# pdlfs/old-vpic

Hardware: AMD Instinct MI355X
Metric: particle-pushes/sec (full step: advance_p + sort when due + field solve + glue) (higher is better)
Workload: dtype f32

## Files before the change

old-vpic_amd/csrc/collide.hip:

```cpp
#include "engine.h"
#include <algorithm>

namespace vpichip {

enum { CW_BAD = 0, CW_FULLEST_A, CW_FULLEST_B, CW_SLOTS = 8, COLLIDE_SLOTS = 64, COLLIDE_WORDS = CW_SLOTS + 4 * COLLIDE_SLOTS };
enum { CS_CELLS = 0, CS_PAIRS, CS_SKIPPED, CS_ONE_SIDED };
constexpr int COLLIDE_MAX_GROUPS_WAVE = 16384, COLLIDE_MAX_GROUPS = 4096;
constexpr int COLLIDE_SLAB_ARRAYS = 6;

__device__ __forceinline__ unsigned c_mix32(unsigned x) { x ^= x >> 16; x *= 0x7feb352du; x ^= x >> 15; x *= 0x846ca68bu; x ^= x >> 16; return x; }
__device__ __forceinline__ float c_unit(unsigned r) { return ((float)(r >> 8) + 0.5f) * (1.f / 16777216.f); }

struct CollideSpK {
  float *ux, *uy, *uz; const float *q; const float4 *r; const int *starts;
  int order, np;
  float wq, f;
  unsigned id;
};
struct CollideK {
  CollideSpK a, b;
  float cvar, dt, den;
  unsigned seed, call, rank;
  const float *draws;
  unsigned long long *words;
  int nx, ny, nz, sy, sz, nv, stride;
  TileK tk;
};

__global__ __launch_bounds__(256) void collide_check_particles(CollideSpK s, CollideK k) {
  const int p = blockIdx.x * 256 + threadIdx.x;
  bool bad = false;
  if (p < s.np) {
    const int v = record_cell(s.r, p);
    if (v < 0 || v >= k.nv) bad = true;
    else {
      int cx, cy, cz;
      voxel_cell(v, k.tk, cx, cy, cz);
      if (cx < 1 || cx > k.nx || cy < 1 || cy > k.ny || cz < 1 || cz > k.nz) bad = true;
      else {
        const int at = s.order == 2 ? sort_key<true>(v, k.tk) : v;
        bad = !(p >= s.starts[at] && p < s.starts[at + 1]);
      }
    }
  }
  if (__ballot(bad) && (threadIdx.x & 63) == 0) atomicOr(k.words + CW_BAD, 1ull);
}
__global__ __launch_bounds__(256) void collide_check_cells(CollideSpK s, int n_ranges, unsigned long long *words, int slot) {
// ... 12 lines not shown
struct Slab { float *ux, *uy, *uz, *w; unsigned *key; int *perm; };
__device__ __forceinline__ Slab slab_at(unsigned *base, int stride) {
  Slab s;
  s.ux = reinterpret_cast<float *>(base); s.uy = s.ux + stride; s.uz = s.uy + stride; s.w = s.uz + stride;
  s.key = base + 4 * stride; s.perm = reinterpret_cast<int *>(base + 5 * stride);
  return s;
}
__device__ __forceinline__ unsigned cell_c0(const CollideK &k, unsigned species, int v) {
  return c_mix32((k.seed ^ c_mix32(k.call * 0x9e3779b9u + species)) + c_mix32(k.rank * 0x85ebca6bu + (unsigned)v));
}
__device__ __forceinline__ void cell_range(const CollideSpK &s, int v, int key, int &lo, int &n) {
  lo = 0; n = 0;
  if (s.order == 0) return;
  const int at = s.order == 2 ? key : v;
  lo = s.starts[at]; n = s.starts[at + 1] - lo;
}
__device__ __forceinline__ bool block_cell(const CollideK &k, unsigned b, int &v, int &key) {
  int x, y, z;
  if (k.a.order == 2) {
    const int tile = (int)(b >> 6), c = (int)(b & 63u);
    const int tx = tile % k.tk.ntx, ty = (tile / k.tk.ntx) % k.tk.nty, tz = tile / (k.tk.ntx * k.tk.nty);
    x = tx << 2 | (c & 3); y = ty << 2 | (c >> 2 & 3); z = tz << 2 | (c >> 4);
    if (x >= k.nx || y >= k.ny || z >= k.nz) return false;
  } else {
    x = (int)(b % (unsigned)k.nx); y = (int)((b / (unsigned)k.nx) % (unsigned)k.ny); z = (int)(b / ((unsigned)k.nx * (unsigned)k.ny));
  }
  v = (x + 1) + k.sy * (y + 1) + k.sz * (z + 1);
  key = (((z >> 2) * k.tk.nty + (y >> 2)) * k.tk.ntx + (x >> 2)) * TILE_CELLS + ((z & 3) << 4 | (y & 3) << 2 | (x & 3));
  return true;
}
template <int T>
__device__ __forceinline__ void load_cell(const CollideSpK &s, const Slab &l, int lo, int n, unsigned c0) {
  for (int k = threadIdx.x; k < n; k += T) {
    l.ux[k] = s.ux[lo + k]; l.uy[k] = s.uy[lo + k]; l.uz[k] = s.uz[lo + k];
    l.w[k] = fabsf(s.q[lo + k]) * s.wq;
    l.key[k] = c_mix32(c0 + (unsigned)k);
  }
}
template <int T>
__device__ __forceinline__ void store_cell(const CollideSpK &s, const Slab &l, int lo, int n) {
  for (int k = threadIdx.x; k < n; k += T) { s.ux[lo + k] = l.ux[k]; s.uy[lo + k] = l.uy[k]; s.uz[lo + k] = l.uz[k]; }
}
template <int T>
__device__ __forceinline__ void rank_cell(const Slab &l, int n, unsigned c0) {
  if (T == 64) {
    const unsigned mine = c_mix32(c0 + threadIdx.x);
    int r = 0;
    for (int j = 0; j < n; j++) r += (unsigned)__shfl((int)mine, j) < mine ? 1 : 0;
    if ((int)threadIdx.x < n) l.perm[r] = (int)threadIdx.x;
  } else {
    for (int k = threadIdx.x; k < n; k += T) {
      const unsigned mine = l.key[k];
      int r = 0;
      for (int j = 0; j < n; j++) r += l.key[j] < mine ? 1 : 0;
      l.perm[r] = k;
    }
  }
}

struct Draws { float n, c, s, u; };
__device__ __forceinline__ Draws pair_draws(const CollideK &k, unsigned c0, unsigned j, int first_index) {
  Draws d;
  if (k.draws) {
    const float4 t = reinterpret_cast<const float4 *>(k.draws)[first_index];
    d.n = t.x; d.c = t.y; d.s = t.z; d.u = t.w;
  } else {
    const unsigned base = c_mix32(c0 ^ 0x2545f491u) + 4u * j;
    const float u0 = c_unit(c_mix32(base)), u1 = c_unit(c_mix32(base + 1u)), u2 = c_unit(c_mix32(base + 2u));
    d.n = sqrtf(-2.f * logf(u0)) * cospif(2.f * u1);
    d.s = sinpif(2.f * u2); d.c = cospif(2.f * u2);
    d.u = c_unit(c_mix32(base + 3u));
  }
  return d;
}
// ... 126 lines not shown
        for (int j = m; j < n_L; j += n_S) {
          const int kf = L.perm[j];
          count(pair_of<REL>(k, L, kf, S, ks, f_L, f_S, fN, false, pair_draws(k, c0_L, (unsigned)j, lo_L + kf)));
        }
      }
    }
    __syncthreads();
    store_cell<T>(k.a, A, lo_a, n_a);
    if (!SAME) store_cell<T>(k.b, B, lo_b, n_b);
  }
  __syncthreads();
  if (n_pairs) atomicAdd(&s_cnt[0], n_pairs);
  if (n_skipped) atomicAdd(&s_cnt[1], n_skipped);
  if (n_one_sided) atomicAdd(&s_cnt[2], n_one_sided);
  __syncthreads();
  if (threadIdx.x == 0 && cells) {
    unsigned long long *slot = k.words + CW_SLOTS + 4 * (blockIdx.x % COLLIDE_SLOTS);
    atomicAdd(slot + CS_CELLS, (unsigned long long)cells);
    if (s_cnt[0]) atomicAdd(slot + CS_PAIRS, (unsigned long long)s_cnt[0]);
    if (s_cnt[1]) atomicAdd(slot + CS_SKIPPED, (unsigned long long)s_cnt[1]);
    if (s_cnt[2]) atomicAdd(slot + CS_ONE_SIDED, (unsigned long long)s_cnt[2]);
  }
}

static CollideSpecies describe(const Species &s, const TileK &tk) {
  CollideSpecies d;
  d.np = s.np; d.n_sorted = s.n_sorted; d.n_holes = s.n_holes; d.fuse_pending = s.fuse_pending;
  d.tile_valid = s.tile_valid && tile_partition_usable(s, tk); d.coarse_sorted = s.coarse_sorted;
  d.partition_valid = !s.tile_valid && s.partition_valid && s.partition;
  return d;
}
static CollideSpK species_k(const Species &s, const CollideSpecies &d, int id, float wq, float f) {
  CollideSpK k;
  k.ux = s.p.ux; k.uy = s.p.uy; k.uz = s.p.uz; k.q = s.p.q; k.r = s.p.r;
  k.order = s.np == 0 ? 0 : d.tile_valid ? 2 : 1;
  k.starts = k.order == 2 ? s.tpart : s.partition;
  k.np = (int)s.np; k.wq = wq; k.f = f; k.id = (unsigned)id;
  return k;
}
static int sort_exact(Engine *e, Species &s, bool wants_tile) {
  if (s.nm > 0) VH_FAIL("collide: the species must be sorted first and has %lld movers pending", (long long)s.nm);
  const bool tile = s.tile_valid || (!s.partition_valid && wants_tile);
  const int knob = e->knobs.tile_coarse;
  e->knobs.tile_coarse = 0;
  const int rc = k_sort_p(e, s, tile, false);
  e->knobs.tile_coarse = knob;
  return rc;
}
static int check_species(Engine *e, const CollideSpK &s, const CollideK &k, int slot) {
  if (s.order == 0) return 0;
  const int n_ranges = s.order == 2 ? k.tk.ntiles * TILE_CELLS : k.nv;
  hipLaunchKernelGGL(collide_check_cells, dim3((n_ranges + 255) / 256), dim3(256), 0, e->stream, s, n_ranges, k.words, slot);
  hipLaunchKernelGGL(collide_check_particles, dim3((s.np + 255) / 256), dim3(256), 0, e->stream, s, k);
  VH_CHECK(hipGetLastError());
  return 0;
}

template <bool REL>
static void launch_collide(Engine *e, const CollideK &K, bool wave, bool same, unsigned groups, size_t lds, unsigned cells) {
  if (wave) {
    if (same) hipLaunchKernelGGL((collide_kernel<64, true, REL>), dim3(groups), dim3(64), lds, e->stream, K, cells);
    else hipLaunchKernelGGL((collide_kernel<64, false, REL>), dim3(groups), dim3(64), lds, e->stream, K, cells);
  } else {
    if (same) hipLaunchKernelGGL((collide_kernel<256, true, REL>), dim3(groups), dim3(256), lds, e->stream, K, cells);
    else hipLaunchKernelGGL((collide_kernel<256, false, REL>), dim3(groups), dim3(256), lds, e->stream, K, cells);
  }
}
// ... 63 lines not shown
```

old-vpic_amd/csrc/cool.hip:

```cpp
#include "dist_coords.h"
#include <algorithm>

namespace vpichip {

constexpr int COOL_WAVES = 4;
constexpr int COOL_THREADS = 64 * COOL_WAVES;
constexpr int COOL_MAX_BLOCKS = 1024;
constexpr int COOL_TOGETHER_ROUNDS = 2;
constexpr unsigned COOL_NEED = NEED_FIELD;
enum { COOL_SEEN = 0, COOL_CHANGED, COOL_REFUSED, COOL_ALONE, COOL_SUM };

struct CoolK { double sync, ic, quantum; };

template <bool DRY, bool CELLS>
__global__ __launch_bounds__(COOL_THREADS)
void cool_kernel(ParticlesK p, long long np, CoolK k, int nv, const vpic_interpolator_t *__restrict__ fi,
                 unsigned long long *__restrict__ cells, unsigned long long *__restrict__ stats) {
  const int lane = threadIdx.x & 63;
  const long long stride = (long long)gridDim.x * COOL_THREADS;
  long long idx = (long long)blockIdx.x * COOL_THREADS + threadIdx.x;
  unsigned long long n_seen = 0, n_changed = 0, n_refused = 0, n_alone = 0;
  long long sum = 0;
  DistRaw next = dist_load<true>(p, idx, np, COOL_NEED);
  float next_q = dist_load_q(p, idx, np, VAL_Q);
  for (; idx - lane < np; idx += stride) {
    const DistRaw r = next;
    const float q = next_q;
    const DistField f = dist_gather(fi, r.voxel, nv, COOL_NEED);
    next = dist_load<true>(p, idx + stride, np, COOL_NEED);
    next_q = dist_load_q(p, idx + stride, np, VAL_Q);
    const bool live = r.voxel >= 0 && r.voxel < nv;
    n_seen += __popcll(__ballot(live));
    bool tallied = false;
    long long addend = 0;
    if (live) {
      const float3 el = dist_e_at(r, f), cb = dist_b_at(r, f);
      const double Ex = (double)el.x, Ey = (double)el.y, Ez = (double)el.z, Bx = (double)cb.x, By = (double)cb.y, Bz = (double)cb.z;
      const double ux = (double)r.ux, uy = (double)r.uy, uz = (double)r.uz;
      const double u2 = (ux * ux + uy * uy) + uz * uz, g = sqrt(1.0 + u2), rg = 1.0 / g;
      const double vx = ux * rg, vy = uy * rg, vz = uz * rg;
      const double Lx = Ex + (vy * Bz - vz * By), Ly = Ey + (vz * Bx - vx * Bz), Lz = Ez + (vx * By - vy * Bx);
      const double vE = (vx * Ex + vy * Ey) + vz * Ez;
      const double Ax = (Ly * Bz - Lz * By) + vE * Ex, Ay = (Lz * Bx - Lx * Bz) + vE * Ey, Az = (Lx * By - Ly * Bx) + vE * Ez;
      const double L2 = (Lx * Lx + Ly * Ly) + Lz * Lz;
      double chi = L2 - vE * vE;
      if (chi < 0.0) chi = 0.0;
      const double D = g * (k.sync * chi + k.ic), den = 1.0 + D;
      const double nx = (ux + k.sync * Ax) / den, ny = (uy + k.sync * Ay) / den, nz = (uz + k.sync * Az) / den;
      if (isfinite(D) && isfinite(nx) && isfinite(ny) && isfinite(nz)) {
        const float fx = (float)nx, fy = (float)ny, fz = (float)nz;
        if (__float_as_uint(fx) != __float_as_uint(r.ux) || __float_as_uint(fy) != __float_as_uint(r.uy) ||
            __float_as_uint(fz) != __float_as_uint(r.uz)) n_changed++;
        if (!DRY) { p.ux[idx] = fx; p.uy[idx] = fy; p.uz[idx] = fz; }
        const double wx = (double)fx, wy = (double)fy, wz = (double)fz;
        const double u2n = (wx * wx + wy * wy) + wz * wz, g1 = sqrt(1.0 + u2n);
        const double val = (double)fabsf(q) * ((u2 - u2n) / (g + g1));
        const double t = val / k.quantum;
        tallied = fabs(t) < 4294967296.0;
        if (tallied) { addend = llrint(t); sum += addend; }
        else n_refused++;
      } else n_alone++;
    }
    if (CELLS) {
      bool pending = tallied;
#pragma unroll
      for (int round = 0; round < COOL_TOGETHER_ROUNDS; round++) {
        const unsigned long long any = __ballot(pending);
        if (!any) break;
        const int lead = __ffsll((long long)any) - 1;
        const int v0 = __builtin_amdgcn_readlane(r.voxel, lead);
        const bool shared = pending && r.voxel == v0;
        const unsigned long long same = __ballot(shared);
        add_sums_together(cells, r.voxel, addend, shared, __popcll(same) >= SUMS_TOGETHER_MIN, same, lead, lane);
        pending = pending && !shared;
      }
      if (pending && addend) atomicAdd(cells + r.voxel, (unsigned long long)addend);
    }
  }
#pragma unroll
  for (int m = 32; m >= 1; m >>= 1) {
    sum += __shfl_xor(sum, m);
    n_changed += __shfl_xor(n_changed, m);
    n_refused += __shfl_xor(n_refused, m);
    n_alone += __shfl_xor(n_alone, m);
  }
  if (lane == 0 && n_seen) {
// ... 28 lines not shown
```

old-vpic_amd/csrc/dist_coords.h:

```cpp
#pragma once
#include "engine.h"
#include <math.h>

namespace vpichip {

constexpr unsigned NEED_POS = 7u, NEED_KE = 3u << VPIC_HIP_COORD_KE;
constexpr unsigned NEED_FIELD = 0x3fu << VPIC_HIP_COORD_U_PAR, NEED_FIELD_E = 1u << VPIC_HIP_COORD_E_PAR;
constexpr unsigned NEED_FIELD_U = NEED_FIELD & ~(1u << VPIC_HIP_COORD_B | NEED_FIELD_E);
constexpr unsigned NEED_FIELD_PERP = 1u << VPIC_HIP_COORD_U_PERP | 1u << VPIC_HIP_COORD_MU;
static_assert(VPIC_HIP_COORD_U_PAR == 16 && VPIC_HIP_COORD_E_PAR == 21 && NEED_FIELD == 0x3f0000u, "the field coordinates are bits 16 to 21");

struct DistCoords { double x, y, z, ux, uy, uz, ke, log_ke, u_par, u_perp, pitch, mu, b, e_par; };

template <bool FIELDS>
__device__ __forceinline__ double dist_coord(const DistCoords &v, int coord) {
  if (FIELDS) {
    if (coord >= VPIC_HIP_COORD_U_PAR)
      return coord == VPIC_HIP_COORD_U_PAR ? v.u_par : coord == VPIC_HIP_COORD_U_PERP ? v.u_perp : coord == VPIC_HIP_COORD_PITCH ? v.pitch
           : coord == VPIC_HIP_COORD_MU ? v.mu : coord == VPIC_HIP_COORD_B ? v.b : v.e_par;
  }
  return coord == VPIC_HIP_COORD_X ? v.x : coord == VPIC_HIP_COORD_Y ? v.y : coord == VPIC_HIP_COORD_Z ? v.z
       : coord == VPIC_HIP_COORD_UX ? v.ux : coord == VPIC_HIP_COORD_UY ? v.uy : coord == VPIC_HIP_COORD_UZ ? v.uz
       : coord == VPIC_HIP_COORD_KE ? v.ke : v.log_ke;
}

template <bool FIELDS>
__device__ __forceinline__ bool dist_in_range(const DistCoords &v, const vpic_hip_dist_range_t &r) {
  const double c = dist_coord<FIELDS>(v, r.coord);
  return c >= r.lo && c < r.hi;
}

template <bool FIELDS>
__device__ __forceinline__ bool dist_in_ranges(const DistCoords &v, const vpic_hip_dist_range_t (&sel)[4], int n_sel) {
  bool in = true;
  if (n_sel > 0) in = in && dist_in_range<FIELDS>(v, sel[0]);
  if (n_sel > 1) in = in && dist_in_range<FIELDS>(v, sel[1]);
  if (n_sel > 2) in = in && dist_in_range<FIELDS>(v, sel[2]);
  if (n_sel > 3) in = in && dist_in_range<FIELDS>(v, sel[3]);
  return in;
}

struct DistRaw { int voxel; float dx, dy, dz, ux, uy, uz; };

template <bool FIELDS>
__device__ __forceinline__ DistRaw dist_load(const ParticlesK &p, long long idx, long long end, unsigned need) {
  DistRaw r{-1, 0.f, 0.f, 0.f, 0.f, 0.f, 0.f};
  const bool u = FIELDS && (need & NEED_FIELD_U);
  if (idx < end) {
    const float4 rec = p.r[idx];
    r.voxel = record_cell(rec); r.dx = rec.x; r.dy = rec.y; r.dz = rec.z;
    if (u || (need & (NEED_KE | 1u << VPIC_HIP_COORD_UX))) r.ux = p.ux[idx];
    if (u || (need & (NEED_KE | 1u << VPIC_HIP_COORD_UY))) r.uy = p.uy[idx];
    if (u || (need & (NEED_KE | 1u << VPIC_HIP_COORD_UZ))) r.uz = p.uz[idx];
  }
  return r;
}

struct DistField { float4 b; float2 c; float4 ex, ey, ez; };

__device__ __forceinline__ DistField dist_gather(const vpic_interpolator_t *__restrict__ fi, int voxel, int nv, unsigned need) {
  DistField f{};
  if (voxel >= 0 && voxel < nv) {
    const float4 *q = reinterpret_cast<const float4 *>(fi + voxel);
    f.b = q[3];
    f.c = *reinterpret_cast<const float2 *>(q + 4);
    if (need & NEED_FIELD_E) { f.ex = q[0]; f.ey = q[1]; f.ez = q[2]; }
  }
  return f;
}
static_assert(sizeof(vpic_interpolator_t) == 80, "an interpolator record is five float4");

__device__ __forceinline__ float3 dist_b_at(const DistRaw &r, const DistField &f) {
  return make_float3(f.b.x + r.dx * f.b.y, f.b.z + r.dy * f.b.w, f.c.x + r.dz * f.c.y);
}
__device__ __forceinline__ float3 dist_e_at(const DistRaw &r, const DistField &f) {
  return make_float3((f.ex.x + r.dy * f.ex.y) + r.dz * (f.ex.z + r.dy * f.ex.w),
                     (f.ey.x + r.dz * f.ey.y) + r.dx * (f.ey.z + r.dz * f.ey.w),
                     (f.ez.x + r.dx * f.ez.y) + r.dy * (f.ez.z + r.dx * f.ez.w));
}

template <bool FIELDS>
__device__ __forceinline__ DistCoords dist_coords(const DistRaw &r, const DistField &f, unsigned need, const TileK &t, int &cx, int &cy, int &cz) {
  DistCoords v{};
  if (need & NEED_POS) {
    voxel_cell(r.voxel, t, cx, cy, cz);
    if (need & 1u) v.x = (double)(cx - 1) + ((double)r.dx + 1.0) * 0.5;
// ... 11 lines not shown
    const double b = sqrt((bx * bx + by * by) + bz * bz);
    v.b = b;
    if (need & NEED_FIELD_U) {
      const double u_par = ((v.ux * bx + v.uy * by) + v.uz * bz) / b;
      const double u2 = (v.ux * v.ux + v.uy * v.uy) + v.uz * v.uz;
      v.u_par = u_par;
      if (need & NEED_FIELD_PERP) {
        const double perp2 = u2 - u_par * u_par;
        const double p2 = perp2 < 0.0 ? 0.0 : perp2;
        if (need & 1u << VPIC_HIP_COORD_U_PERP) v.u_perp = sqrt(p2);
        if (need & 1u << VPIC_HIP_COORD_MU) v.mu = p2 / (2.0 * b);
      }
      if (need & 1u << VPIC_HIP_COORD_PITCH) v.pitch = u_par / sqrt(u2);
    }
    if (need & NEED_FIELD_E) {
      const float3 el = dist_e_at(r, f);
      v.e_par = (((double)el.x * bx + (double)el.y * by) + (double)el.z * bz) / b;
    }
  }
  return v;
}

constexpr unsigned VAL_Q = 1u, VAL_EDOTV = 2u, VAL_EPAR_VPAR = 4u;
inline void dist_factor_need(int code, unsigned &need, unsigned &vneed) {
  if (code < VPIC_HIP_FACTOR_ONE) { need |= 1u << code; return; }
  if (code == VPIC_HIP_FACTOR_Q) vneed |= VAL_Q;
  if (code == VPIC_HIP_FACTOR_EDOTV) { vneed |= VAL_EDOTV; need |= 1u << VPIC_HIP_COORD_KE | NEED_FIELD_E; }
  if (code == VPIC_HIP_FACTOR_EPAR_VPAR) { vneed |= VAL_EPAR_VPAR; need |= 1u << VPIC_HIP_COORD_KE | NEED_FIELD_E | 1u << VPIC_HIP_COORD_U_PAR; }
}

struct DistExtra { double q, edotv, epar_vpar; };

__device__ __forceinline__ float dist_load_q(const ParticlesK &p, long long idx, long long end, unsigned vneed) {
  return (vneed & VAL_Q) && idx < end ? p.q[idx] : 0.f;
}

template <bool FIELDS>
__device__ __forceinline__ DistExtra dist_extra(const DistRaw &r, const DistField &f, float q, const DistCoords &v, unsigned vneed) {
  DistExtra x{};
  x.q = (double)q;
  if (FIELDS && (vneed & (VAL_EDOTV | VAL_EPAR_VPAR))) {
    const double gamma = sqrt(((1.0 + v.ux * v.ux) + v.uy * v.uy) + v.uz * v.uz);
    if (vneed & VAL_EDOTV) {
      const float3 el = dist_e_at(r, f);
      x.edotv = (((double)el.x * v.ux + (double)el.y * v.uy) + (double)el.z * v.uz) / gamma;
    }
    if (vneed & VAL_EPAR_VPAR) x.epar_vpar = (v.e_par * v.u_par) / gamma;
  }
  return x;
}

template <bool FIELDS>
__device__ __forceinline__ double dist_factor(const DistCoords &v, const DistExtra &x, int code) {
  if (code >= VPIC_HIP_FACTOR_ONE)
    return code == VPIC_HIP_FACTOR_ONE ? 1.0 : code == VPIC_HIP_FACTOR_Q ? x.q
         : FIELDS && code == VPIC_HIP_FACTOR_EDOTV ? x.edotv : x.epar_vpar;
  return dist_coord<FIELDS>(v, code);
}

struct SelectK {
  vpic_hip_select_t s;
  unsigned need;
  int use_tag;
};
inline SelectK make_select_k(const vpic_hip_select_t &d) {
  SelectK k{};
  k.s = d;
// ... 18 lines not shown
```

old-vpic_amd/csrc/engine.h:

```cpp
#pragma once
#include <hip/hip_runtime.h>
#include <stdint.h>
#include <string>
#include <vector>
#include "vpic_hip.h"
#include "policy.h"
#include "moments_device.h"

namespace vpichip {

void set_error(const char *fmt, ...);
#define VH_CHECK(expr)                                                                     \
  do {                                                                                     \
    hipError_t _e = (expr);                                                                \
    if (_e != hipSuccess) {                                                                \
      vpichip::set_error("%s failed: %s (%s:%d)", #expr, hipGetErrorString(_e), __FILE__, __LINE__); \
      return 1;                                                                            \
    }                                                                                      \
  } while (0)
#define VH_FAIL(...) do { vpichip::set_error(__VA_ARGS__); return 1; } while (0)

struct GridK {
  int nx, ny, nz, sy, sz, nv;
  int fbc[6], pbc[6];
  int rank;
};

enum { F_EX = 0, F_EY, F_EZ, F_DIV_E_ERR, F_CBX, F_CBY, F_CBZ, F_DIV_B_ERR,
       F_TCAX, F_TCAY, F_TCAZ, F_RHOB, F_JFX, F_JFY, F_JFZ, F_RHOF, F_NCOMP };
enum { M_EMATX = 0, M_EMATY, M_EMATZ, M_NMAT, M_FMATX, M_FMATY, M_FMATZ, M_CMAT, M_NCOMP };
struct FieldsK {
  float *c[F_NCOMP];
  uint16_t *m[M_NCOMP];
};

struct ParticlesK {
  float4 *r;
  float *ux, *uy, *uz, *q;
};
__host__ __device__ __forceinline__ float4 make_record(float dx, float dy, float dz, int i) {
  union { int i; float f; } w; w.i = i;
  return make_float4(dx, dy, dz, w.f);
}
__device__ __forceinline__ int record_cell(const float4 *r, long long k) { return __float_as_int(r[k].w); }
__device__ __forceinline__ int record_cell(const float4 &v) { return __float_as_int(v.w); }
__device__ __forceinline__ void record_set_cell(float4 *r, long long k, int i) { r[k].w = __int_as_float(i); }
__host__ __device__ __forceinline__ ParticlesK offset_particles(const ParticlesK &p, int64_t at) {
  ParticlesK o = p;
  o.r += at; o.ux += at; o.uy += at; o.uz += at; o.q += at;
  return o;
}

struct DrainParams {
  int nx, ny, nz, sy, sz, rank, max_nm;
  unsigned mul_sz;
  int pbc[6];
  unsigned mul_sy, shifts;
  vpic_particle_mover_t *pm;
  int *nm_counter;
};

inline void magic_div(unsigned d, unsigned &mul, unsigned &shift) {
  unsigned l = 0;
  while ((1ull << l) < d) l++;
  const unsigned p = 31 + l;
  mul = (unsigned)(((unsigned long long)1 << p) / d + 1);
  shift = p - 32;
}

enum { C_NM = 0, C_DISORDER = 1, C_LOCAL = 2, C_SEND = 8, C_HOLES = 14, C_FILLS = 15, C_NP = 16, C_NMS = 48, C_CHARGED = 80, C_OVER = 81, C_RETRY = 82, C_QMSG = 83, C_NHOLE = 96, C_QTOP = 128, C_TOTAL = 160 };
constexpr int MAX_SPECIES = 32;
constexpr int HEADER_BASE = 256, MAX_HEADERS = 192;
constexpr int RETRY_CAP = 1 << 16;
static_assert(C_NMS + MAX_SPECIES == C_CHARGED && C_NP + MAX_SPECIES == C_NMS && C_NHOLE + MAX_SPECIES == C_QTOP && C_QTOP + MAX_SPECIES == C_TOTAL && C_TOTAL <= HEADER_BASE, "counter layout");

struct Species {
  float q_m = 0;
  float q_max = 0;
  int64_t np = 0, max_np = 0, nm = 0, max_nm = 0;
  int64_t n_holes = 0;
  ParticlesK p{}, aux{};
  DrainParams *drain_k = nullptr;
// ... 374 lines not shown
```

old-vpic_amd/csrc/engine.hip:

```cpp
#include "engine.h"
#include "cell_coords.h"
#include <algorithm>
#include <cstdarg>
#include <cstdio>
#include <cstring>
#include <functional>
#include <cstdlib>
#include <cmath>

namespace vpichip {

static thread_local char g_error[1024] = "";
void set_error(const char *fmt, ...) {
  va_list ap;
  va_start(ap, fmt);
  vsnprintf(g_error, sizeof(g_error), fmt, ap);
  va_end(ap);
}

static vpic_hip_host_access_fn g_host_access = nullptr;
void host_will_read(const void *p, size_t bytes) { if (g_host_access && p && bytes) g_host_access(p, bytes, 0); }
void host_will_write(void *p, size_t bytes) { if (g_host_access && p && bytes) g_host_access(p, bytes, 1); }

int ensure_stage(Engine *e, size_t bytes) { return grow(e->stage, e->stage_bytes, bytes); }
// ... 103 lines not shown
static double fixed_scale(double largest) {
  int ex = 0;
  (void)frexp(largest, &ex);
  return ldexp(1.0, 37 - ex);
}
int acc_prepare_det(Engine *e, double q_arriving) {
  if (!e->acc64) {
    VH_CHECK(hipMalloc(&e->acc64, sizeof(unsigned long long) * 12 * (size_t)e->gk.nv));
    VH_CHECK(hipMemsetAsync(e->acc64, 0, sizeof(unsigned long long) * 12 * (size_t)e->gk.nv, e->stream));
  }
  if (e->acc_scale == 0) {
    double q = e->acc_qref;
    if (!(q > 0)) for (auto &s : e->species) q = std::max(q, (double)s.q_max);
    if (!(q > 0)) q = q_arriving;
    if (!(q > 0) && q_arriving < 0) return 0;
    if (!(q > 0)) VH_FAIL("deterministic accumulation: no macro-particle charge is known yet (give vpic_hip_set_accumulation a reference charge)");
    e->acc_scale = fixed_scale(4.2 * q);
  }
  e->acc64_dirty = true;
  return 0;
}
int acc_finalize(Engine *e) {
  if (!e->acc64 || !e->acc64_dirty) return 0;
  const size_t n = 12 * (size_t)e->gk.nv;
  hipLaunchKernelGGL(acc_finalize_kernel, dim3((unsigned)((n + 255) / 256)), dim3(256), 0, e->stream,
                     reinterpret_cast<float *>(e->acc), e->acc64, n, 1.0 / e->acc_scale);
  VH_CHECK(hipGetLastError());
  e->acc64_dirty = false;
  return 0;
}

void free_particles(ParticlesK &p) {
  (void)hipFree(p.r);
  (void)hipFree(p.ux); (void)hipFree(p.uy); (void)hipFree(p.uz); (void)hipFree(p.q);
  p = ParticlesK{};
}

static void destroy(Engine *e) {
  if (e->stream) (void)hipStreamSynchronize(e->stream);
  for (auto &s : e->species) {
    free_particles(s.p); free_particles(s.aux);
    (void)hipFree(s.tag); (void)hipFree(s.tag2); (void)hipFree(s.tag_aux); (void)hipFree(s.tag2_aux);
    (void)hipFree(s.pm); (void)hipFree(s.partition); (void)hipFree(s.tpart); (void)hipFree(s.tpart2); (void)hipFree(s.ttail); (void)hipFree(s.hist); (void)hipFree(s.drain_k); (void)hipFree(s.crossed_dev); (void)hipHostFree(s.crossed_host);
    for (int i = 0; i < 4; i++) if (s.ev[i]) (void)hipEventDestroy(s.ev[i]);
    for (auto ev : s.sp_ev) if (ev) (void)hipEventDestroy(ev);
    for (auto ev : s.hp_ev) if (ev) (void)hipEventDestroy(ev);
  }
  (void)hipFree(e->field_block); (void)hipFree(e->mat_block); (void)hipFree(e->mc);
  (void)hipFree(e->fi); (void)hipFree(e->acc_block); (void)hipHostFree(e->host_miss); (void)hipFree(e->stage); (void)hipFree(e->counters); (void)hipFree(e->hydro); (void)hipFree(e->hydro_buf[0]); (void)hipFree(e->hydro_buf[1]);
  (void)hipHostFree(e->host_counters); (void)hipFree(e->dsum); (void)hipHostFree(e->host_dsum);
  (void)hipFree(e->sort_next); (void)hipFree(e->scan_tmp);
  (void)hipFree(e->face_buf[0]); (void)hipFree(e->face_buf[1]);
  for (int f = 0; f < 6; f++) (void)hipFree(e->send_buf[f]);
  (void)hipFree(e->local_buf); (void)hipFree(e->reflux_draws); (void)hipFree(e->emit_draws);
  (void)hipFree(e->wall_table); (void)hipFree(e->wall_rec); (void)hipFree(e->wall_cursor);
  (void)hipFree(e->collide_draws); (void)hipFree(e->collide_dev); (void)hipHostFree(e->collide_host);
  (void)hipFree(e->load_draws); (void)hipFree(e->load_tab);
  (void)hipFree(e->cool_cells); (void)hipHostFree(e->cool_cells_host); e->cool_stats.release();
  (void)hipFree(e->hole_list); (void)hipFree(e->fill_list); (void)hipFree(e->tail_flag);
  (void)hipFree(e->sp_table_dev); (void)hipHostFree(e->sp_table_host); (void)hipFree(e->xmsg_dev); (void)hipHostFree(e->xmsg_host);
  (void)hipFree(e->retry_buf); (void)hipFree(e->tile_list[0]); (void)hipFree(e->tile_list[1]);
  (void)hipFree(e->acc64); (void)hipFree(e->rho64);
  (void)hipFree(e->spec_lin); (void)hipFree(e->spec_bands); (void)hipFree(e->spec_log); (void)hipHostFree(e->spec_log_host);
  e->species_hist.release(); e->cell_hist.release(); (void)hipFree(e->hydro64);
  (void)hipFree(e->sel_mask); (void)hipFree(e->sel_offsets); (void)hipFree(e->sel_counts);
  (void)hipFree(e->sel_p); (void)hipFree(e->sel_f); (void)hipFree(e->sel_i);
  for (DiagStats<4> *st : {&e->spec_stats, &e->dist_stats, &e->mom_stats, &e->sel_stats}) st->release();
  for (auto &ev : e->ev_pool) { (void)hipEventDestroy(ev.first); (void)hipEventDestroy(ev.second); }
// ... 365 lines not shown
  if (s.nm == 0) return 0;
  host_will_write(pm, sizeof(*pm) * (size_t)s.nm);
  if (copy_out(e, pm, s.pm, sizeof(*pm) * (size_t)s.nm)) return 1;
  std::sort(pm, pm + s.nm, [](const vpic_particle_mover_t &a, const vpic_particle_mover_t &b) { return a.i < b.i; });
  return 0;
}
int vpic_hip_species_get_partition(vpic_hip_engine_t *e, int sp, int32_t *partition) {
  ENGINE(e); SPECIES(e, sp);
  Species &s = e->species[sp];
  if (!s.partition || !s.partition_valid) VH_FAIL("partition is only valid right after sort_p");
  return copy_out(e, partition, s.partition, sizeof(int) * ((size_t)e->gk.nv + 1));
}

#ifdef VPIC_HIP_ABLATION
int vpic_hip_debug_set_ablate(vpic_hip_engine_t *e, int bits) { ENGINE(e); e->knobs.ablate = bits; return 0; }
#endif
int vpic_hip_debug_poke_tile_max(vpic_hip_engine_t *e, int sp, unsigned value) {
  ENGINE(e); SPECIES(e, sp);
  if (!e->species[sp].crossed_host) VH_FAIL("no counter word");
  e->species[sp].crossed_host[PW_FULLEST_TILE] = value;
  return 0;
}
int vpic_hip_debug_set_particles_any_voxel(vpic_hip_engine_t *e, int sp, const vpic_particle_t *p, int64_t np) {
  ENGINE(e); SPECIES(e, sp);
  if (np < 0 || (np > 0 && !p)) VH_FAIL("Bad particle array");
  host_will_read(p, sizeof(*p) * (size_t)np);
  return k_particles_from_aos(e, e->species[sp], p, np, 0, true);
}
int vpic_hip_debug_set_momenta(vpic_hip_engine_t *e, int sp, const float *ux, const float *uy, const float *uz, int64_t n) {
  ENGINE(e); SPECIES(e, sp);
  Species &s = e->species[sp];
  if (!ux || !uy || !uz || n != s.np) VH_FAIL("Bad momenta: %lld, the species' extent is %lld", (long long)n, (long long)s.np);
  if (n == 0) return 0;
  if (copy_in(e, s.p.ux, ux, sizeof(float) * (size_t)n) || copy_in(e, s.p.uy, uy, sizeof(float) * (size_t)n)) return 1;
  return copy_in(e, s.p.uz, uz, sizeof(float) * (size_t)n);
}
int vpic_hip_species_get_tile_partition(vpic_hip_engine_t *e, int sp, int32_t *tpart, int64_t *count) {
  ENGINE(e); SPECIES(e, sp);
  Species &s = e->species[sp];
  const int64_t n1 = (int64_t)make_tile_k(e->gk).ntiles * TILE_CELLS + 1;
  if (count) *count = n1;
  if (!tpart) return 0;
  if (!s.tpart || !s.tile_valid || s.tpart_count < n1) VH_FAIL("the tile partition is only valid while the species is in the engine's order");
  return copy_out(e, tpart, s.tpart, sizeof(int) * (size_t)n1);
}

int vpic_hip_load_interpolator(vpic_hip_engine_t *e) { ENGINE(e); return k_load_interpolator(e); }
int vpic_hip_clear_accumulators(vpic_hip_engine_t *e) {
  ENGINE(e);
  VH_CHECK(hipMemsetAsync(e->acc, 0, sizeof(vpic_accumulator_t) * (size_t)e->gk.nv, e->stream));
  if (e->acc64 && e->acc64_dirty) {
    VH_CHECK(hipMemsetAsync(e->acc64, 0, sizeof(unsigned long long) * 12 * (size_t)e->gk.nv, e->stream));
    e->acc64_dirty = false;
  }
  return 0;
}
int vpic_hip_set_accumulation(vpic_hip_engine_t *e, int mode, double q_ref) {
  ENGINE(e);
  if (mode != 0 && mode != 1) VH_FAIL("Bad accumulation mode %d", mode);
  if (acc_finalize(e)) return 1;
  e->det_acc = mode == 1;
  e->acc_qref = q_ref > 0 ? q_ref : 0;
  e->acc_scale = 0;
  return 0;
}
int vpic_hip_reduce_accumulators(vpic_hip_engine_t *e) { ENGINE(e); return 0; }
int vpic_hip_unload_accumulator(vpic_hip_engine_t *e) { ENGINE(e); return k_unload_accumulator(e); }
int vpic_hip_set_push_mode(vpic_hip_engine_t *e, int mode) {
// ... 587 lines not shown
```

old-vpic_amd/csrc/fields.hip:

```cpp
#include "push_device.h"

namespace vpichip {

#define VOX(x, y, z) ((x) + g.sy * (y) + g.sz * (z))

struct Box3 { int bx, by, bz; };
__device__ __forceinline__ bool decode(const Box3 &b, unsigned t, int &x, int &y, int &z) {
  const unsigned per_z = (unsigned)b.bx * b.by;
  if (t >= per_z * (unsigned)b.bz) return false;
  const unsigned zz = t / per_z, r = t - zz * per_z, yy = r / (unsigned)b.bx;
  x = 1 + (int)(r - yy * b.bx); y = 1 + (int)yy; z = 1 + (int)zz;
  return true;
}

constexpr int BAND = 8;
__host__ __device__ __forceinline__ unsigned banded_count(const Box3 &b) {
  return (unsigned)((b.by + BAND - 1) / BAND) * (unsigned)b.bz * BAND * (unsigned)b.bx;
}
static inline unsigned banded_grid(const Box3 &b) { return ((banded_count(b) + 255u) / 256u + 7u) / 8u * 8u; }
__device__ __forceinline__ bool decode_banded(const Box3 &b, unsigned block, unsigned nblocks, unsigned tid, int &x, int &y, int &z) {
  const unsigned t = xcd_block(block, nblocks) * 256u + tid;
  if (t >= banded_count(b)) return false;
  const unsigned r = t / (unsigned)b.bx, yy = r % BAND, r2 = r / BAND, band = r2 / (unsigned)b.bz;
  x = 1 + (int)(t - r * b.bx); z = 1 + (int)(r2 - band * b.bz); y = 1 + (int)(band * BAND + yy);
// ... 699 lines not shown
  const vpic_hip_grid_t &G = e->grid;
  if (!e->mc) VH_FAIL("energy_f: no material coefficients set");
  const int nb = (int)(e->dsum_count / 6);
  if (e->f.m[0])
    hipLaunchKernelGGL(energy_f_kernel<false>, dim3(nb), dim3(256), 0, e->stream, e->f, e->mc, g, e->dsum);
  else
    hipLaunchKernelGGL(energy_f_kernel<true>, dim3(nb), dim3(256), 0, e->stream, e->f, e->mc, g, e->dsum);
  VH_CHECK(hipGetLastError());
  VH_CHECK(hipMemcpyAsync(e->host_dsum, e->dsum, sizeof(double) * 6 * nb, hipMemcpyDeviceToHost, e->stream));
  VH_CHECK(hipStreamSynchronize(e->stream));
  const double v0 = 0.5 * G.eps0 * G.dx * G.dy * G.dz;
  for (int k = 0; k < 6; k++) {
    double s = 0;
    for (int b = 0; b < nb; b++) s += e->host_dsum[b * 6 + k];
    en6[k] = s * v0;
  }
  return 0;
}



int k_clear_rhof(Engine *e) {
  VH_CHECK(hipMemsetAsync(e->f.c[F_RHOF], 0, sizeof(float) * (size_t)e->gk.nv, e->stream));
  return 0;
}

__global__ __launch_bounds__(256)
void accumulate_rho_p_kernel(float *__restrict__ rhof, ParticlesK p, int np, float r8V, int sy, int sz) {
  const int idx = blockIdx.x * 256 + threadIdx.x;
  if (idx >= np) return;
  const float4 rec = p.r[idx];
  if (record_cell(rec) < 0) return;
  float w[8];
  node_weights(rec.x, rec.y, rec.z, p.q[idx], r8V, w);
  float *r = rhof + record_cell(rec);
  atomicAdd(r, w[0]); atomicAdd(r + 1, w[1]); atomicAdd(r + sy, w[2]); atomicAdd(r + sy + 1, w[3]);
  atomicAdd(r + sz, w[4]); atomicAdd(r + sz + 1, w[5]); atomicAdd(r + sz + sy, w[6]); atomicAdd(r + sz + sy + 1, w[7]);
}
__global__ __launch_bounds__(256)
void accumulate_rho_cells_kernel(float *__restrict__ rhof, ParticlesK p, const int *__restrict__ partition, int nv,
                                 float r8V, int sy, int sz) {
  const int v = blockIdx.x * 256 + threadIdx.x;
  if (v >= nv) return;
  const int first = partition[v], last = partition[v + 1];
  if (first >= last) return;
  float s0 = 0, s1 = 0, s2 = 0, s3 = 0, s4 = 0, s5 = 0, s6 = 0, s7 = 0;
#pragma unroll 1
  for (int idx = first; idx < last; idx++) {
    float w[8];
    const float4 rec = p.r[idx];
    node_weights(rec.x, rec.y, rec.z, p.q[idx], r8V, w);
    s0 += w[0]; s1 += w[1]; s2 += w[2]; s3 += w[3]; s4 += w[4]; s5 += w[5]; s6 += w[6]; s7 += w[7];
  }
  float *r = rhof + v;
  atomicAdd(r, s0); atomicAdd(r + 1, s1); atomicAdd(r + sy, s2); atomicAdd(r + sy + 1, s3);
  atomicAdd(r + sz, s4); atomicAdd(r + sz + 1, s5); atomicAdd(r + sz + sy, s6); atomicAdd(r + sz + sy + 1, s7);
}
int k_rho_p_untiled(Engine *e, Species &s, bool by_cell) {
  const vpic_hip_grid_t &G = e->grid;
  const float r8V = 0.125 * G.rdx * G.rdy * G.rdz;
  if (by_cell) {
    if (!s.partition_valid && k_sort_p(e, s)) return 1;
    hipLaunchKernelGGL(accumulate_rho_cells_kernel, dim3((unsigned)((e->gk.nv + 255) / 256)), dim3(256), 0, e->stream,
                       e->f.c[F_RHOF], s.p, s.partition, e->gk.nv, r8V, e->gk.sy, e->gk.sz);
    VH_CHECK(hipGetLastError());
    return 0;
  }
  hipLaunchKernelGGL(accumulate_rho_p_kernel, dim3((unsigned)((s.np + 255) / 256)), dim3(256), 0, e->stream,
                     e->f.c[F_RHOF], s.p, (int)s.np, r8V, e->gk.sy, e->gk.sz);
  VH_CHECK(hipGetLastError());
  return 0;
}

static int local_adjust_rho(Engine *e) {
  const GridK &g = e->gk;
  for (int comp = 0; comp < 2; comp++)
    for (int face = 0; face < 6; face++) {
      const int bc = g.fbc[face];
      if (bc >= 0) continue;
      const int axis = face % 3, hi = face >= 3, n = n_axis(g, axis);
      const PlaneBox b = node_box(g, axis, hi ? n + 1 : 1);
      if (bc == VPIC_PEC_FIELDS) { if (local_op(e, one_seg(b, e->f.c[comp ? F_RHOB : F_RHOF]), L_ZERO)) return 1; }
      else if (!comp)            { if (local_op(e, one_seg(b, e->f.c[F_RHOF]), L_DOUBLE)) return 1; }
    }
// ... 445 lines not shown
```

old-vpic_amd/csrc/load.hip:

```cpp
#include "engine.h"
#include "load_rule.h"
#include <cmath>
#include <cstring>
#include <algorithm>
#include <vector>

namespace vpichip {

struct LoadK {
  const int *count;
  const float *q, *ud[3], *uth[3];
  int tsx, tsy, tsz;
  long long g0x, g0y, g0z, GX, GY;
  unsigned seed, stream;
  int flip;
  const float *draws;
  long long tag0;
};

__global__ __launch_bounds__(256)
void load_counts_kernel(int *__restrict__ per_voxel, int nv, GridK g, TileK t, LoadK k) {
  const int v = blockIdx.x * 256 + threadIdx.x;
  if (v > nv) return;
  int n = 0;
// ... 27 lines not shown
  if (threadIdx.x == 64) s_span[1] = holding_voxel(off, 0, nv, m_last);
  __syncthreads();
  const int v0 = s_span[0], v1 = s_span[1], span = v1 - v0;
  const bool in_lds = span < LOAD_SPAN;
  if (in_lds) {
    for (int a = threadIdx.x; a <= span + 1; a += 256) s_off[a] = off[v0 + a];
    __syncthreads();
  }
  const int m = m0 + (int)threadIdx.x;
  if (m >= total) return;
  int v, first;
  if (in_lds) { const int a = holding_voxel(s_off, 0, span + 1, m); v = v0 + a; first = s_off[a]; }
  else { v = holding_voxel(off, v0, v1 + 1, m); first = off[v]; }
  int cx, cy, cz;
  voxel_cell(v, t, cx, cy, cz);
  cx -= 1; cy -= 1; cz -= 1;
  const int at = cx * k.tsx + cy * k.tsy + cz * k.tsz;
  const uint64_t cell = load_global_cell((uint64_t)(k.g0x + cx), (uint64_t)(k.g0y + cy), (uint64_t)(k.g0z + cz), (uint64_t)k.GX, (uint64_t)k.GY);
  float d[7];
  if (k.draws) {
#pragma unroll
    for (int a = 0; a < 7; a++) d[a] = k.draws[7ll * m + a];
  } else {
    uint32_t r[8];
    load_words(cell, (uint32_t)(m - first), k.seed, k.stream, r);
    load_numbers(r, d);
  }
  float uth[3], ud[3], u[3];
#pragma unroll
  for (int a = 0; a < 3; a++) { uth[a] = k.uth[a] ? k.uth[a][at] : 0.f; ud[a] = k.ud[a] ? k.ud[a][at] : 0.f; }
  const float n[3] = {d[3], d[4], d[5]};
  load_momentum(uth, ud, n, d[6], k.flip != 0, u);
  p.r[m] = make_record(load_offset(d[0]), load_offset(d[1]), load_offset(d[2]), v);
  p.ux[m] = u[0]; p.uy[m] = u[1]; p.uz[m] = u[2]; p.q[m] = k.q[at];
  if (tags) { tag[m] = tags == 1 ? k.tag0 + m : 0; tag2[m] = 0; }
}

int k_load_profile(Engine *e, Species &s, const vpic_hip_load_t &d, int64_t *n_loaded) {
  const GridK &g = e->gk;
  const int n[3] = {g.nx, g.ny, g.nz};
  if (!d.count) VH_FAIL("load_profile: count is NULL");
  if (!d.q) VH_FAIL("load_profile: q is NULL");
  if (d.flags & ~(VPIC_HIP_LOAD_APPEND | VPIC_HIP_LOAD_FLIP | VPIC_HIP_LOAD_TAGS)) VH_FAIL("load_profile: flags = %d has unknown bits", d.flags);
  const bool append = d.flags & VPIC_HIP_LOAD_APPEND, with_tags = d.flags & VPIC_HIP_LOAD_TAGS;
  for (int a = 0; a < 3; a++) {
    if (d.tdim[a] != 1 && d.tdim[a] != n[a]) VH_FAIL("load_profile: tdim[%d] = %d is neither 1 nor the grid's %d", a, d.tdim[a], n[a]);
    if (d.goff[a] < 0) VH_FAIL("load_profile: goff[%d] = %lld is negative", a, (long long)d.goff[a]);
    if (d.goff[a] > d.gdim[a] - n[a]) VH_FAIL("load_profile: goff[%d] + %d = %lld is beyond gdim[%d] = %lld", a, n[a], (long long)d.goff[a] + n[a], a, (long long)d.gdim[a]);
  }
  if ((double)d.gdim[0] * (double)d.gdim[1] * (double)d.gdim[2] >= 9.2e18) VH_FAIL("load_profile: gdim holds more than 2^63 cells");
  const int64_t T = (int64_t)d.tdim[0] * d.tdim[1] * d.tdim[2], cells = (int64_t)g.nx * g.ny * g.nz, mult = cells / T;
  const size_t count_bytes = sizeof(int32_t) * (size_t)T, table_bytes = sizeof(float) * (size_t)T;
  host_will_read(d.count, count_bytes); host_will_read(d.q, table_bytes);
  for (int a = 0; a < 3; a++) { host_will_read(d.ud[a], table_bytes); host_will_read(d.uth[a], table_bytes); }
  int64_t sum = 0;
  float q_top = 0;
  for (int64_t c = 0; c < T; c++) {
    if (d.count[c] < 0) VH_FAIL("load_profile: count[%lld] = %d is negative", (long long)c, d.count[c]);
    if (!std::isfinite(d.q[c])) VH_FAIL("load_profile: q[%lld] is not finite", (long long)c);
    for (int a = 0; a < 3; a++) {
      if (d.ud[a] && !std::isfinite(d.ud[a][c])) VH_FAIL("load_profile: ud[%d][%lld] is not finite", a, (long long)c);
      if (d.uth[a] && !std::isfinite(d.uth[a][c])) VH_FAIL("load_profile: uth[%d][%lld] is not finite", a, (long long)c);
      if (d.uth[a] && d.uth[a][c] < 0) VH_FAIL("load_profile: uth[%d][%lld] = %g is negative", a, (long long)c, (double)d.uth[a][c]);
    }
    sum += d.count[c];
    if (d.count[c] > 0) q_top = std::max(q_top, fabsf(d.q[c]));
  }
// ... 74 lines not shown
```

old-vpic_amd/csrc/moments.hip:

```cpp
#include "engine.h"
#include "push_device.h"
#include "dist_coords.h"
#include <algorithm>
#include <math.h>

namespace vpichip {

constexpr int MOM_WX = TILE_EDGE + 3;
constexpr int MOM_SLOTS = MOM_WX * MOM_WX * MOM_WX;
constexpr int MOM_TAIL_BLOCKS = 4096;

struct MomK {
  ParticlesK p;
  const float4 *fi;
  const int *tpart; const unsigned *bad;
  long long n_sorted, np;
  int sy, sz, nv_safe;
  TileK t;
  HydroConsts h;
  double scale[HYDRO_MOMENTS];
  unsigned long long *stats;
};
enum { MOM_SEL_NONE = 0, MOM_SEL_BOX = 1, MOM_SEL_FIELD = 2 };
template <int SEL> struct MomKS : MomK { SelectK sel; const int64_t *tag; };
// ... 6 lines not shown
  if (j >= ntiles) return;
  const long long b0 = tpart[(size_t)j * TILE_CELLS], b1 = j + 1 < ntiles ? (long long)tpart[(size_t)(j + 1) * TILE_CELLS] : n_sorted;
  if (b0 < 0 || b0 > b1 || b1 > n_sorted || (j == 0 && b0 != 0)) atomicOr(bad, 1u);
}
int k_check_tile_partition(Engine *e, const Species &s, unsigned *bad) {
  const int ntiles = make_tile_k(e->gk).ntiles;
  hipLaunchKernelGGL(check_tile_partition_kernel, dim3((ntiles + 255) / 256), dim3(256), 0, e->stream, (const int *)s.tpart, ntiles,
                     (long long)s.n_sorted, bad);
  VH_CHECK(hipGetLastError());
  return 0;
}

__device__ __forceinline__ void mom_add(float *word, float x, double, unsigned &) { atomicAdd(word, x); }
__device__ __forceinline__ void mom_add(unsigned long long *word, float x, double scale, unsigned &n_range) {
  if (fabs((double)x * scale) < 2251799813685248.0) atomicAdd(word, to_fixed(x, scale));
  else n_range++;
}

template <int NM, typename ACC> struct MomLayout { static constexpr int STRIDE = NM; };
template <> struct MomLayout<HYDRO_MOMENTS, float> { static constexpr int STRIDE = HYDRO_STRIDE; };

struct MomCount { unsigned live = 0, lds = 0, global = 0, range = 0; };

template <int NM, typename ACC, bool WINDOW, int SEL>
__device__ __forceinline__ void moments_of_particle(const MomKS<SEL> &K, ACC *__restrict__ out, ACC *s_win, long long idx, int bx, int by, int bz, MomCount &n) {
  const float4 rec = K.p.r[idx];
  const int voxel = record_cell(rec);
  if (voxel < 0 || voxel >= K.nv_safe) return;
  HydroP P;
  if constexpr (SEL != MOM_SEL_NONE) {
    static_assert(NM == HYDRO_MOMENTS, "a selection is for the hydro moments");
    constexpr bool FIELDS = SEL == MOM_SEL_FIELD;
    if (K.sel.use_tag && !select_tag_ok(K.sel.s, K.tag ? K.tag[idx] : 0)) return;
    const DistRaw r{voxel, rec.x, rec.y, rec.z, K.p.ux[idx], K.p.uy[idx], K.p.uz[idx]};
    InterpK f;
    if (FIELDS) f = load_interp(K.fi, voxel);
    if (K.sel.s.n_sel > 0) {
      const DistField df = FIELDS ? DistField{f.b0, f.b1, f.ex, f.ey, f.ez} : DistField{};
      int cx = 0, cy = 0, cz = 0;
      const DistCoords v = dist_coords<FIELDS>(r, df, K.sel.need, K.t, cx, cy, cz);
      if (!dist_in_ranges<FIELDS>(v, K.sel.s.sel, K.sel.s.n_sel)) return;
    }
    if (!FIELDS) f = load_interp(K.fi, voxel);
    n.live++;
    hydro_particle(r.dx, r.dy, r.dz, r.ux, r.uy, r.uz, K.p.q[idx], f, K.h, P);
  } else {
    n.live++;
    if constexpr (NM == HYDRO_MOMENTS)
      hydro_particle(rec.x, rec.y, rec.z, K.p.ux[idx], K.p.uy[idx], K.p.uz[idx], K.p.q[idx], load_interp(K.fi, voxel), K.h, P);
    else
      node_weights(rec.x, rec.y, rec.z, K.p.q[idx], K.h.r8V, P.w);
  }
  bool inside = false;
  int slot0 = 0;
  if (WINDOW) {
    int cx, cy, cz;
    voxel_cell(voxel, K.t, cx, cy, cz);
    const unsigned lx = (unsigned)(cx - bx), ly = (unsigned)(cy - by), lz = (unsigned)(cz - bz);
    inside = lx < (unsigned)(MOM_WX - 1) && ly < (unsigned)(MOM_WX - 1) && lz < (unsigned)(MOM_WX - 1);
    slot0 = (int)(lx + MOM_WX * (ly + MOM_WX * lz));
  }
  unsigned range = 0;
  if constexpr (SEL != MOM_SEL_NONE) { n.lds += inside ? 1u : 0u; n.global += inside ? 0u : 1u; }
  if (WINDOW && inside) {
#pragma unroll
    for (int nd = 0; nd < 8; nd++) {
      float c[NM];
      if constexpr (NM == HYDRO_MOMENTS) hydro_node(P, P.w[nd], K.h.mc_q, c); else c[0] = P.w[nd];
      const int slot = slot0 + (nd & 1) + ((nd >> 1) & 1) * MOM_WX + (nd >> 2) * MOM_WX * MOM_WX;
#pragma unroll
      for (int k = 0; k < NM; k++) mom_add(&s_win[k * MOM_SLOTS + slot], c[k], K.scale[k], range);
    }
    if constexpr (SEL == MOM_SEL_NONE) n.lds++;
  } else {
    ACC *g = out + (size_t)voxel * MomLayout<NM, ACC>::STRIDE;
#pragma unroll
    for (int nd = 0; nd < 8; nd++) {
      float c[NM];
      if constexpr (NM == HYDRO_MOMENTS) hydro_node(P, P.w[nd], K.h.mc_q, c); else c[0] = P.w[nd];
      ACC *m = g + (size_t)((nd & 1) + ((nd >> 1) & 1) * K.sy + (nd >> 2) * K.sz) * MomLayout<NM, ACC>::STRIDE;
#pragma unroll
      for (int k = 0; k < NM; k++) mom_add(m + k, c[k], K.scale[k], range);
    }
    if constexpr (SEL == MOM_SEL_NONE) n.global++;
// ... 185 lines not shown
```

old-vpic_amd/csrc/particles.hip:

```cpp
#include "push_device.h"
#include "unit_draw.h"
#include "dist_coords.h"
#include <cstddef>
#include <cstring>
#include <algorithm>

namespace vpichip {

__global__ void particles_from_aos_kernel(ParticlesK p, int64_t *tag, int64_t *tag2,
                                          const vpic_particle_t *__restrict__ src, int64_t first, int n) {
  const int t = blockIdx.x * blockDim.x + threadIdx.x;
  if (t >= n) return;
  const vpic_particle_t s = src[t];
  const int64_t k = first + t;
  p.r[k] = make_record(s.dx, s.dy, s.dz, s.i);
  p.ux[k] = s.ux; p.uy[k] = s.uy; p.uz[k] = s.uz; p.q[k] = s.q;
  if (tag) { tag[k] = s.tag; tag2[k] = s.tag2; }
}
__global__ void particles_to_aos_kernel(ParticlesK p, const int64_t *tag, const int64_t *tag2,
                                        vpic_particle_t *__restrict__ dst, int64_t first, int n) {
  const int t = blockIdx.x * blockDim.x + threadIdx.x;
  if (t >= n) return;
  const int64_t k = first + t;
  vpic_particle_t s;
  const float4 rec = p.r[k];
  s.dx = rec.x; s.dy = rec.y; s.dz = rec.z; s.i = record_cell(rec);
  s.ux = p.ux[k]; s.uy = p.uy[k]; s.uz = p.uz[k]; s.q = p.q[k];
  s.tag = tag ? tag[k] : 0; s.tag2 = tag ? tag2[k] : 0;
  dst[t] = s;
}

static int alloc_particles_raw_impl(ParticlesK &p, int64_t n);
static int alloc_particles_raw(ParticlesK &p, int64_t n) { return alloc_particles_raw_impl(p, n); }
static const int64_t CHUNK = 8 << 20;

int ensure_tags(Engine *e, Species &s) {
  if (s.tag) return 0;
  VH_CHECK(hipMalloc(&s.tag, sizeof(int64_t) * s.max_np));
  VH_CHECK(hipMalloc(&s.tag2, sizeof(int64_t) * s.max_np));
  VH_CHECK(hipMemsetAsync(s.tag, 0, sizeof(int64_t) * s.max_np, e->stream));
  VH_CHECK(hipMemsetAsync(s.tag2, 0, sizeof(int64_t) * s.max_np, e->stream));
  return 0;
}

int k_particles_from_aos(Engine *e, Species &s, const vpic_particle_t *host, int64_t n_new, int64_t at, bool any_voxel) {
  const int64_t np = at + n_new;
  if (np > s.max_np) VH_FAIL("species particles: np=%lld exceeds max_np=%lld", (long long)np, (long long)s.max_np);
  {
    const GridK &g = e->gk;
    for (int64_t k = 0; k < n_new; k++) {
      const int v = host[k].i, z = v / g.sz, r = v - z * g.sz, y = r / g.sy, x = r - y * g.sy;
      if (any_voxel && v >= 0 && v < g.nv) continue;
      if (v < 0 || (unsigned)(x - 1) >= (unsigned)g.nx || (unsigned)(y - 1) >= (unsigned)g.ny || (unsigned)(z - 1) >= (unsigned)g.nz)
        VH_FAIL("particle %lld is not in an interior voxel (i = %d)", (long long)k, v);
    }
  }
  bool any_tag = false;
  for (int64_t k = 0; k < n_new && !any_tag; k++) any_tag = host[k].tag != 0 || host[k].tag2 != 0;
  if (any_tag) { if (ensure_tags(e, s)) return 1; s.has_tags = true; }
  bool any_q = false;
// ... 19 lines not shown
  if (cap < count) VH_FAIL("species_get_particles: buffer holds %lld, asked for %lld", (long long)cap, (long long)count);
  host -= from;
  for (int64_t first = from; first < from + count; first += CHUNK) {
    const int n = (int)((from + count - first < CHUNK) ? from + count - first : CHUNK);
    if (ensure_stage(e, sizeof(vpic_particle_t) * (size_t)n)) return 1;
    hipLaunchKernelGGL(particles_to_aos_kernel, dim3((n + 255) / 256), dim3(256), 0, e->stream, s.p,
                       s.has_tags ? s.tag : nullptr, s.tag2, (vpic_particle_t *)e->stage, first, n);
    VH_CHECK(hipGetLastError());
    VH_CHECK(hipMemcpyAsync(host + first, e->stage, sizeof(vpic_particle_t) * (size_t)n, hipMemcpyDeviceToHost, e->stream));
    VH_CHECK(hipStreamSynchronize(e->stream));
  }
  return 0;
}

__device__ __forceinline__ unsigned hash32(unsigned x) {
  x ^= x >> 16; x *= 0x7feb352du; x ^= x >> 15; x *= 0x846ca68bu; x ^= x >> 16;
  return x;
}
__device__ __forceinline__ float u01(unsigned seed, unsigned idx, unsigned k) {
  const unsigned h = hash32(hash32(idx * 9u + k) ^ hash32(seed * 0x9e3779b9u + k));
  return unit_top_closed(h);
}
__global__ __launch_bounds__(256)
void load_maxwellian_kernel(ParticlesK p, GridK g, int ppc, int np, unsigned seed, float q,
                            float ux0, float uy0, float uz0, float vth) {
  const int idx = blockIdx.x * 256 + threadIdx.x;
  if (idx >= np) return;
  const int cell = idx / ppc;
  const int cz = cell / (g.nx * g.ny), r = cell - cz * g.nx * g.ny, cy = r / g.nx, cx = r - cy * g.nx;
  p.r[idx] = make_record(2.f * u01(seed, idx, 0) - 1.f, 2.f * u01(seed, idx, 1) - 1.f, 2.f * u01(seed, idx, 2) - 1.f,
                         (cx + 1) + g.sy * (cy + 1) + g.sz * (cz + 1));
  const float r1 = sqrtf(-2.f * logf(u01(seed, idx, 3))), a1 = 6.2831853f * u01(seed, idx, 4);
  const float r2 = sqrtf(-2.f * logf(u01(seed, idx, 5))), a2 = 6.2831853f * u01(seed, idx, 6);
  p.ux[idx] = ux0 + vth * r1 * cosf(a1);
  p.uy[idx] = uy0 + vth * r1 * sinf(a1);
  p.uz[idx] = uz0 + vth * r2 * cosf(a2);
  p.q[idx] = q;
}

int k_load_maxwellian(Engine *e, Species &s, int ppc, unsigned seed, float q, float ux, float uy, float uz, float vth) {
  const int64_t np = (int64_t)e->gk.nx * e->gk.ny * e->gk.nz * ppc;
  if (ppc < 1 || np > s.max_np) VH_FAIL("load_maxwellian: %lld particles exceed max_np=%lld", (long long)np, (long long)s.max_np);
  hipLaunchKernelGGL(load_maxwellian_kernel, dim3((unsigned)((np + 255) / 256)), dim3(256), 0, e->stream, s.p, e->gk,
                     ppc, (int)np, seed, q, ux, uy, uz, vth);
  VH_CHECK(hipGetLastError());
  s.np = np; s.nm = 0; s.partition_valid = false; s.tile_valid = false; s.n_holes = 0; s.hist_valid = false;
  s.q_max = std::max(s.q_max, fabsf(q));
  s.chargeless = q == 0.f;
  return 0;
}

constexpr int MAX_GROUPS = 16;
__device__ __forceinline__ void group_info(int key, bool valid, int lane, int &leader, int &rank, int &cnt) {
  unsigned long long todo = __ballot(valid);
  leader = lane; rank = 0; cnt = 1;
  for (int it = 0; todo && it < MAX_GROUPS; ++it) {
    const int lead = __ffsll((long long)todo) - 1;
    const int k0 = __builtin_amdgcn_readlane(key, lead);
    const bool mine = valid && key == k0;
    const unsigned long long m = __ballot(mine);
    if (mine) {
      leader = lead;
      rank = (int)__builtin_amdgcn_mbcnt_hi((unsigned)(m >> 32), __builtin_amdgcn_mbcnt_lo((unsigned)m, 0u));
      cnt = __popcll(m);
    }
    todo &= ~m;
  }
}

TileK make_tile_k(const GridK &g) {
// ... 50 lines not shown
    const int v = k < nb ? block_sum[k] : 0;
    int incl = v;
    for (int off = 1; off < 64; off <<= 1) { const int u = __shfl_up(incl, off); if (lane >= off) incl += u; }
    if (lane == 63) s_wave[threadIdx.x >> 6] = incl;
    __syncthreads();
    int wave_off = 0;
    for (int w = 0; w < (int)(threadIdx.x >> 6); w++) wave_off += s_wave[w];
    const int carry = s_carry;
    if (k < nb) block_sum[k] = carry + wave_off + incl - v;
    __syncthreads();
    if (threadIdx.x == 255) s_carry = carry + wave_off + incl;
    __syncthreads();
  }
}
__global__ __launch_bounds__(256)
void scan_add_kernel(int *__restrict__ out, int *__restrict__ copy, const int *__restrict__ block_sum, int n) {
  const int base = blockIdx.x * 1024 + threadIdx.x * 4;
  const int add = block_sum[blockIdx.x];
#pragma unroll
  for (int k = 0; k < 4; k++)
    if (base + k < n) { const int v = out[base + k] + add; out[base + k] = v; copy[base + k] = v; }
}

template <bool TILE>
__global__ __launch_bounds__(256)
void sort_scatter_kernel(ParticlesK in, ParticlesK out, const int64_t *tin, const int64_t *t2in,
                         int64_t *tout, int64_t *t2out, int np, int *__restrict__ next, const TileK t) {
  const int idx = blockIdx.x * 256 + threadIdx.x;
  const int lane = threadIdx.x & 63;
  const int li = idx < np ? idx : 0;
  const float4 rec = in.r[li];
  const int key = idx < np ? record_cell(rec) : -1;
  const bool valid = key >= 0;
  const float ux = in.ux[li], uy = in.uy[li], uz = in.uz[li], q = in.q[li];
  int leader, rank, cnt;
  group_info(key, valid, lane, leader, rank, cnt);
  int base = 0;
  if (valid && lane == leader) base = atomicAdd(&next[sort_key<TILE>(key, t)], cnt);
  base = __shfl(base, leader);
  if (!valid) return;
  const int dst = base + rank;
  out.r[dst] = rec;
  out.ux[dst] = ux; out.uy[dst] = uy; out.uz[dst] = uz; out.q[dst] = q;
  if (tin) { tout[dst] = tin[idx]; t2out[dst] = t2in[idx]; }
}

#ifndef VPIC_HIP_SORT_THREADS
#define VPIC_HIP_SORT_THREADS 256
#endif
#ifndef VPIC_HIP_SORT_XCD
#define VPIC_HIP_SORT_XCD 1
#endif
constexpr int WG_T = VPIC_HIP_SORT_THREADS, WG_PER_THREAD = 8, WG_CHUNK = WG_T * WG_PER_THREAD, WG_TABLE = 512, WG_EPT = WG_TABLE / WG_T;
static_assert(WG_T == 256 || WG_T == 512, "threads of a sort workgroup");

__device__ __forceinline__ int wg_slot(int *s_key, int skey) {
  unsigned h = ((unsigned)skey * 2654435761u) >> 23;
  for (int probe = 0; probe < WG_TABLE; probe++) {
    const int prev = atomicCAS(&s_key[h], -1, skey);
    if (prev == -1 || prev == skey) return (int)h;
    h = (h + 1) & (WG_TABLE - 1);
  }
  return -1;
}

template <bool TILE>
__global__ __launch_bounds__(WG_T)
void wg_count_kernel(const float4 *__restrict__ rec, int np, int *__restrict__ count, const TileK t) {
  __shared__ int s_key[WG_TABLE], s_cnt[WG_TABLE];
  for (int k = threadIdx.x; k < WG_TABLE; k += WG_T) { s_key[k] = -1; s_cnt[k] = 0; }
  __syncthreads();
  const int first = blockIdx.x * WG_CHUNK;
  int key[WG_PER_THREAD];
#pragma unroll
  for (int j = 0; j < WG_PER_THREAD; j++) { const int idx = first + j * WG_T + threadIdx.x; key[j] = idx < np ? record_cell(rec, idx) : -1; }
  const int lane = threadIdx.x & 63;
#pragma unroll
  for (int j = 0; j < WG_PER_THREAD; j++) {
    const bool valid = key[j] >= 0;
    int leader, rank, cnt;
    group_info(key[j], valid, lane, leader, rank, cnt);
    if (valid && lane == leader) {
      const int skey = sort_key<TILE>(key[j], t);
      const int h = wg_slot(s_key, skey);
      if (h >= 0) atomicAdd(&s_cnt[h], cnt); else atomicAdd(&count[skey], cnt);
    }
  }
  __syncthreads();
  for (int k = threadIdx.x; k < WG_TABLE; k += WG_T) if (s_key[k] >= 0) atomicAdd(&count[s_key[k]], s_cnt[k]);
}

template <bool TILE, bool COARSE = false>
__global__ __launch_bounds__(WG_T)
void wg_scatter_kernel(ParticlesK in, ParticlesK out, const int64_t *tin, const int64_t *t2in,
                       int64_t *tout, int64_t *t2out, int np, int *__restrict__ next, const TileK t) {
  static_assert(WG_CHUNK >= 4 * WG_TABLE, "the tables fit the first staging buffer");
  __shared__ float4 s_both[WG_CHUNK / 2];
  int *const s_tables = reinterpret_cast<int *>(s_both);
  float *const s_stage = reinterpret_cast<float *>(s_both) + WG_CHUNK;
  int *const s_key = s_tables, *const s_cnt = s_tables + WG_TABLE, *const s_lbase = s_tables + 2 * WG_TABLE, *const s_gbase = s_tables + 3 * WG_TABLE;
  __shared__ int s_dst[WG_CHUNK];
  __shared__ int s_wave[WG_T / 64], s_total;
  for (int k = threadIdx.x; k < WG_TABLE; k += WG_T) { s_key[k] = -1; s_cnt[k] = 0; }
  __syncthreads();
#if VPIC_HIP_SORT_XCD
  if ((long long)xcd_block(blockIdx.x, gridDim.x) * WG_CHUNK >= np) return;
  const int first = (int)xcd_block(blockIdx.x, gridDim.x) * WG_CHUNK;
#else
  if ((long long)blockIdx.x * WG_CHUNK >= np) return;
  const int first = blockIdx.x * WG_CHUNK;
#endif
  int slot[WG_PER_THREAD], rank[WG_PER_THREAD], key[WG_PER_THREAD];
#pragma unroll
  for (int j = 0; j < WG_PER_THREAD; j++) { const int idx = first + j * WG_T + threadIdx.x; key[j] = idx < np ? record_cell(in.r, idx) : -1; }
  const int lane = threadIdx.x & 63;
#pragma unroll
  for (int j = 0; j < WG_PER_THREAD; j++) {
    const bool valid = key[j] >= 0;
    int leader, r, cnt, h = -2, base = 0;
    const int gkey = COARSE ? (valid ? sort_key<true>(key[j], t) / TILE_CELLS : -1) : key[j];
    group_info(gkey, valid, lane, leader, r, cnt);
    if (valid && lane == leader) {
      const int skey = COARSE ? gkey * TILE_CELLS : sort_key<TILE>(key[j], t);
      h = wg_slot(s_key, skey);
      if (h >= 0) base = atomicAdd(&s_cnt[h], cnt);
      else base = atomicAdd(&next[skey], cnt);
    }
    h = __shfl(h, leader); base = __shfl(base, leader);
    slot[j] = valid ? h : -2; rank[j] = base + r;
  }
  __syncthreads();
  {
    int c[WG_EPT], t = 0;
#pragma unroll
    for (int k = 0; k < WG_EPT; k++) { c[k] = s_cnt[WG_EPT * threadIdx.x + k]; t += c[k]; }
    int incl = t;
    const int lane = threadIdx.x & 63;
    for (int off = 1; off < 64; off <<= 1) { const int u = __shfl_up(incl, off); if (lane >= off) incl += u; }
    if (lane == 63) s_wave[threadIdx.x >> 6] = incl;
    __syncthreads();
    int wave_off = 0;
    for (int w = 0; w < (int)(threadIdx.x >> 6); w++) wave_off += s_wave[w];
    int run = wave_off + incl - t;
#pragma unroll
    for (int k = 0; k < WG_EPT; k++) {
      s_lbase[WG_EPT * threadIdx.x + k] = run; run += c[k];
      if (c[k]) s_gbase[WG_EPT * threadIdx.x + k] = atomicAdd(&next[s_key[WG_EPT * threadIdx.x + k]], c[k]);
    }
    if (threadIdx.x == WG_T - 1) s_total = wave_off + incl;
  }
  __syncthreads();
  int local[WG_PER_THREAD];
#pragma unroll
  for (int j = 0; j < WG_PER_THREAD; j++) {
    local[j] = -1;
    if (slot[j] >= 0) { local[j] = s_lbase[slot[j]] + rank[j]; s_dst[local[j]] = s_gbase[slot[j]] + rank[j]; }
  }
  __syncthreads();
  const int n_staged = s_total;
  float *const src[4] = {in.ux, in.uy, in.uz, in.q};
  float *const dst[4] = {out.ux, out.uy, out.uz, out.q};
  float *const stage2 = reinterpret_cast<float *>(s_tables);
  float v[WG_PER_THREAD];
  {
    constexpr int HALF = WG_CHUNK / 2, GROUP = 4;
#pragma unroll
    for (int half = 0; half < 2; half++) {
#pragma unroll
      for (int j0 = 0; j0 < WG_PER_THREAD; j0 += GROUP) {
        float4 rec[GROUP];
        bool here[GROUP];
#pragma unroll
        for (int j = 0; j < GROUP; j++) {
          const int idx = first + (j0 + j) * WG_T + threadIdx.x;
          here[j] = local[j0 + j] >= 0 ? (local[j0 + j] >= HALF) == (half == 1) : (slot[j0 + j] == -1 && half == 0);
          rec[j] = here[j] ? in.r[idx] : make_float4(0.f, 0.f, 0.f, 0.f);
        }
#pragma unroll
        for (int j = 0; j < GROUP; j++) {
          if (!here[j]) continue;
          if (local[j0 + j] >= 0) s_both[local[j0 + j] - half * HALF] = rec[j];
          else out.r[rank[j0 + j]] = rec[j];
        }
      }
      if (half == 1) {
#pragma unroll
        for (int j = 0; j < WG_PER_THREAD; j++) { const int idx = first + j * WG_T + threadIdx.x; v[j] = (slot[j] != -2) ? src[0][idx] : 0.f; }
      }
      __syncthreads();
      for (int k = threadIdx.x; k < HALF; k += WG_T) { if (half * HALF + k < n_staged) out.r[s_dst[half * HALF + k]] = s_both[k]; }
      __syncthreads();
    }
  }
#pragma unroll
  for (int f = 0; f < 4; f++) {
    float *const stage = (f & 1) ? stage2 : s_stage;
    float vn[WG_PER_THREAD];
    if (f + 1 < 4) {
#pragma unroll
      for (int j = 0; j < WG_PER_THREAD; j++) { const int idx = first + j * WG_T + threadIdx.x; vn[j] = (slot[j] != -2) ? src[f + 1][idx] : 0.f; }
    }
#pragma unroll
    for (int j = 0; j < WG_PER_THREAD; j++) {
      if (local[j] >= 0) stage[local[j]] = v[j];
      else if (slot[j] == -1) dst[f][rank[j]] = v[j];
    }
    __syncthreads();
#pragma unroll
    for (int j = 0; j < WG_PER_THREAD; j++) { const int k = j * WG_T + threadIdx.x; if (k < n_staged) dst[f][s_dst[k]] = stage[k]; }
    if (f + 1 < 4) {
#pragma unroll
      for (int j = 0; j < WG_PER_THREAD; j++) v[j] = vn[j];
    }
  }
  if (tin) {
#pragma unroll
    for (int j = 0; j < WG_PER_THREAD; j++) {
      if (slot[j] == -2) continue;
      const int idx = first + j * WG_T + threadIdx.x;
      const int d = local[j] >= 0 ? s_dst[local[j]] : rank[j];
      tout[d] = tin[idx]; t2out[d] = t2in[idx];
    }
  }
}

constexpr int COARSE_CHUNK = 2048, COARSE_PER_THREAD = COARSE_CHUNK / 256, COARSE_TABLE = 128;

__device__ __forceinline__ int tile_of(int voxel, const TileK &t) { return sort_key<true>(voxel, t) / TILE_CELLS; }

__device__ __forceinline__ int coarse_slot(int *s_key, int tile) {
  unsigned h = ((unsigned)tile * 2654435761u) >> 25;
  for (int probe = 0; probe < COARSE_TABLE; probe++) {
    const int prev = atomicCAS(&s_key[h], -1, tile);
    if (prev == -1 || prev == tile) return (int)h;
    h = (h + 1) & (COARSE_TABLE - 1);
  }
  return -1;
}

__global__ __launch_bounds__(256)
void coarse_count_kernel(const float4 *__restrict__ rec, int np, int *__restrict__ count, const TileK t) {
  __shared__ int s_key[COARSE_TABLE], s_cnt[COARSE_TABLE];
  if (threadIdx.x < COARSE_TABLE) { s_key[threadIdx.x] = -1; s_cnt[threadIdx.x] = 0; }
  __syncthreads();
  const int first = blockIdx.x * COARSE_CHUNK;
#pragma unroll
  for (int j = 0; j < COARSE_PER_THREAD; j++) {
    const int idx = first + j * 256 + threadIdx.x;
    const int voxel = idx < np ? record_cell(rec, idx) : -1;
    if (voxel >= 0) {
      const int tile = tile_of(voxel, t);
      const int h = coarse_slot(s_key, tile);
      if (h >= 0) atomicAdd(&s_cnt[h], 1);
      else atomicAdd(&count[tile * TILE_CELLS], 1);
    }
  }
  __syncthreads();
  if (threadIdx.x < COARSE_TABLE && s_key[threadIdx.x] >= 0) atomicAdd(&count[s_key[threadIdx.x] * TILE_CELLS], s_cnt[threadIdx.x]);
}

int alloc_particles(ParticlesK &p, int64_t n_req) {
  const int64_t n = (n_req + PUSH_TILE + PARTICLE_PAD - 1) / PARTICLE_PAD * PARTICLE_PAD;
  if (alloc_particles_raw(p, n)) return 1;
  VH_CHECK(hipMemset(p.r + (n - PARTICLE_PAD), 0, sizeof(float4) * PARTICLE_PAD));
  float *arr[4] = {p.ux, p.uy, p.uz, p.q};
  for (float *a : arr) VH_CHECK(hipMemset(a + (n - PARTICLE_PAD), 0, sizeof(float) * PARTICLE_PAD));
  VH_CHECK(hipDeviceSynchronize());
  return 0;
}
static int alloc_particles_raw_impl(ParticlesK &p, int64_t n) {
  VH_CHECK(hipMalloc(&p.r, sizeof(float4) * n));
  VH_CHECK(hipMalloc(&p.ux, sizeof(float) * n)); VH_CHECK(hipMalloc(&p.uy, sizeof(float) * n));
  VH_CHECK(hipMalloc(&p.uz, sizeof(float) * n)); VH_CHECK(hipMalloc(&p.q, sizeof(float) * n));
  return 0;
}

__global__ __launch_bounds__(256) void tile_max_kernel(const int *__restrict__ tpart, int ntiles, unsigned *__restrict__ host_word) {
  __shared__ int s_max[4];
  int m = 0;
  for (int t = blockIdx.x * 256 + threadIdx.x; t < ntiles; t += gridDim.x * 256) m = max(m, tpart[(t + 1) * TILE_CELLS] - tpart[t * TILE_CELLS]);
  for (int off = 32; off; off >>= 1) m = max(m, __shfl_down(m, off));
  if ((threadIdx.x & 63) == 0) s_max[threadIdx.x >> 6] = m;
  __syncthreads();
  if (threadIdx.x == 0) atomicMax(host_word, (unsigned)max(max(s_max[0], s_max[1]), max(s_max[2], s_max[3])));
}
__global__ void clear_word_kernel(unsigned *__restrict__ w) { *w = 0; }
__global__ void publish_word_kernel(unsigned *__restrict__ host_word, const unsigned *__restrict__ dev_word) { *host_word = *dev_word; }

int k_sort_p(Engine *e, Species &s, bool tile_order, bool may_fuse) {
  const TileK tk = make_tile_k(e->gk);
  const int n1 = (tile_order ? tk.ntiles * TILE_CELLS : e->gk.nv) + 1;
  SortInputs in;
  in.tile_order = tile_order; in.may_fuse = may_fuse; in.np = s.np; in.n_sorted = s.n_sorted;
  in.adaptive = s.adaptive; in.chargeless = s.chargeless; in.has_tags = s.has_tags;
  in.tile_valid = s.tile_valid; in.coarse_sorted = s.coarse_sorted; in.counts_ready = s.hist_valid && s.hist && s.hist_count >= n1;
  in.det_acc = e->det_acc; in.time_kernels = e->time_kernels; in.tile_coarse = e->knobs.tile_coarse; in.old_sort = e->knobs.old_sort;
  const SortPlan pl = plan_sort(s.pol, in);
  const bool coarse = pl.coarse;
  const int nv = e->gk.nv;
  if (!s.partition) VH_CHECK(hipMalloc(&s.partition, sizeof(int) * (nv + 1)));
  if (tile_order && s.tpart_count < n1) {
    if (s.tpart) VH_CHECK(hipFree(s.tpart));
    s.tpart = nullptr; s.tpart_count = 0;
    VH_CHECK(hipMalloc(&s.tpart, sizeof(int) * n1));
    s.tpart_count = n1;
  }
// ... 58 lines not shown
  hipLaunchKernelGGL(scan_add_kernel, dim3(nb), dim3(256), 0, e->stream, starts, e->sort_next, e->scan_tmp, n1);
  VH_CHECK(hipGetLastError());
  return 0;
}

int k_sort_finish(Engine *e, Species &s, bool tile_order, bool coarse) {
  const TileK tk = make_tile_k(e->gk);
  if (tile_order) {
    unsigned *word = reinterpret_cast<unsigned *>(e->counters + 200);
    hipLaunchKernelGGL(clear_word_kernel, dim3(1), dim3(1), 0, e->stream, word);
    hipLaunchKernelGGL(tile_max_kernel, dim3((unsigned)std::min(256, (tk.ntiles + 255) / 256)), dim3(256), 0, e->stream, s.tpart, tk.ntiles, word);
    hipLaunchKernelGGL(publish_word_kernel, dim3(1), dim3(1), 0, e->stream, s.crossed_host_dev + PW_FULLEST_TILE, (const unsigned *)word);
  }
  VH_CHECK(hipGetLastError());
  std::swap(s.p, s.aux);
  if (s.has_tags) { std::swap(s.tag, s.tag_aux); std::swap(s.tag2, s.tag2_aux); }
  s.np -= s.n_holes; s.n_holes = 0;
  s.partition_valid = !tile_order;
  s.tile_valid = tile_order; s.n_sorted = s.np; s.coarse_sorted = coarse;
  if (s.crossed_dev) VH_CHECK(hipMemsetAsync(s.crossed_dev + 2, 0, sizeof(unsigned), e->stream));
  if (e->time_kernels) { (void)hipEventRecord(s.ev[3], e->stream); s.sort_timed = true; }
  s.pol.new_cycle(tile_order);
  return 0;
}

int k_compact(Engine *e, Species &s) { return s.n_holes > 0 ? k_sort_p(e, s, s.tile_valid) : 0; }

int k_species_reserve(Engine *e, Species &s, int64_t max_np, int64_t max_nm) {
  VH_CHECK(hipStreamSynchronize(e->stream));
  if (max_np > (1ll << 31) - 8192) VH_FAIL("a species holds at most 2^31 - 8192 particles");
  if (max_np > s.max_np) {
    ParticlesK bigger{};
    if (alloc_particles(bigger, max_np)) return 1;
    float *src[4] = {s.p.ux, s.p.uy, s.p.uz, s.p.q};
    float *dst[4] = {bigger.ux, bigger.uy, bigger.uz, bigger.q};
    if (s.np > 0) VH_CHECK(hipMemcpyAsync(bigger.r, s.p.r, sizeof(float4) * (size_t)s.np, hipMemcpyDeviceToDevice, e->stream));
    for (int a = 0; a < 4; a++) {
      if (s.np > 0) VH_CHECK(hipMemcpyAsync(dst[a], src[a], sizeof(float) * (size_t)s.np, hipMemcpyDeviceToDevice, e->stream));
    }
    VH_CHECK(hipStreamSynchronize(e->stream));
    free_particles(s.p);
    s.p = bigger;
    if (s.aux.r) free_particles(s.aux);
    if (s.tag) {
      int64_t *t = nullptr, *t2 = nullptr;
      VH_CHECK(hipMalloc(&t, sizeof(int64_t) * max_np)); VH_CHECK(hipMalloc(&t2, sizeof(int64_t) * max_np));
      VH_CHECK(hipMemsetAsync(t, 0, sizeof(int64_t) * max_np, e->stream)); VH_CHECK(hipMemsetAsync(t2, 0, sizeof(int64_t) * max_np, e->stream));
      if (s.np > 0) {
        VH_CHECK(hipMemcpyAsync(t, s.tag, sizeof(int64_t) * (size_t)s.np, hipMemcpyDeviceToDevice, e->stream));
        VH_CHECK(hipMemcpyAsync(t2, s.tag2, sizeof(int64_t) * (size_t)s.np, hipMemcpyDeviceToDevice, e->stream));
      }
      VH_CHECK(hipStreamSynchronize(e->stream));
      (void)hipFree(s.tag); (void)hipFree(s.tag2); (void)hipFree(s.tag_aux); (void)hipFree(s.tag2_aux);
      s.tag = t; s.tag2 = t2; s.tag_aux = s.tag2_aux = nullptr;
    }
    s.max_np = max_np;
  }
  if (max_nm > s.max_nm) {
    vpic_particle_mover_t *pm = nullptr;
    VH_CHECK(hipMalloc(&pm, sizeof(vpic_particle_mover_t) * max_nm));
    if (s.nm > 0) VH_CHECK(hipMemcpy(pm, s.pm, sizeof(vpic_particle_mover_t) * (size_t)s.nm, hipMemcpyDeviceToDevice));
    (void)hipFree(s.pm);
    s.pm = pm; s.max_nm = max_nm;
    VH_CHECK(hipMemcpy(reinterpret_cast<char *>(s.drain_k) + offsetof(DrainParams, pm), &pm, sizeof(pm), hipMemcpyHostToDevice));
    const int cap = (int)max_nm;
    VH_CHECK(hipMemcpy(reinterpret_cast<char *>(s.drain_k) + offsetof(DrainParams, max_nm), &cap, sizeof(cap), hipMemcpyHostToDevice));
  }
  return 0;
}

__global__ __launch_bounds__(256)
void tail_copy_back_kernel(ParticlesK dst, ParticlesK src, const int64_t *tsrc, const int64_t *t2src, int64_t *tdst, int64_t *t2dst, int n,
                           const int *__restrict__ n_live) {
  const int k = blockIdx.x * 256 + threadIdx.x;
  if (k >= n) return;
  if (k >= *n_live) { record_set_cell(dst.r, k, -1); return; }
  dst.r[k] = src.r[k];
  dst.ux[k] = src.ux[k]; dst.uy[k] = src.uy[k]; dst.uz[k] = src.uz[k]; dst.q[k] = src.q[k];
  if (tsrc) { tdst[k] = tsrc[k]; t2dst[k] = t2src[k]; }
}

int k_tail_sort(Engine *e, Species &s) {
  s.tail_sorted = false;
  if (!s.tile_valid || s.np <= s.n_sorted) return 0;
  const TileK tk = make_tile_k(e->gk);
  const int n1 = tk.ntiles * TILE_CELLS + 1;
  const int n = (int)(s.np - s.n_sorted), nb = (n1 + 1023) / 1024;
  if (!s.ttail) VH_CHECK(hipMalloc(&s.ttail, sizeof(int) * s.tpart_count));
  if (!s.aux.r && alloc_particles(s.aux, s.max_np)) return 1;
  if (s.has_tags && !s.tag_aux) {
    VH_CHECK(hipMalloc(&s.tag_aux, sizeof(int64_t) * s.max_np));
    VH_CHECK(hipMalloc(&s.tag2_aux, sizeof(int64_t) * s.max_np));
  }
  const ParticlesK in = offset_particles(s.p, s.n_sorted), out = offset_particles(s.aux, s.n_sorted);
  const int64_t *tin = s.has_tags ? s.tag + s.n_sorted : nullptr, *t2in = s.has_tags ? s.tag2 + s.n_sorted : nullptr;
  int64_t *tout = s.has_tags ? s.tag_aux + s.n_sorted : nullptr, *t2out = s.has_tags ? s.tag2_aux + s.n_sorted : nullptr;
  VH_CHECK(hipMemsetAsync(e->sort_next, 0, sizeof(int) * n1, e->stream));
  hipLaunchKernelGGL(sort_count_kernel<true>, dim3((n + 255) / 256), dim3(256), 0, e->stream, (const float4 *)in.r, n, e->sort_next, tk);
  hipLaunchKernelGGL(scan_local_kernel, dim3(nb), dim3(256), 0, e->stream, e->sort_next, s.ttail, e->scan_tmp, n1);
  hipLaunchKernelGGL(scan_blocks_kernel, dim3(1), dim3(256), 0, e->stream, e->scan_tmp, nb);
  hipLaunchKernelGGL(scan_add_kernel, dim3(nb), dim3(256), 0, e->stream, s.ttail, e->sort_next, e->scan_tmp, n1);
  hipLaunchKernelGGL(sort_scatter_kernel<true>, dim3((n + 255) / 256), dim3(256), 0, e->stream, in, out, tin, t2in, tout, t2out, n, e->sort_next, tk);
  hipLaunchKernelGGL(tail_copy_back_kernel, dim3((n + 255) / 256), dim3(256), 0, e->stream, in, out, (const int64_t *)tout, (const int64_t *)t2out,
                     s.has_tags ? s.tag + s.n_sorted : nullptr, s.has_tags ? s.tag2 + s.n_sorted : nullptr, n,
                     (const int *)(s.ttail + (size_t)tk.ntiles * TILE_CELLS));
  VH_CHECK(hipGetLastError());
  s.tail_sorted = true;
  return 0;
}


// ... 129 lines not shown
int k_accumulate_rhob(Engine *e, const vpic_particle_t *host, int64_t n, float q_scale) {
  for (int64_t first = 0; first < n; first += CHUNK) {
    const int m = (int)((n - first < CHUNK) ? n - first : CHUNK);
    if (ensure_stage(e, sizeof(vpic_particle_t) * (size_t)m)) return 1;
    VH_CHECK(hipMemcpyAsync(e->stage, host + first, sizeof(vpic_particle_t) * (size_t)m, hipMemcpyHostToDevice, e->stream));
    hipLaunchKernelGGL(accumulate_rhob_list_kernel, dim3((m + 255) / 256), dim3(256), 0, e->stream, e->f.c[F_RHOB],
                       (const vpic_particle_t *)e->stage, m, q_scale, e->gk, e->grid.rdx, e->grid.rdy, e->grid.rdz);
    VH_CHECK(hipGetLastError());
    VH_CHECK(hipStreamSynchronize(e->stream));
  }
  return 0;
}

template <bool WALLS>
__global__ __launch_bounds__(256)
void boundary_classify_kernel(ParticlesK p, const vpic_particle_mover_t *__restrict__ pm, int nm, int np,
                              int sp_id, GridK g, float rdx, float rdy, float rdz, float *__restrict__ rhob,
                              SendTable send, int *__restrict__ counters, int *__restrict__ tail_flag,
                              int *__restrict__ holes, RefluxK rk, float gdx, float gdy, float gdz,
                              const int *__restrict__ nm_dev = nullptr, const int *__restrict__ np_dev = nullptr,
                              RetryMover *__restrict__ retry = nullptr, const WallK wk = WallK{}) {
  const int t = blockIdx.x * 256 + threadIdx.x;
  if (nm_dev) {
    const int have = *nm_dev;
    if (have > nm && t == 0) atomicOr(&counters[C_OVER], 1);
    nm = min(have, nm); np = *np_dev;
  }
  if (t >= nm) return;
  const vpic_particle_mover_t m = pm[t];
  bool parked = false;
  const int idx = m.i, new_np = np - nm;
  const float4 rec = p.r[idx];
  const float dx = rec.x, dy = rec.y, dz = rec.z;
  const float ux = p.ux[idx], uy = p.uy[idx], uz = p.uz[idx], q = p.q[idx];
  const int pi = record_cell(rec);
  bool absorb = true;
  int abs_face = 6, abs_flags = 0;
  for (int face = 0; face < 6; face++) {
    const int axis = face % 3, hi = face >= 3;
    const float d = axis == 0 ? dx : axis == 1 ? dy : dz, u = axis == 0 ? ux : axis == 1 ? uy : uz;
    const bool cond = hi ? ((d == 1.f) & (u > 0)) : ((d == -1.f) & (u < 0));
    if (!cond) continue;
    const int code = pbc_of(g, face);
    if (WALLS && code <= VPIC_ABSORB_PARTICLES) {
      abs_flags = wall_flags_of(wk, code);
      if (abs_flags || code == VPIC_ABSORB_PARTICLES) { abs_face = face; break; }
    }
    if (code == VPIC_ABSORB_PARTICLES) break;
    if (code < VPIC_ABSORB_PARTICLES) {
      int h = -1;
      for (int k = 0; k < rk.n; k++) if (rk.code[k] == code) h = k;
      if (h < 0) continue;
      float u[3];
      if (rk.draws && idx < rk.draws_n) {
        u[0] = rk.ut_para[h] * (hi ? -1.41421356237309504880f : 1.41421356237309504880f) * sqrtf(-logf(rk.draws[3 * idx]));
        u[1] = rk.ut_perp[h] * rk.draws[3 * idx + 1];
        u[2] = rk.ut_perp[h] * rk.draws[3 * idx + 2];
      } else {
        const unsigned c0 = mix32(rk.seed ^ mix32(rk.call * 0x9e3779b9u + (unsigned)sp_id) ^ mix32((unsigned)t * 3u + 1u));
        const float r0 = unit_open(mix32(c0)), r1 = unit_open(mix32(c0 + 0x68bc21ebu)), r2 = unit_open(mix32(c0 + 0x02e5be93u));
        const float rad = sqrtf(-2.f * logf(r1));
        u[0] = rk.ut_para[h] * (hi ? -1.41421356237309504880f : 1.41421356237309504880f) * sqrtf(-logf(r0));
        u[1] = rk.ut_perp[h] * rad * cosf(6.28318530717958647692f * r2);
        u[2] = rk.ut_perp[h] * rad * sinf(6.28318530717958647692f * r2);
      }
      const float nux = axis == 0 ? u[0] : axis == 1 ? u[2] : u[1];
      const float nuy = axis == 0 ? u[1] : axis == 1 ? u[0] : u[2];
// ... 69 lines not shown
  __syncthreads();
  for (int base = 0; base < left; base += blockDim.x) {
    const int t = base + threadIdx.x;
    vpic_particle_mover_t m; m.dispx = m.dispy = m.dispz = 0; m.i = 0;
    if (t < left) m = pm[nm_cap + t];
    __syncthreads();
    if (t < left) pm[t] = m;
    __syncthreads();
  }
  if (threadIdx.x == 0) *nm_dev = left;
}
__global__ void exchange_unpark_kernel(int *__restrict__ counters, const RetryMover *__restrict__ retry, const SpeciesTable *__restrict__ Tp) {
  const int n = min(counters[C_RETRY], RETRY_CAP);
  for (int t = threadIdx.x; t < n; t += blockDim.x) {
    const int s = retry[t].sp;
    const int slot = atomicAdd(&counters[C_NMS + s], 1);
    if (slot < Tp->max_nm[s]) Tp->pm[s][slot] = retry[t].m; else atomicOr(&counters[C_OVER], 8);
  }
  __syncthreads();
  if (threadIdx.x == 0) counters[C_RETRY] = 0;
}
__global__ void exchange_header_kernel(int *__restrict__ counters, int *const *__restrict__ hdr, const int *__restrict__ cap) {
  const int f = threadIdx.x;
  if (f >= 6) return;
  if (hdr[f]) { hdr[f][0] = min(counters[C_SEND + f], cap[f]); hdr[f][1] = counters[C_SEND + f]; hdr[f][2] = 0; hdr[f][3] = 0; }
  counters[C_SEND + f] = 0;
}
__global__ void boundary_backfill_kernel(ParticlesK p, int64_t *tag, int64_t *tag2, const int *__restrict__ counters,
                                         const int *__restrict__ holes, const int *__restrict__ fills) {
  const int t = blockIdx.x * blockDim.x + threadIdx.x;
  if (t >= counters[C_HOLES]) return;
  const int d = holes[t], s = fills[t];
  p.r[d] = p.r[s];
  p.ux[d] = p.ux[s]; p.uy[d] = p.uy[s]; p.uz[d] = p.uz[s]; p.q[d] = p.q[s];
  if (tag) { tag[d] = tag[s]; tag2[d] = tag2[s]; }
}

static WallK wall_k(const Engine *e, size_t k) {
  WallK wk = {};
  if (!e->wall_ready) return wk;
  wk.n = (int)e->walls.size();
  for (int h = 0; h < wk.n; h++) { wk.code[h] = e->walls[h].code; wk.flags[h] = e->walls[h].flags; }
  wk.quantum[0] = e->wall_quantum[0]; wk.quantum[1] = e->wall_quantum[1];
  wk.row = e->wall_table + k; wk.row_stride = MAX_SPECIES;
  wk.rec = e->wall_rec; wk.rec_cap = e->wall_rec_cap; wk.cursor = e->wall_cursor;
  const Species &s = e->species[k];
  wk.tag = s.has_tags ? s.tag : nullptr; wk.tag2 = s.has_tags ? s.tag2 : nullptr;
  return wk;
}

static int ensure_lists(Engine *e, int64_t n) {
  if (n <= e->list_cap) return 0;
  if (e->hole_list) { (void)hipFree(e->hole_list); (void)hipFree(e->fill_list); (void)hipFree(e->tail_flag); }
  const int64_t cap = n + (n >> 2) + 1024;
  VH_CHECK(hipMalloc(&e->hole_list, sizeof(int) * cap));
  VH_CHECK(hipMalloc(&e->fill_list, sizeof(int) * cap));
  VH_CHECK(hipMalloc(&e->tail_flag, sizeof(int) * cap));
  e->list_cap = cap; e->tail_clean = false;
  return 0;
}

static int ensure_send(Engine *e, int64_t n) {
  if (n <= e->send_cap) return 0;
  const int64_t cap = n + (n >> 2) + 1024;
  for (int f = 0; f < 6; f++) {
    const int code = e->gk.pbc[f];
    if (!(code >= 0 && code != e->gk.rank)) continue;
// ... 76 lines not shown
  const int s = inj.sp_id;
  if (s < 0 || s >= Tp->n) return;
  int idx = 0;
  {
    const int lane = threadIdx.x & 63;
    unsigned long long todo = __ballot(true);
    while (todo) {
      const int lead = __ffsll((long long)todo) - 1;
      const int s0 = __builtin_amdgcn_readlane(s, lead);
      const unsigned long long m = __ballot(s == s0) & todo;
      if (s == s0) {
        int base = 0;
        if (lane == lead) base = atomicAdd(&counters[C_NP + s0], __popcll(m));
        base = __builtin_amdgcn_readlane(base, lead);
        idx = base + __popcll(m & ((1ull << lane) - 1ull));
      }
      const unsigned long long charged = __ballot(s == s0 && inj.q != 0.f);
      if (charged && lane == lead) atomicOr(&counters[C_CHARGED], 1 << s0);
      todo &= ~m;
    }
  }
  if (idx >= Tp->max_np[s]) { atomicOr(&counters[C_OVER], 4); return; }
  {
    const unsigned qb = __float_as_uint(fabsf(inj.q));
    unsigned *top = reinterpret_cast<unsigned *>(counters + C_QTOP + s);
    if (qb < 0x7f800000u && qb > *top) atomicMax(top, qb);
  }
  float dx = inj.dx, dy = inj.dy, dz = inj.dz, ux = inj.ux, uy = inj.uy, uz = inj.uz;
  float mx = inj.dispx, my = inj.dispy, mz = inj.dispz;
  int pi = inj.i;
  const int stuck = move_p_lane<false>(dx, dy, dz, pi, ux, uy, uz, inj.q, mx, my, mz, nullptr, g_acc, NO_WINDOW, g, false, det_scale);
  const ParticlesK p = Tp->p[s];
  p.r[idx] = make_record(dx, dy, dz, pi);
  p.ux[idx] = ux; p.uy[idx] = uy; p.uz[idx] = uz; p.q[idx] = inj.q;
  if (Tp->tag[s]) { Tp->tag[s][idx] = tags ? tags[2 * t] : 0; Tp->tag2[s][idx] = tags ? tags[2 * t + 1] : 0; }

  if (stuck) {
    const int slot = atomicAdd(&counters[C_NMS + s], 1);
    if (slot >= Tp->max_nm[s]) atomicOr(&counters[C_OVER], 8);
    if (slot < Tp->max_nm[s]) {
      vpic_particle_mover_t m; m.dispx = mx; m.dispy = my; m.dispz = mz; m.i = idx;
      Tp->pm[s][slot] = m;
    }
  }
}

__global__ __launch_bounds__(256)
void injector_q_top_kernel(const vpic_particle_injector_t *__restrict__ in, int n, const int *__restrict__ n_dev, int n_species,
                           unsigned *__restrict__ top) {
  if (n_dev) n = min(*n_dev, n);
  unsigned best = 0;
  for (int t = blockIdx.x * 256 + threadIdx.x; t < n; t += gridDim.x * 256) {
    const unsigned qb = __float_as_uint(fabsf(in[t].q));
    if (in[t].sp_id >= 0 && in[t].sp_id < n_species && qb < 0x7f800000u && qb > best) best = qb;
  }
  if (best) atomicMax(top, best);
}
static int prepare_det_for_arrivals(Engine *e, const vpic_particle_injector_t *inj, int n, const int *n_dev) {
  bool known = e->acc_scale != 0 || e->acc_qref > 0;
  for (auto &s : e->species) known = known || s.q_max > 0;
  if (known) return acc_prepare_det(e);
  unsigned *top = reinterpret_cast<unsigned *>(e->counters + C_QMSG), bits = 0;
  VH_CHECK(hipMemsetAsync(top, 0, sizeof(unsigned), e->stream));
  hipLaunchKernelGGL(injector_q_top_kernel, dim3(std::min((n + 255) / 256, 64)), dim3(256), 0, e->stream, inj, n, n_dev,
                     (int)e->species.size(), top);
  VH_CHECK(hipGetLastError());
  VH_CHECK(hipMemcpyAsync(e->host_counters + C_QMSG, top, sizeof(unsigned), hipMemcpyDeviceToHost, e->stream));
// ... 290 lines not shown
```

old-vpic_amd/csrc/push.hip:

```cpp
#include "push_device.h"
#include "record_offsets.h"
#include <cstdlib>
#include <cstring>
#include <cstddef>
#include <vector>
#include <algorithm>

namespace vpichip {

struct PushParams {
  float qdt_2mc, cdt_dx, cdt_dy, cdt_dz;
  int np;
  int iters;
  int sy, sz;
  int idx_base;
  unsigned *crossed;
  const int *tpart, *ttail; int ntx, nty, ntiles, n_sorted; unsigned mul_sy, sh_sy, mul_sz, sh_sz;
  const int *tile_list; int n_launch, tail_chunks;
  int nx, ny, nz;
  int follow;
  double acc_scale;
  int *hist; int ntz;
  ParticlesK out; int *next;
  int stage;
#ifdef VPIC_HIP_ABLATION
  int ablate;
#endif
};

#define SEG_STEP(v, flag, CTRL)                                                                   \
  asm volatile("v_fmac_f32_dpp %0, %0, %1 " CTRL : "+v"(v) : "v"(flag))
#define SEG_STEP12(a, flag, CTRL)                                                                 \
  do {                                                                                            \
    asm volatile("s_nop 1");                                                                      \
    SEG_STEP(a[0], flag, CTRL); SEG_STEP(a[1], flag, CTRL); SEG_STEP(a[2], flag, CTRL);           \
    SEG_STEP(a[3], flag, CTRL); SEG_STEP(a[4], flag, CTRL); SEG_STEP(a[5], flag, CTRL);           \
    SEG_STEP(a[6], flag, CTRL); SEG_STEP(a[7], flag, CTRL); SEG_STEP(a[8], flag, CTRL);           \
    SEG_STEP(a[9], flag, CTRL); SEG_STEP(a[10], flag, CTRL); SEG_STEP(a[11], flag, CTRL);         \
  } while (0)

typedef float rec4 __attribute__((ext_vector_type(4)));
__device__ __forceinline__ rec4 ldr(const float4 *base, unsigned off) { return *reinterpret_cast<const rec4 *>(reinterpret_cast<const char *>(base) + off); }
__device__ __forceinline__ void str(float4 *base, unsigned off, float x, float y, float z, int i) {
  rec4 v; v.x = x; v.y = y; v.z = z; v.w = __int_as_float(i);
  *reinterpret_cast<rec4 *>(reinterpret_cast<char *>(base) + off) = v;
}
__device__ __forceinline__ void str_nt(float4 *base, unsigned off, float x, float y, float z, int i) {
  rec4 v; v.x = x; v.y = y; v.z = z; v.w = __int_as_float(i);
  __builtin_nontemporal_store(v, reinterpret_cast<rec4 *>(reinterpret_cast<char *>(base) + off));
}
__device__ __forceinline__ rec4 *rec_at(float4 *base, unsigned dst) {
  return reinterpret_cast<rec4 *>(reinterpret_cast<char *>(base) + ((uint64_t)dst << RECORD_SHIFT));
}
__device__ __forceinline__ int ldcell(const float4 *base, unsigned off) { return __float_as_int(*reinterpret_cast<const float *>(reinterpret_cast<const char *>(base) + off + 12u)); }
__device__ __forceinline__ float ldf(const float *base, unsigned off) { return *reinterpret_cast<const float *>(reinterpret_cast<const char *>(base) + off); }
__device__ __forceinline__ void stf(float *base, unsigned off, float v) { *reinterpret_cast<float *>(reinterpret_cast<char *>(base) + off) = v; }
__device__ __forceinline__ void stf_nt(float *base, unsigned off, float v) { __builtin_nontemporal_store(v, reinterpret_cast<float *>(reinterpret_cast<char *>(base) + off)); }


__device__ __forceinline__ int in_vgpr(int s) { int v; asm volatile("v_mov_b32 %0, %1" : "=v"(v) : "s"(s)); return v; }

__device__ __forceinline__ int mbcnt64(unsigned long long m) {
  return (int)__builtin_amdgcn_mbcnt_hi((unsigned)(m >> 32), __builtin_amdgcn_mbcnt_lo((unsigned)m, 0u));
}

#ifndef VPIC_HIP_MAX_KEYS
#define VPIC_HIP_MAX_KEYS 12
#endif
constexpr int MAX_KEYS = VPIC_HIP_MAX_KEYS;

__device__ __forceinline__ int group_lanes_by_key(int key, int lane) {
  unsigned long long todo = ~0ull;
  int dest = lane, offset = 0;
  for (int it = 0; todo && it < MAX_KEYS; ++it) {
    const int lead = __ffsll((long long)todo) - 1;
    const int k0 = __builtin_amdgcn_readlane(key, lead);
    const bool mine = (key == k0);
    const unsigned long long m = __ballot(mine);
    if (mine) dest = offset + mbcnt64(m);
    offset += __popcll(m);
    todo &= ~m;
  }
  if ((todo >> lane) & 1ull) dest = offset + mbcnt64(todo);
  return dest;
}

constexpr int MISS_CAP = 5;
struct MissList { int key[MISS_CAP]; float v[MISS_CAP][12]; int total; };

__device__ __forceinline__ void flush_misses(MissList *ml, int &n_miss, float *g_acc, int lane) {
// ... 167 lines not shown
struct StagePark { int base[STAGE_CAP], qb[STAGE_CAP]; unsigned cm_lo[STAGE_CAP], cm_hi[STAGE_CAP], act_lo[STAGE_CAP], act_hi[STAGE_CAP]; };
constexpr int STAGED_BIT = 31;
struct Straggler { float4 pos_i, disp_idx; float q; bool live; unsigned long long again; };

template <bool FAST, class W, bool HIST = false, bool STAGE = false, bool WIDE = false>
__device__ __forceinline__ int drain_wave(const ParticlesK &p, const int rel, WaveQueue *mq, const int n_mq,
                                          const int lane, typename W::acc_t *s_acc, float *g_acc, const int wbase,
                                          const DrainParams *dp, const int ablate, const int max_round, const int idx_base,
                                          MissList *ml, int &n_miss, const double det_scale = 0, const HistK *hk = nullptr, Straggler *sg = nullptr) {
  if (ablate & 64) return 0;
  typedef int int8v __attribute__((ext_vector_type(8)));
  typedef int int4v __attribute__((ext_vector_type(4)));
  int8v d0, d1; int4v d2;
  asm volatile("s_load_dwordx8 %0, %3, 0x0\n\ts_load_dwordx8 %1, %3, 0x20\n\ts_load_dwordx4 %2, %3, 0x40\n\ts_waitcnt lgkmcnt(0)"
               : "=&s"(d0), "=&s"(d1), "=&s"(d2) : "s"(dp));
  static_assert(offsetof(DrainParams, pbc) == 0x20 && offsetof(DrainParams, pm) == 0x40 && sizeof(DrainParams) == 0x50, "DrainParams layout");
  const int gnx = d0[0], gny = d0[1], gnz = d0[2], gsy = d0[3], gsz = d0[4], grank = d0[5], max_nm = d0[6];
  const unsigned mul_sz = (unsigned)d0[7], mul_sy = (unsigned)d1[6], sh_sz = (unsigned)d1[7] >> 8, sh_sy = (unsigned)d1[7] & 255u;
  const int pb0 = d1[0], pb1 = d1[1], pb2 = d1[2], pb3 = d1[3], pb4 = d1[4], pb5 = d1[5];
  const TileDiv td = {mul_sy, sh_sy, mul_sz, sh_sz, det_scale};
  typedef __attribute__((address_space(1))) vpic_particle_mover_t *global_mover_ptr;
  typedef __attribute__((address_space(1))) int *global_int_ptr;
  const global_mover_ptr pm = (global_mover_ptr)(((unsigned long long)(unsigned)d2[1] << 32) | (unsigned)d2[0]);
  const global_int_ptr nm_counter = (global_int_ptr)(((unsigned long long)(unsigned)d2[3] << 32) | (unsigned)d2[2]);
  int n_again = 0;
  for (int base = 0; base < n_mq; base += 64) {
    const int k = base + lane;
    bool live = k < n_mq;
    const int kq = live ? k : 0;
    const float4 c0 = mq->pos_i[kq], c2 = mq->disp_idx[kq];
    const float q = mq->q[kq];
    vpic_particle_mover_t m; m.dispx = c2.x; m.dispy = c2.y; m.dispz = c2.z; m.i = __float_as_int(c2.w);
    const int idx = m.i;
    const unsigned o4 = word_offset(idx, rel);
    float dx = c0.x, dy = c0.y, dz = c0.z;
    int flips = (__float_as_int(c0.w) >> FLIP_SHIFT) & 7;
    const bool staged = STAGE && live && (__float_as_int(c0.w) >> STAGED_BIT) & 1;
    int pi = live ? (__float_as_int(c0.w) & ((1 << FLIP_SHIFT) - 1)) : -1, cx = 0, cy = 0, cz = 0;
    if (live) {
      cz = (int)(__umulhi((unsigned)pi, mul_sz) >> sh_sz); const int rem = pi - cz * gsz;
      cy = (int)(__umulhi((unsigned)rem, mul_sy) >> sh_sy); cx = rem - cy * gsy;
    }
    const bool mine = live;
    bool stuck = false;
    const bool w0 = pb0 != grank, w1 = pb1 != grank, w2 = pb2 != grank, w3 = pb3 != grank, w4 = pb4 != grank, w5 = pb5 != grank;
    const bool r0 = pb0 == VPIC_REFLECT_PARTICLES, r1 = pb1 == VPIC_REFLECT_PARTICLES, r2 = pb2 == VPIC_REFLECT_PARTICLES,
               r3 = pb3 == VPIC_REFLECT_PARTICLES, r4 = pb4 == VPIC_REFLECT_PARTICLES, r5 = pb5 == VPIC_REFLECT_PARTICLES;
    for (int round = 0; round < max_round && __ballot(live); round++) {
      const bool up0 = m.dispx > 0, up1 = m.dispy > 0, up2 = m.dispz > 0;
      const float s_dir0 = up0 ? 1.f : -1.f, s_dir1 = up1 ? 1.f : -1.f, s_dir2 = up2 ? 1.f : -1.f;
      const float big = (float)3.4e38;
      float t0, t1, t2;
      if (FAST) {
        t0 = (fabsf(m.dispx) < 7.9e-31f) ? big : (s_dir0 - dx) * fast_rcp(m.dispx);
        t1 = (fabsf(m.dispy) < 7.9e-31f) ? big : (s_dir1 - dy) * fast_rcp(m.dispy);
        t2 = (fabsf(m.dispz) < 7.9e-31f) ? big : (s_dir2 - dz) * fast_rcp(m.dispz);
      } else {
        t0 = (m.dispx == 0) ? big : div_normal(s_dir0 - dx, m.dispx);
        t1 = (m.dispy == 0) ? big : div_normal(s_dir1 - dy, m.dispy);
        t2 = (m.dispz == 0) ? big : div_normal(s_dir2 - dz, m.dispz);
      }
      float v3 = 2.f;
      const bool lt0 = t0 < v3; v3 = lt0 ? t0 : v3;
      const bool lt1 = t1 < v3; v3 = lt1 ? t1 : v3;
      const bool lt2 = t2 < v3; v3 = lt2 ? t2 : v3;
      const bool ty2 = lt2, ty1 = lt1 && !lt2, ty0 = lt0 && !lt1 && !lt2;
      const bool moved_on = lt0 || lt1 || lt2;
// ... 43 lines not shown
        if (__ballot(fin)) {
          float b[12];
          mover_streak12<W>(b, q, dx + m.dispx, dy + m.dispy, dz + m.dispz, m.dispx, m.dispy, m.dispz);
          const int fkey = fin ? pi : -1;
          if (fin) {
            dx += m.dispx + m.dispx; dy += m.dispy + m.dispy; dz += m.dispz + m.dispz;
            live = false;
          }
          if (ablate & 32) {}
          else run_deposit<W::DRAIN_BLOCK, W>(b, fkey, lane, s_acc, g_acc, wbase, gsy, gsz, td, ml, n_miss);
        }
      }
    }
    const unsigned long long again = __ballot(live);
    if (STAGE) {
      sg->live = live; sg->again = again; sg->q = q;
      sg->pos_i = make_float4(dx, dy, dz, __int_as_float(pi | (flips << FLIP_SHIFT)));
      sg->disp_idx = make_float4(m.dispx, m.dispy, m.dispz, __int_as_float(idx));
      if (staged) mq->pos_i[k] = make_float4(dx, dy, dz, __int_as_float(live ? -1 : pi));
    } else
    if (live) {
      const int d = mbcnt64(again);
      mq->pos_i[d] = make_float4(dx, dy, dz, __int_as_float(pi | (flips << FLIP_SHIFT)));
      mq->disp_idx[d] = make_float4(m.dispx, m.dispy, m.dispz, __int_as_float(idx));
      mq->q[d] = q;
    }
    n_again = __popcll(again);
    if (mine && !live) {
#ifdef VPIC_HIP_ABLATION
      if (ablate & 256) {} else
#endif
      if (!staged) {
        if (WIDE) { rec4 v; v.x = dx; v.y = dy; v.z = dz; v.w = __int_as_float(pi); __builtin_nontemporal_store(v, rec_at(p.r, (unsigned)idx)); }
        else str_nt(p.r, o4 << 2, dx, dy, dz, pi);
      }
      if (HIST) hist_count<W>(*hk, pi, wbase, gsy, gsz, td);
      if (flips) {
        asm volatile("s_waitcnt vmcnt(0)" ::: "memory");
        if (flips & 1) stf(p.ux, o4, -ldf(p.ux, o4));
        if (flips & 2) stf(p.uy, o4, -ldf(p.uy, o4));
        if (flips & 4) stf(p.uz, o4, -ldf(p.uz, o4));
      }
      if (stuck) {
        const int gs = __hip_atomic_fetch_add(nm_counter, 1, __ATOMIC_RELAXED, __HIP_MEMORY_SCOPE_AGENT);
        if (gs < max_nm) { pm[gs].dispx = m.dispx; pm[gs].dispy = m.dispy; pm[gs].dispz = m.dispz; pm[gs].i = m.i + idx_base; }
      }
    }
  }
  return n_again;
}

constexpr int TAIL_CHUNK = 1024;

template <bool CHARGELESS = false, bool FAST = false, int WIN = 0, bool HIST = false, bool SORT = false>
#ifndef VPIC_HIP_PUSH_VGPRS
#define VPIC_HIP_PUSH_VGPRS 80
#endif
__global__ __launch_bounds__(PUSH_THREADS) __attribute__((amdgpu_num_vgpr(VPIC_HIP_PUSH_VGPRS)))
void advance_p_kernel(ParticlesK p, const float4 *__restrict__ fi, float *__restrict__ g_acc,
                      const DrainParams *__restrict__ dp, const PushParams P) {
  typedef Window<WIN> W;
  typedef typename W::acc_t acc_t;
  constexpr bool TILE = W::TILE;
  constexpr bool DET = is_det<W>::value;
  constexpr bool UNORDERED = WIN == 3 || WIN == 5 || WIN == 6;
  constexpr int WX = W::WX, NSLOT_PAD = W::NSLOT_PAD;
  __shared__ acc_t s_acc[12 * NSLOT_PAD];
  __shared__ WaveQueue s_mq[WAVES];
  __shared__ MissList s_miss[WAVES];
  __shared__ int s_wbase;
  __shared__ unsigned s_cnt[HIST ? (NSLOT_PAD + 1) / 2 : SORT ? NSLOT_PAD : 1];
  constexpr bool STAGE = (WIN == 3 || CHARGELESS) && !HIST && !SORT;
  __shared__ StagePark s_park[STAGE ? WAVES : 1];
  static_assert(!HIST || WIN == 2, "the histogram of the next sort is taken in tile order, by cell");
// ... 189 lines not shown
        }
      }
    }
    __syncthreads();
    for (int t = tid; t < W::NSLOT; t += PUSH_THREADS) {
      const unsigned c = s_cnt[t];
      if (c) {
        const int lx = t % WX, lyz = t / WX, ly = lyz % WX, lz = lyz / WX;
        s_cnt[t] = (unsigned)__hip_atomic_fetch_add((global_int_ptr)P.next + sort_key<true>(wbase + lx + gsy * ly + gsz * lz, hk.tk), (int)c,
                                                    __ATOMIC_RELAXED, __HIP_MEMORY_SCOPE_AGENT);
      }
    }
    __syncthreads();
  }

#pragma unroll 1
  for (int seg = 0; seg < (TILE ? 2 : 1); seg++) {
  const int sfirst = seg ? first2 : first, slast = seg ? last2 : last;
  if (TILE && sfirst >= slast) continue;
  const int sspan = TILE ? ((slast - sfirst + 64 * WAVES - 1) / (64 * WAVES)) * 64 : wave_span;
  const int wave_passes = TILE ? sspan >> 6 : P.iters;
  constexpr int PASS_STRIDE = 64;
  const int wave_first = sfirst + wave * sspan;
  const int wave_last = TILE ? min(slast, wave_first + sspan) : slast;
  if (TILE && !SORT && seg && (n_mq > 0 || (STAGE && n_pend > 0))) {
    __builtin_amdgcn_fence(__ATOMIC_RELEASE, "workgroup");
    if constexpr (STAGE) n_mq = drain_release(true);
    else n_mq = drain_wave<FAST, W, HIST>(pw, rel, mq, n_mq, lane, s_acc, g_acc, wbase, dp, ablate, 1 << 30, P.idx_base, ml, n_miss, td.scale, &hk);
    __builtin_amdgcn_fence(__ATOMIC_ACQ_REL, "workgroup");
  }
  pw = offset_particles(p, sfirst);
  rel = SORT ? 0 : sfirst;
  const int vrel_max = TILE ? in_vgpr(P.np - 1 - sfirst) : P.np - 1 - sfirst;
  rec4 r_rec;
  float r_ux, r_uy, r_uz, r_q;
  {
    const unsigned k4 = (unsigned)min(wave_first - sfirst + lane, P.np - 1 - sfirst) << 2;
    r_rec = ldr(pw.r, k4 << 2);
    r_ux = ldf(pw.ux, k4); r_uy = ldf(pw.uy, k4); r_uz = ldf(pw.uz, k4); r_q = ldf(pw.q, k4);
  }

#pragma unroll 1
  for (int it = 0; it < wave_passes; it++) {
    const int base = wave_first + it * PASS_STRIDE;
    if (base >= wave_last) break;
    int idx = base + lane, key = (base + lane < wave_last) ? __float_as_int(r_rec.w) : -1;
    float dx = r_rec.x, dy = r_rec.y, dz = r_rec.z, ux = r_ux, uy = r_uy, uz = r_uz, q = r_q;
    const int kk = key < 0 ? 0x7fffffff : key;
    const int kprev = __builtin_amdgcn_update_dpp((int)0x80000000, kk, 0x138 , 0xf, 0xf, false);
    if (!UNORDERED && !(ablate & 16) && __ballot(kk < kprev)) {
      const int dest = group_lanes_by_key(key, lane);
      if (__ballot(dest != lane)) {
        const int a4 = dest << 2;
        idx = base + __builtin_amdgcn_ds_permute(a4, lane);
        key = __builtin_amdgcn_ds_permute(a4, key);
        dx = __int_as_float(__builtin_amdgcn_ds_permute(a4, __float_as_int(dx)));
        dy = __int_as_float(__builtin_amdgcn_ds_permute(a4, __float_as_int(dy)));
        dz = __int_as_float(__builtin_amdgcn_ds_permute(a4, __float_as_int(dz)));
        ux = __int_as_float(__builtin_amdgcn_ds_permute(a4, __float_as_int(ux)));
        uy = __int_as_float(__builtin_amdgcn_ds_permute(a4, __float_as_int(uy)));
        uz = __int_as_float(__builtin_amdgcn_ds_permute(a4, __float_as_int(uz)));
        q = __int_as_float(__builtin_amdgcn_ds_permute(a4, __float_as_int(q)));
      }
    }
    int dst = idx, sort_slot = -2, sort_b = 0, sort_head = 0;
    if (SORT) {
      typedef __attribute__((address_space(1))) int *global_int_ptr;
      const int slot = key >= 0 ? slot_of<W>(key, wbase, vsy, vsz, vtd) : -1;
      sort_slot = slot;
      const int kprev2 = __builtin_amdgcn_update_dpp(-2, key, 0x138 , 0xf, 0xf, false);
      const unsigned long long heads = __ballot(kprev2 != key);
      const unsigned long long upto = (2ull << lane) - 1ull;
      const int head = 63 - __clzll((long long)(heads & upto));
      const unsigned long long above = heads & ~upto;
      const int run_end = above ? __ffsll((long long)above) - 1 : 64;
      const bool reserves = lane == head && key >= 0;
      int b = 0;
      if (reserves && slot >= 0) b = (int)atomicAdd(&s_cnt[slot], (unsigned)(run_end - lane));
      if (__ballot(reserves && slot < 0)) {
        if (reserves && slot < 0)
          b = __hip_atomic_fetch_add((global_int_ptr)P.next + sort_key<true>(key, hk.tk), run_end - lane, __ATOMIC_RELAXED, __HIP_MEMORY_SCOPE_AGENT);
      }
      sort_b = b; sort_head = head;
    }
    const float4 *f = reinterpret_cast<const float4 *>(reinterpret_cast<const char *>(fi) + (unsigned)((ablate & 4) ? 0 : max(key, 0)) * 80u);
    const float4 fe_x = f[0], fe_y = f[1], fe_z = f[2], fb0 = f[3];
    const float2 fb1 = *reinterpret_cast<const float2 *>(f + 4);
    __builtin_amdgcn_sched_barrier(0);
    {
      const int k = base - sfirst + ((it + 1 < wave_passes) ? PASS_STRIDE : 0) + lane;
      const unsigned k4 = (unsigned)min(k, vrel_max) << 2;
      r_rec = ldr(pw.r, k4 << 2);
      r_ux = ldf(pw.ux, k4); r_uy = ldf(pw.uy, k4); r_uz = ldf(pw.uz, k4); r_q = ldf(pw.q, k4);
    }
    __builtin_amdgcn_sched_barrier(0);
    const bool active = key >= 0;
    float a[12];
    bool crosser;
    float sux, suy, suz;
    float spx = 0.f, spy = 0.f, spz = 0.f;
    {
      const unsigned o4 = word_offset(idx, sfirst);
      float v0, v1, v2, v3, v4, v5;
      if (FAST) {
        const float hax = qdt_2mc * __builtin_fmaf(dz, __builtin_fmaf(dy, fe_x.w, fe_x.z), __builtin_fmaf(dy, fe_x.y, fe_x.x));
        const float hay = qdt_2mc * __builtin_fmaf(dx, __builtin_fmaf(dz, fe_y.w, fe_y.z), __builtin_fmaf(dz, fe_y.y, fe_y.x));
        const float haz = qdt_2mc * __builtin_fmaf(dy, __builtin_fmaf(dx, fe_z.w, fe_z.z), __builtin_fmaf(dx, fe_z.y, fe_z.x));
        const float cbx = __builtin_fmaf(dx, fb0.y, fb0.x), cby = __builtin_fmaf(dy, fb0.w, fb0.z), cbz = __builtin_fmaf(dz, fb1.y, fb1.x);
        ux += hax; uy += hay; uz += haz;
        v0 = qdt_2mc * fast_rsq(__builtin_fmaf(ux, ux, __builtin_fmaf(uy, uy, __builtin_fmaf(uz, uz, one))));
        v1 = __builtin_fmaf(cbx, cbx, __builtin_fmaf(cby, cby, cbz * cbz));
        v2 = (v0 * v0) * v1;
        v3 = v0 * __builtin_fmaf(v2, __builtin_fmaf(v2, two_fifteenths, one_third), one);
        v4 = (v3 + v3) * fast_rcp(__builtin_fmaf(v1, v3 * v3, one));
        v0 = __builtin_fmaf(v3, __builtin_fmaf(uy, cbz, -(uz * cby)), ux);
        v1 = __builtin_fmaf(v3, __builtin_fmaf(uz, cbx, -(ux * cbz)), uy);
        v2 = __builtin_fmaf(v3, __builtin_fmaf(ux, cby, -(uy * cbx)), uz);
        ux = __builtin_fmaf(v4, __builtin_fmaf(v1, cbz, -(v2 * cby)), ux);
        uy = __builtin_fmaf(v4, __builtin_fmaf(v2, cbx, -(v0 * cbz)), uy);
        uz = __builtin_fmaf(v4, __builtin_fmaf(v0, cby, -(v1 * cbx)), uz);
        ux += hax; uy += hay; uz += haz;
      } else {
        const float hax = qdt_2mc * ((fe_x.x + dy * fe_x.y) + dz * (fe_x.z + dy * fe_x.w));
        const float hay = qdt_2mc * ((fe_y.x + dz * fe_y.y) + dx * (fe_y.z + dz * fe_y.w));
        const float haz = qdt_2mc * ((fe_z.x + dx * fe_z.y) + dy * (fe_z.z + dx * fe_z.w));
        const float cbx = fb0.x + dx * fb0.y;
        const float cby = fb0.z + dy * fb0.w;
        const float cbz = fb1.x + dz * fb1.y;
        ux += hax; uy += hay; uz += haz;
        v0 = div_normal(qdt_2mc, sqrt_normal(one + (ux * ux + (uy * uy + uz * uz))));
        v1 = cbx * cbx + (cby * cby + cbz * cbz);
        v2 = (v0 * v0) * v1;
        v3 = v0 * (one + v2 * (one_third + v2 * two_fifteenths));
        v4 = div_normal(v3, one + v1 * (v3 * v3));
        v4 += v4;
        v0 = ux + v3 * (uy * cbz - uz * cby);
        v1 = uy + v3 * (uz * cbx - ux * cbz);
        v2 = uz + v3 * (ux * cby - uy * cbx);
        ux += v4 * (v1 * cbz - v2 * cby);
        uy += v4 * (v2 * cbx - v0 * cbz);
        uz += v4 * (v0 * cby - v1 * cbx);
        ux += hax; uy += hay; uz += haz;
      }
      sux = ux; suy = uy; suz = uz;
      if (FAST) v0 = fast_rsq(__builtin_fmaf(ux, ux, __builtin_fmaf(uy, uy, __builtin_fmaf(uz, uz, one))));
      else v0 = div_normal(one, sqrt_normal(one + (ux * ux + (uy * uy + uz * uz))));
      ux *= cdt_dx; uy *= cdt_dy; uz *= cdt_dz;
      ux *= v0; uy *= v0; uz *= v0;
      v0 = dx + ux; v1 = dy + uy; v2 = dz + uz;
      v3 = v0 + ux; v4 = v1 + uy; v5 = v2 + uz;
      const bool incell = (ablate & 2) || fmaxf(fmaxf(fabsf(v3), fabsf(v4)), fabsf(v5)) <= one;
      crosser = active && !incell;
      if (SORT) {
        dst = __shfl(sort_b, sort_head) + (lane - sort_head);
        if (active) {
          const unsigned d4 = (unsigned)dst << 2;
          stf(P.out.ux, d4, sux); stf(P.out.uy, d4, suy); stf(P.out.uz, d4, suz);
          rec4 v; v.x = incell ? v3 : dx; v.y = incell ? v4 : dy; v.z = incell ? v5 : dz; v.w = __int_as_float(key);
          *rec_at(P.out.r, (unsigned)dst) = v;
          stf(P.out.q, d4, q);
        }
      } else
      if (STAGE && stage) {
        if (!TILE || active) { stf(pw.ux, o4, sux); stf(pw.uy, o4, suy); stf(pw.uz, o4, suz); }
        spx = incell ? v3 : dx; spy = incell ? v4 : dy; spz = incell ? v5 : dz;
      } else
      if ((!TILE || active) && !(ablate & 128)) {
        stf_nt(pw.ux, o4, sux); stf_nt(pw.uy, o4, suy); stf_nt(pw.uz, o4, suz);
        str(pw.r, o4 << 2, incell ? v3 : dx, incell ? v4 : dy, incell ? v5 : dz, key);
      }
      if (!CHARGELESS && !(ablate & 1)) {
        const float qd = (incell && active) ? q : 0.f;
        if constexpr (is_det<W>::value) streak12(a, qd, v0, v1, v2, ux, uy, uz, qd * ux * uy * uz * one_third);
        else streak12_moments(a, qd, v0, v1, v2, ux, uy, uz);
      } else {
#pragma unroll
        for (int k = 0; k < 12; k++) a[k] = 0.f;
      }
    }
    if constexpr (WIN == 4) run_deposit_fixed<16, W>(a, key, lane, s_acc, g_acc, wbase, gsy, gsz, td, ml, n_miss);
    else
    if (!CHARGELESS) run_deposit<UNORDERED ? 1 : TILE ? TILE_MAIN_BLOCK : MAIN_BLOCK, W>(a, (UNORDERED && crosser) ? -1 : key, lane, s_acc, g_acc, wbase, vsy, vsz, vtd, ml, n_miss,
                                                                                            HIST ? &hk : nullptr, active && !crosser, SORT ? sort_slot : -2);
    {
      const unsigned long long cm = __ballot(crosser);
      const int cnt = __popcll(cm);
      n_crossed += cnt;
      if constexpr (STAGE) {
        int phase = (n_mq + cnt > MQW) ? 0 : 1, attempt = 0;
#pragma unroll 1
        for (;;) {
          if (phase == 1) {
            if (crosser) {
              const int d = n_mq + mbcnt64(cm);
              mq->pos_i[d] = make_float4(dx, dy, dz, __int_as_float(stage ? (key | (1 << STAGED_BIT)) : key));
              mq->disp_idx[d] = make_float4(ux, uy, uz, __int_as_float(idx));
              mq->q[d] = q;
            }
            if (stage) {
              if (n_pend == 0) { st0x = spx; st0y = spy; st0z = spz; st0i = key; } else { st1x = spx; st1y = spy; st1z = spz; st1i = key; }
              const unsigned long long act = __ballot(!TILE || active);
              if (lane == 0) {
// ... 306 lines not shown
    }
    if (!s.phase_pending) {
      hipLaunchKernelGGL(publish_counter_kernel, dim3(1), dim3(256), 0, e->stream, s.crossed_host_dev, s.crossed_dev, (unsigned)(s.pol.n_cycle - (fuse ? 1 : 0)),
                         fuse ? ~0ull : (unsigned long long)e->knobs.follow_from * (unsigned long long)make_tile_k(e->gk).ntiles);
      if (e->time_kernels) { (void)hipEventRecord(s.ev[1], e->stream); s.push_timed = true; }
    }
    VH_CHECK(hipGetLastError());
  }
  if (!e->can_strand || async) { s.partition_valid = false; return 0; }
  VH_CHECK(hipMemcpyAsync(e->host_counters, s.nm_dev, sizeof(int), hipMemcpyDeviceToHost, e->stream));
  VH_CHECK(hipStreamSynchronize(e->stream));
  int64_t nm = e->host_counters[0];
  if (nm > s.max_nm) {
    fprintf(stderr, "vpic_hip: advance_p ran out of storage for %lld movers\n", (long long)(nm - s.max_nm));
    nm = s.max_nm;
  }
  s.nm = nm;
  s.partition_valid = false;
  return 0;
}

__global__ __launch_bounds__(256)
void energy_p_kernel(ParticlesK p, const float4 *__restrict__ fi, double *__restrict__ partial,
                     float qdt_2mc, int np) {
  __shared__ double s_sum[4];
  double en = 0;
  const float one = 1.f;
  for (long long idx = (long long)blockIdx.x * 256 + threadIdx.x; idx < np; idx += (long long)gridDim.x * 256) {
    const float4 rec = p.r[idx];
    if (record_cell(rec) < 0) continue;
    const float dx = rec.x, dy = rec.y, dz = rec.z;
    const float4 *f = fi + (size_t)record_cell(rec) * 5;
    const float4 fe_x = f[0], fe_y = f[1], fe_z = f[2];
    float v0 = p.ux[idx] + qdt_2mc * ((fe_x.x + dy * fe_x.y) + dz * (fe_x.z + dy * fe_x.w));
    float v1 = p.uy[idx] + qdt_2mc * ((fe_y.x + dz * fe_y.y) + dx * (fe_y.z + dz * fe_y.w));
    float v2 = p.uz[idx] + qdt_2mc * ((fe_z.x + dx * fe_z.y) + dy * (fe_z.z + dx * fe_z.w));
    v0 = v0 * v0 + v1 * v1 + v2 * v2;
    v0 /= sqrtf(one + v0) + one;
    en += (double)v0 * (double)p.q[idx];
  }
  for (int off = 32; off; off >>= 1) en += __shfl_down(en, off);
  if ((threadIdx.x & 63) == 0) s_sum[threadIdx.x >> 6] = en;
  __syncthreads();
  if (threadIdx.x == 0) partial[blockIdx.x] = (s_sum[0] + s_sum[1]) + (s_sum[2] + s_sum[3]);
}

int k_energy_p(Engine *e, Species &s, double *energy) {
  const vpic_hip_grid_t &g = e->grid;
  const float qdt_2mc = (float)(0.5 * s.q_m * g.dt / g.cvac);
  const int nb = (int)e->dsum_count;
  hipLaunchKernelGGL(energy_p_kernel, dim3(nb), dim3(256), 0, e->stream, s.p,
                     reinterpret_cast<const float4 *>(e->fi), e->dsum, qdt_2mc, (int)s.np);
  VH_CHECK(hipGetLastError());
  VH_CHECK(hipMemcpyAsync(e->host_dsum, e->dsum, sizeof(double) * nb, hipMemcpyDeviceToHost, e->stream));
  VH_CHECK(hipStreamSynchronize(e->stream));
  double sum = 0;
  for (int k = 0; k < nb; k++) sum += e->host_dsum[k];
  *energy = (double)g.cvac * (double)g.cvac * sum / (double)s.q_m;
  return 0;
}

}

namespace vpichip {
template <bool UNCENTER>
__global__ __launch_bounds__(256)
void center_p_kernel(ParticlesK p, const float4 *__restrict__ fi, float args_qdt_2mc, int np) {
  const int idx = blockIdx.x * 256 + threadIdx.x;
  if (idx >= np) return;
  const float4 rec = p.r[idx];
  if (record_cell(rec) < 0) return;
  const float qdt_2mc = UNCENTER ? -args_qdt_2mc : args_qdt_2mc;
  const float qdt_4mc = UNCENTER ? (float)(-0.5 * args_qdt_2mc) : (float)(0.5 * args_qdt_2mc);
  const float one = 1.f, one_third = 1. / 3., two_fifteenths = 2. / 15.;
  const float dx = rec.x, dy = rec.y, dz = rec.z;
  const float4 *f = fi + (size_t)record_cell(rec) * 5;
  const float4 fe_x = f[0], fe_y = f[1], fe_z = f[2], fb0 = f[3];
  const float2 fb1 = *reinterpret_cast<const float2 *>(f + 4);
  const float hax = qdt_2mc * ((fe_x.x + dy * fe_x.y) + dz * (fe_x.z + dy * fe_x.w));
  const float hay = qdt_2mc * ((fe_y.x + dz * fe_y.y) + dx * (fe_y.z + dz * fe_y.w));
  const float haz = qdt_2mc * ((fe_z.x + dx * fe_z.y) + dy * (fe_z.z + dx * fe_z.w));
  const float cbx = fb0.x + dx * fb0.y, cby = fb0.z + dy * fb0.w, cbz = fb1.x + dz * fb1.y;
  float ux = p.ux[idx], uy = p.uy[idx], uz = p.uz[idx], v0, v1, v2, v3, v4;
  if (!UNCENTER) { ux += hax; uy += hay; uz += haz; }
  v0 = qdt_4mc / sqrtf(one + (ux * ux + (uy * uy + uz * uz)));
  v1 = cbx * cbx + (cby * cby + cbz * cbz);
  v2 = (v0 * v0) * v1;
  v3 = v0 * (one + v2 * (one_third + v2 * two_fifteenths));
  v4 = v3 / (one + v1 * (v3 * v3));
  v4 += v4;
  v0 = ux + v3 * (uy * cbz - uz * cby);
  v1 = uy + v3 * (uz * cbx - ux * cbz);
  v2 = uz + v3 * (ux * cby - uy * cbx);
  ux += v4 * (v1 * cbz - v2 * cby);
  uy += v4 * (v2 * cbx - v0 * cbz);
  uz += v4 * (v0 * cby - v1 * cbx);
  if (UNCENTER) { ux += hax; uy += hay; uz += haz; }
  p.ux[idx] = ux; p.uy[idx] = uy; p.uz[idx] = uz;
}

int k_center_p(Engine *e, Species &s, bool uncenter) {
  if (s.np == 0) return 0;
  const vpic_hip_grid_t &g = e->grid;
  const float qdt_2mc = (float)(0.5 * s.q_m * g.dt / g.cvac);
  const unsigned nb = (unsigned)((s.np + 255) / 256);
  if (uncenter)
    hipLaunchKernelGGL(center_p_kernel<true>, dim3(nb), dim3(256), 0, e->stream, s.p, reinterpret_cast<const float4 *>(e->fi), qdt_2mc, (int)s.np);
  else
    hipLaunchKernelGGL(center_p_kernel<false>, dim3(nb), dim3(256), 0, e->stream, s.p, reinterpret_cast<const float4 *>(e->fi), qdt_2mc, (int)s.np);
  VH_CHECK(hipGetLastError());
  return 0;
}
}

namespace vpichip {
__global__ __launch_bounds__(256)
void accumulate_hydro_p_kernel(float *__restrict__ h0, ParticlesK p, const float4 *__restrict__ fi, int np, HydroConsts hc, int sy, int sz) {
  const int idx = blockIdx.x * 256 + threadIdx.x;
  if (idx >= np) return;
  const float4 rec = p.r[idx];
  const int ii = record_cell(rec);
  if (ii < 0) return;
  HydroP P;
  hydro_particle(rec.x, rec.y, rec.z, p.ux[idx], p.uy[idx], p.uz[idx], p.q[idx], load_interp(fi, ii), hc, P);
  float *h = h0 + (size_t)ii * HYDRO_STRIDE;
#pragma unroll
  for (int n = 0; n < 8; n++) {
    float *m = h + HYDRO_STRIDE * (size_t)((n & 1) + ((n >> 1) & 1) * sy + (n >> 2) * sz), c[HYDRO_MOMENTS];
    hydro_node(P, P.w[n], hc.mc_q, c);
#pragma unroll
    for (int k = 0; k < HYDRO_MOMENTS; k++) atomicAdd(m + k, c[k]);
  }
}

__global__ __launch_bounds__(256)
void accumulate_hydro_cells_kernel(float *__restrict__ h0, ParticlesK p, const float4 *__restrict__ fi,
                                   const int *__restrict__ partition, int nv, HydroConsts hc, int sy, int sz) {
  const int ii = blockIdx.x * 256 + threadIdx.x;
  if (ii >= nv) return;
  const int first = partition[ii], last = partition[ii + 1];
  if (first >= last) return;
  const InterpK f = load_interp(fi, ii);
  float S[8][HYDRO_MOMENTS];
#pragma unroll
  for (int n = 0; n < 8; n++)
#pragma unroll
    for (int k = 0; k < HYDRO_MOMENTS; k++) S[n][k] = 0.f;
#pragma unroll 1
  for (int idx = first; idx < last; idx++) {
    HydroP P;
    const float4 rec = p.r[idx];
    hydro_particle(rec.x, rec.y, rec.z, p.ux[idx], p.uy[idx], p.uz[idx], p.q[idx], f, hc, P);
#pragma unroll
    for (int n = 0; n < 8; n++) {
      float c[HYDRO_MOMENTS];
      hydro_node(P, P.w[n], hc.mc_q, c);
#pragma unroll
      for (int k = 0; k < HYDRO_MOMENTS; k++) S[n][k] += c[k];
    }
  }
  float *h = h0 + (size_t)ii * HYDRO_STRIDE;
#pragma unroll
  for (int n = 0; n < 8; n++) {
    float *m = h + HYDRO_STRIDE * (size_t)((n & 1) + ((n >> 1) & 1) * sy + (n >> 2) * sz);
#pragma unroll
    for (int k = 0; k < HYDRO_MOMENTS; k++) atomicAdd(m + k, S[n][k]);
  }
}

HydroConsts hydro_consts(const Engine *e, const Species &s) {
  const vpic_hip_grid_t &g = e->grid;
  HydroConsts hc;
  hc.qdt_2mc = 0.5 * s.q_m * g.dt / g.cvac;
  hc.qdt_4mc2 = 0.25 * s.q_m * g.dt / (g.cvac * g.cvac);
  hc.c = g.cvac;
  hc.r8V = 0.125 * g.rdx * g.rdy * g.rdz;
  hc.mc_q = g.cvac / s.q_m;
  return hc;
}

int k_hydro_p_untiled(Engine *e, Species &s, bool by_cell) {
  const HydroConsts hc = hydro_consts(e, s);
  if (by_cell) {
    if (!s.partition_valid && k_sort_p(e, s)) return 1;
    hipLaunchKernelGGL(accumulate_hydro_cells_kernel, dim3((unsigned)((e->gk.nv + 255) / 256)), dim3(256), 0, e->stream,
// ... 11 lines not shown
```

old-vpic_amd/csrc/select.hip:

```cpp
#include "dist_coords.h"
#include <algorithm>

namespace vpichip {

constexpr int SEL_WAVES = 4;
constexpr int SEL_CHUNK = 2048;
constexpr int SEL_GROUPS = SEL_CHUNK / 64;
constexpr int SEL_PASSES = SEL_CHUNK / (64 * SEL_WAVES);
constexpr int SEL_MAX_BLOCKS = 4096;
static_assert(SEL_CHUNK % 256 == 0 && SEL_GROUPS <= 64, "a chunk is a multiple of 256 particles whose masks one wavefront scans");

template <bool MASKS, bool FIELDS>
__global__ __launch_bounds__(64 * SEL_WAVES)
void select_mark_kernel(ParticlesK p, const int64_t *__restrict__ tag, long long np, long long n_chunks, SelectK k, GridK g, TileK t,
                        unsigned long long *__restrict__ mask, unsigned *__restrict__ counts, unsigned long long *__restrict__ stats,
                        const vpic_interpolator_t *__restrict__ fi) {
  __shared__ unsigned s_kept[SEL_WAVES];
  const int lane = threadIdx.x & 63, wave = threadIdx.x >> 6;
  unsigned long long n_seen = 0;
  for (long long c = blockIdx.x; c < n_chunks; c += gridDim.x) {
    const long long first = c * SEL_CHUNK + threadIdx.x;
    unsigned n_kept = 0;
    DistRaw next = dist_load<FIELDS>(p, first, np, k.need), next2{};
    DistField f{}, f_next{};
// ... 73 lines not shown
                         const unsigned long long *__restrict__ offsets, const vpic_interpolator_t *__restrict__ fi,
                         long long cap, vpic_particle_t *__restrict__ out_p, float *__restrict__ out_f, long long *__restrict__ out_i) {
  __shared__ unsigned long long s_mask[SEL_GROUPS];
  __shared__ unsigned s_before[SEL_GROUPS];
  const int lane = threadIdx.x & 63, wave = threadIdx.x >> 6;
  for (long long c = blockIdx.x; c < n_chunks; c += gridDim.x) {
    const long long offset = (long long)offsets[c];
    if (counts[c] == 0 || offset >= cap) continue;
    if (wave == 0) {
      const unsigned long long m = lane < SEL_GROUPS ? mask[c * SEL_GROUPS + lane] : 0;
      const unsigned mine = (unsigned)__popcll(m);
      unsigned incl = mine;
#pragma unroll
      for (int d = 1; d < 64; d <<= 1) {
        const unsigned up = __shfl_up(incl, d);
        if (lane >= d) incl += up;
      }
      if (lane < SEL_GROUPS) { s_mask[lane] = m; s_before[lane] = incl - mine; }
    }
    __syncthreads();
    for (int pass = 0; pass < SEL_PASSES; pass++) {
      const int group = pass * SEL_WAVES + wave;
      const unsigned long long m = s_mask[group];
      if (!(m >> lane & 1ull)) continue;
      const long long dest = offset + s_before[group] + __popcll(m & ((1ull << lane) - 1ull));
      if (dest >= cap) continue;
      const long long idx = c * SEL_CHUNK + (long long)group * 64 + lane;
      const float4 pos = p.r[idx];
      const int voxel = record_cell(pos);
      const float dx = pos.x, dy = pos.y, dz = pos.z;
      if (out_p) {
        float4 *rec = reinterpret_cast<float4 *>(out_p + dest);
        rec[0] = make_float4(dx, dy, dz, __int_as_float(voxel));
        rec[1] = make_float4(p.ux[idx], p.uy[idx], p.uz[idx], p.q[idx]);
        const long long t1 = tag ? tag[idx] : 0, t2 = tag ? tag2[idx] : 0;
        *reinterpret_cast<ulonglong2 *>(rec + 2) = make_ulonglong2((unsigned long long)t1, (unsigned long long)t2);
      }
      if (out_f) {
        const float4 *q = reinterpret_cast<const float4 *>(fi + voxel);
        const float4 fx = q[0], fy = q[1], fz = q[2], fb = q[3];
        const float2 fc = *reinterpret_cast<const float2 *>(q + 4);
        float2 *o = reinterpret_cast<float2 *>(out_f + 6 * dest);
        o[0] = make_float2((fx.x + dy * fx.y) + dz * (fx.z + dy * fx.w), (fy.x + dz * fy.y) + dx * (fy.z + dz * fy.w));
        o[1] = make_float2((fz.x + dx * fz.y) + dy * (fz.z + dx * fz.w), fb.x + dx * fb.y);
        o[2] = make_float2(fb.z + dy * fb.w, fc.x + dz * fc.y);
      }
      if (out_i) out_i[dest] = idx;
    }
    __syncthreads();
  }
}

int k_species_select(Engine *e, Species &s, const vpic_hip_select_t &d, int64_t cap, bool want_p, bool want_f, bool want_i, bool count_only) {
  const SelectK k = make_select_k(d);
  const long long np = s.np, n_chunks = (np + SEL_CHUNK - 1) / SEL_CHUNK;
  const int64_t *tag = s.has_tags ? s.tag : nullptr;
  if (grow(e->sel_counts, e->sel_counts_n, (size_t)n_chunks) || grow(e->sel_offsets, e->sel_offsets_n, (size_t)n_chunks)) return 1;
  if (!count_only && grow(e->sel_mask, e->sel_mask_n, (size_t)n_chunks * SEL_GROUPS)) return 1;
  if (e->sel_stats.begin(e->stream)) return 1;
  const unsigned nb = (unsigned)std::min<long long>(n_chunks, SEL_MAX_BLOCKS);
  const TileK tk = make_tile_k(e->gk);
  if (n_chunks > 0) {
    auto mark = k.need & NEED_FIELD ? (count_only ? select_mark_kernel<false, true> : select_mark_kernel<true, true>)
                                    : (count_only ? select_mark_kernel<false, false> : select_mark_kernel<true, false>);
    hipLaunchKernelGGL(mark, dim3(nb), dim3(64 * SEL_WAVES), 0, e->stream, s.p, tag, np, n_chunks, k, e->gk, tk,
                       count_only ? nullptr : e->sel_mask, e->sel_counts, e->sel_stats.dev, (const vpic_interpolator_t *)e->fi);
    VH_CHECK(hipGetLastError());
// ... 24 lines not shown
```

old-vpic_amd/csrc/spectrum.hip:

```cpp
#include "engine.h"

namespace vpichip {

constexpr int SPEC_WAVES = 4;

struct SpectrumK {
  int n_lin, n_log, win;
  double d_lin, log_lo, d_log;
};


template <bool TILE>
__device__ __forceinline__ int voxel_of_key(int key, const GridK &g, const TileK &t) {
  if (!TILE) return key < g.nv ? key : -1;
  const int tile = key >> 6, c = key & 63;
  if (tile >= t.ntiles) return -1;
  const int tz = tile / (t.ntx * t.nty), r = tile - tz * (t.ntx * t.nty), ty = r / t.ntx, tx = r - ty * t.ntx;
  const int x = 4 * tx + (c & 3) + 1, y = 4 * ty + ((c >> 2) & 3) + 1, z = 4 * tz + (c >> 4) + 1;
  if (x > g.nx || y > g.ny || z > g.nz) return -1;
  return x + g.sy * y + g.sz * z;
}

template <bool TILE>
__device__ __forceinline__ void flush_window(unsigned *win, int base, const SpectrumK &k, const GridK &g, const TileK &t,
                                             unsigned *__restrict__ lin, int lane) {
  __builtin_amdgcn_fence(__ATOMIC_ACQ_REL, "wavefront");
  for (int slot = lane; slot < k.win; slot += 64) {
    const int voxel = voxel_of_key<TILE>(base + slot, g, t);
    for (int b = 0; b < k.n_lin; b++) {
      const unsigned c = win[slot * k.n_lin + b];
      if (c) {
        if (voxel >= 0) atomicAdd(lin + (size_t)b * g.nv + voxel, c);
        win[slot * k.n_lin + b] = 0;
      }
    }
  }
  __builtin_amdgcn_fence(__ATOMIC_ACQ_REL, "wavefront");
}

template <bool TILE>
__global__ __launch_bounds__(64 * SPEC_WAVES)
void energy_spectrum_kernel(const float4 *__restrict__ prec, const float *__restrict__ pux, const float *__restrict__ puy,
                            const float *__restrict__ puz, long long np, long long chunk, SpectrumK k, GridK g, TileK t,
                            unsigned *__restrict__ lin, unsigned long long *__restrict__ logc,
                            unsigned long long *__restrict__ stats) {
  extern __shared__ unsigned s_mem[];
  unsigned *s_log = s_mem;
  const int lane = threadIdx.x & 63, wave = threadIdx.x >> 6;
  unsigned *win = s_mem + k.n_log + wave * (k.win * k.n_lin);
  for (int j = threadIdx.x; j < k.n_log + SPEC_WAVES * k.win * k.n_lin; j += 64 * SPEC_WAVES) s_mem[j] = 0;
  __syncthreads();

  const long long w = (long long)blockIdx.x * SPEC_WAVES + wave;
  const long long begin = w * chunk, end = begin + chunk < np ? begin + chunk : np;
  SlideWindow w_state;
  unsigned long long n_seen = 0, n_miss = 0;
  for (long long at = begin; at < end; at += 64) {
    const long long idx = at + lane;
    const int voxel = idx < end ? record_cell(prec, idx) : -1;
    const bool live = voxel >= 0 && voxel < g.nv;
    n_seen += __popcll(__ballot(live));
    if (!__any(live)) continue;
    double ke = 0;
    if (live) {
      const float ux = pux[idx], uy = puy[idx], uz = puz[idx];
      const double gam2 = ((1.0 + (double)ux * (double)ux) + (double)uy * (double)uy) + (double)uz * (double)uz;
      ke = sqrt(gam2) - 1.0;
    }
    if (k.n_log > 0 && live) {
      const double x = (log10(ke) - k.log_lo) / k.d_log + 1.0;
      if (x > -1.0 && x < (double)k.n_log) atomicAdd(&s_log[(int)x], 1u);
    }
    if (k.n_lin > 0) {
      int band = 0, key = 0;
      bool pending = live;
      if (live) {
        const double q = ke / k.d_lin;
        band = q < (double)(k.n_lin - 1) ? (int)q : k.n_lin - 1;
        if (band < 0) band = 0;
        key = sort_key<TILE>(voxel, t);
        if (TILE) {
          int cx, cy, cz;
          voxel_cell(voxel, t, cx, cy, cz);
          if (cx < 1 || cx > g.nx || cy < 1 || cy > g.ny || cz < 1 || cz > g.nz) key = -1;
        }
      }
      if (k.win > 0)
        pending = window_add(w_state, win, k.win, k.n_lin, key, band, pending, lane,
          [&](unsigned long long left) {
            const int first = __builtin_amdgcn_readlane(key, __ffsll((long long)left) - 1);
            return TILE ? first & ~63 : first;
          },
          [&](int base) { flush_window<TILE>(win, base, k, g, t, lin, lane); });
      if (pending) atomicAdd(lin + (size_t)band * g.nv + voxel, 1u);
      n_miss += __popcll(__ballot(pending));
    }
  }
  if (k.n_lin > 0 && k.win > 0 && w_state.placed) flush_window<TILE>(win, w_state.base, k, g, t, lin, lane);
// ... 3 lines not shown
    if (s_log[j]) atomicAdd(&logc[j], (unsigned long long)s_log[j]);
}

__global__ __launch_bounds__(256)
void energy_bands_kernel(const unsigned *__restrict__ lin, float *__restrict__ bands, int n_lin, GridK g) {
  const int v = blockIdx.x * 256 + threadIdx.x;
  if (v >= g.nv) return;
  const int z = v / g.sz, r = v - z * g.sz, y = r / g.sy, x = r - y * g.sy;
  const int xs = min(max(x, 1), g.nx), ys = min(max(y, 1), g.ny), zs = min(max(z, 1), g.nz);
  const int src = xs + g.sy * ys + g.sz * zs;
  unsigned long long n = 0;
  for (int b = 0; b < n_lin; b++) n += lin[(size_t)b * g.nv + src];
  for (int b = 0; b < n_lin; b++)
    bands[(size_t)b * g.nv + v] = n ? (float)((double)lin[(size_t)b * g.nv + src] / (double)n) : 0.f;
}

int k_energy_spectrum(Engine *e, Species &s, const vpic_hip_spectrum_t &sp) {
  const size_t lin_words = (size_t)sp.n_lin * (size_t)e->gk.nv;
  if (!e->spec_log) VH_CHECK(hipMalloc((void **)&e->spec_log, VPIC_HIP_SPECTRUM_MAX_LOG * sizeof(unsigned long long)));
  if (!e->spec_log_host) VH_CHECK(hipHostMalloc((void **)&e->spec_log_host, VPIC_HIP_SPECTRUM_MAX_LOG * sizeof(unsigned long long), hipHostMallocDefault));
  size_t bands_words = e->spec_lin_words;
  if (grow(e->spec_lin, e->spec_lin_words, lin_words) || grow(e->spec_bands, bands_words, lin_words)) { e->spec_lin_words = 0; return 1; }
  if (e->spec_stats.begin(e->stream)) return 1;
  SpectrumK k{};
  k.n_lin = sp.n_lin; k.n_log = sp.n_log; k.d_lin = sp.d_lin; k.log_lo = sp.log_lo; k.d_log = sp.d_log;
  k.win = spectrum_window(sp.n_lin);
  if (lin_words) VH_CHECK(hipMemsetAsync(e->spec_lin, 0, lin_words * sizeof(unsigned), e->stream));
  if (sp.n_log) VH_CHECK(hipMemsetAsync(e->spec_log, 0, (size_t)sp.n_log * sizeof(unsigned long long), e->stream));
  if (s.np > 0) {
    const Chunks ch = plan_chunks(s.np, SPEC_WAVES);
    const size_t lds = sizeof(unsigned) * ((size_t)sp.n_log + (size_t)SPEC_WAVES * k.win * sp.n_lin);
    const TileK tk = make_tile_k(e->gk);
    auto kernel = s.tile_valid ? energy_spectrum_kernel<true> : energy_spectrum_kernel<false>;
    hipLaunchKernelGGL(kernel, dim3((unsigned)ch.groups), dim3(64 * SPEC_WAVES), lds, e->stream, (const float4 *)s.p.r, s.p.ux, s.p.uy, s.p.uz,
                       (long long)s.np, ch.chunk, k, e->gk, tk, e->spec_lin, e->spec_log, e->spec_stats.dev);
    VH_CHECK(hipGetLastError());
  }
  if (sp.n_log) VH_CHECK(hipMemcpyAsync(e->spec_log_host, e->spec_log, (size_t)sp.n_log * sizeof(unsigned long long), hipMemcpyDeviceToHost, e->stream));
  return e->spec_stats.read(e->stream);
}

int k_energy_bands(Engine *e, int n_lin) {
  hipLaunchKernelGGL(energy_bands_kernel, dim3((e->gk.nv + 255) / 256), dim3(256), 0, e->stream, e->spec_lin, e->spec_bands, n_lin, e->gk);
  VH_CHECK(hipGetLastError());
  return 0;
}

}
```

Baseline: 60.27 billion.

## Pack particle momenta and charge into one float4 array

Replaces the four separate ux/uy/uz/q float arrays with a single float4 momentum record per particle, and updates every kernel (push, sort, collide, moments, load, select, spectrum) to match. The push and sort kernels now issue one 16-byte load and store for momentum and charge instead of four scalar accesses, and the sort scatter moves whole float4 records instead of staging four float fields separately. The intent is fewer memory transactions and simpler scatter logic in the bandwidth-bound particle push and sort. Kernels that only need charge or only some components now read the full 16-byte record, and setting momenta from the host now goes through a staging buffer and an extra kernel.

```diff
diff --git a/old-vpic_amd/csrc/collide.hip b/old-vpic_amd/csrc/collide.hip
--- a/old-vpic_amd/csrc/collide.hip
+++ b/old-vpic_amd/csrc/collide.hip
@@ -12,7 +12,7 @@
 __device__ __forceinline__ float c_unit(unsigned r) { return ((float)(r >> 8) + 0.5f) * (1.f / 16777216.f); }
 
 struct CollideSpK {
-  float *ux, *uy, *uz; const float *q; const float4 *r; const int *starts;
+  float4 *u; const float4 *r; const int *starts;
   int order, np;
   float wq, f;
   unsigned id;
@@ -91,14 +91,15 @@
 template <int T>
 __device__ __forceinline__ void load_cell(const CollideSpK &s, const Slab &l, int lo, int n, unsigned c0) {
   for (int k = threadIdx.x; k < n; k += T) {
-    l.ux[k] = s.ux[lo + k]; l.uy[k] = s.uy[lo + k]; l.uz[k] = s.uz[lo + k];
-    l.w[k] = fabsf(s.q[lo + k]) * s.wq;
+    const float4 mom = s.u[lo + k];
+    l.ux[k] = mom.x; l.uy[k] = mom.y; l.uz[k] = mom.z;
+    l.w[k] = fabsf(mom.w) * s.wq;
     l.key[k] = c_mix32(c0 + (unsigned)k);
   }
 }
 template <int T>
 __device__ __forceinline__ void store_cell(const CollideSpK &s, const Slab &l, int lo, int n) {
-  for (int k = threadIdx.x; k < n; k += T) { s.ux[lo + k] = l.ux[k]; s.uy[lo + k] = l.uy[k]; s.uz[lo + k] = l.uz[k]; }
+  for (int k = threadIdx.x; k < n; k += T) s.u[lo + k] = make_float4(l.ux[k], l.uy[k], l.uz[k], record_charge(s.u, lo + k));
 }
 template <int T>
 __device__ __forceinline__ void rank_cell(const Slab &l, int n, unsigned c0) {
@@ -291,7 +292,7 @@
 }
 static CollideSpK species_k(const Species &s, const CollideSpecies &d, int id, float wq, float f) {
   CollideSpK k;
-  k.ux = s.p.ux; k.uy = s.p.uy; k.uz = s.p.uz; k.q = s.p.q; k.r = s.p.r;
+  k.u = s.p.u; k.r = s.p.r;
   k.order = s.np == 0 ? 0 : d.tile_valid ? 2 : 1;
   k.starts = k.order == 2 ? s.tpart : s.partition;
   k.np = (int)s.np; k.wq = wq; k.f = f; k.id = (unsigned)id;
diff --git a/old-vpic_amd/csrc/cool.hip b/old-vpic_amd/csrc/cool.hip
--- a/old-vpic_amd/csrc/cool.hip
+++ b/old-vpic_amd/csrc/cool.hip
@@ -51,7 +51,7 @@
         const float fx = (float)nx, fy = (float)ny, fz = (float)nz;
         if (__float_as_uint(fx) != __float_as_uint(r.ux) || __float_as_uint(fy) != __float_as_uint(r.uy) ||
             __float_as_uint(fz) != __float_as_uint(r.uz)) n_changed++;
-        if (!DRY) { p.ux[idx] = fx; p.uy[idx] = fy; p.uz[idx] = fz; }
+        if (!DRY) p.u[idx] = make_float4(fx, fy, fz, q);
         const double wx = (double)fx, wy = (double)fy, wz = (double)fz;
         const double u2n = (wx * wx + wy * wy) + wz * wz, g1 = sqrt(1.0 + u2n);
         const double val = (double)fabsf(q) * ((u2 - u2n) / (g + g1));
diff --git a/old-vpic_amd/csrc/dist_coords.h b/old-vpic_amd/csrc/dist_coords.h
--- a/old-vpic_amd/csrc/dist_coords.h
+++ b/old-vpic_amd/csrc/dist_coords.h
@@ -49,9 +49,10 @@
   if (idx < end) {
     const float4 rec = p.r[idx];
     r.voxel = record_cell(rec); r.dx = rec.x; r.dy = rec.y; r.dz = rec.z;
-    if (u || (need & (NEED_KE | 1u << VPIC_HIP_COORD_UX))) r.ux = p.ux[idx];
-    if (u || (need & (NEED_KE | 1u << VPIC_HIP_COORD_UY))) r.uy = p.uy[idx];
-    if (u || (need & (NEED_KE | 1u << VPIC_HIP_COORD_UZ))) r.uz = p.uz[idx];
+    if (u || (need & (NEED_KE | 1u << VPIC_HIP_COORD_UX | 1u << VPIC_HIP_COORD_UY | 1u << VPIC_HIP_COORD_UZ))) {
+      const float *m = reinterpret_cast<const float *>(p.u + idx);
+      r.ux = m[0]; r.uy = m[1]; r.uz = m[2];
+    }
   }
   return r;
 }
@@ -129,7 +130,7 @@
 struct DistExtra { double q, edotv, epar_vpar; };
 
 __device__ __forceinline__ float dist_load_q(const ParticlesK &p, long long idx, long long end, unsigned vneed) {
-  return (vneed & VAL_Q) && idx < end ? p.q[idx] : 0.f;
+  return (vneed & VAL_Q) && idx < end ? record_charge(p.u, idx) : 0.f;
 }
 
 template <bool FIELDS>
diff --git a/old-vpic_amd/csrc/engine.h b/old-vpic_amd/csrc/engine.h
--- a/old-vpic_amd/csrc/engine.h
+++ b/old-vpic_amd/csrc/engine.h
@@ -36,7 +36,7 @@
 
 struct ParticlesK {
   float4 *r;
-  float *ux, *uy, *uz, *q;
+  float4 *u;
 };
 __host__ __device__ __forceinline__ float4 make_record(float dx, float dy, float dz, int i) {
   union { int i; float f; } w; w.i = i;
@@ -45,9 +45,10 @@
 __device__ __forceinline__ int record_cell(const float4 *r, long long k) { return __float_as_int(r[k].w); }
 __device__ __forceinline__ int record_cell(const float4 &v) { return __float_as_int(v.w); }
 __device__ __forceinline__ void record_set_cell(float4 *r, long long k, int i) { r[k].w = __int_as_float(i); }
+__device__ __forceinline__ float record_charge(const float4 *u, long long k) { return u[k].w; }
 __host__ __device__ __forceinline__ ParticlesK offset_particles(const ParticlesK &p, int64_t at) {
   ParticlesK o = p;
-  o.r += at; o.ux += at; o.uy += at; o.uz += at; o.q += at;
+  o.r += at; o.u += at;
   return o;
 }
 
diff --git a/old-vpic_amd/csrc/engine.hip b/old-vpic_amd/csrc/engine.hip
--- a/old-vpic_amd/csrc/engine.hip
+++ b/old-vpic_amd/csrc/engine.hip
@@ -159,8 +159,15 @@
 
 void free_particles(ParticlesK &p) {
   (void)hipFree(p.r);
-  (void)hipFree(p.ux); (void)hipFree(p.uy); (void)hipFree(p.uz); (void)hipFree(p.q);
+  (void)hipFree(p.u);
   p = ParticlesK{};
+}
+
+__global__ __launch_bounds__(256) void set_momenta_kernel(float4 *__restrict__ u, const float *__restrict__ src, int64_t n) {
+  const int64_t k = (int64_t)blockIdx.x * 256 + threadIdx.x;
+  if (k >= n) return;
+  float *m = reinterpret_cast<float *>(u + k);
+  m[0] = src[k]; m[1] = src[n + k]; m[2] = src[2 * n + k];
 }
 
 static void destroy(Engine *e) {
@@ -592,8 +599,14 @@
   Species &s = e->species[sp];
   if (!ux || !uy || !uz || n != s.np) VH_FAIL("Bad momenta: %lld, the species' extent is %lld", (long long)n, (long long)s.np);
   if (n == 0) return 0;
-  if (copy_in(e, s.p.ux, ux, sizeof(float) * (size_t)n) || copy_in(e, s.p.uy, uy, sizeof(float) * (size_t)n)) return 1;
-  return copy_in(e, s.p.uz, uz, sizeof(float) * (size_t)n);
+  const size_t bytes = sizeof(float) * (size_t)n;
+  if (ensure_stage(e, 3 * bytes)) return 1;
+  if (copy_in(e, e->stage, ux, bytes) || copy_in(e, e->stage + bytes, uy, bytes) || copy_in(e, e->stage + 2 * bytes, uz, bytes)) return 1;
+  hipLaunchKernelGGL(vpichip::set_momenta_kernel, dim3((unsigned)((n + 255) / 256)), dim3(256), 0, e->stream, s.p.u,
+                     reinterpret_cast<const float *>(e->stage), n);
+  VH_CHECK(hipGetLastError());
+  VH_CHECK(hipStreamSynchronize(e->stream));
+  return 0;
 }
 int vpic_hip_species_get_tile_partition(vpic_hip_engine_t *e, int sp, int32_t *tpart, int64_t *count) {
   ENGINE(e); SPECIES(e, sp);
diff --git a/old-vpic_amd/csrc/fields.hip b/old-vpic_amd/csrc/fields.hip
--- a/old-vpic_amd/csrc/fields.hip
+++ b/old-vpic_amd/csrc/fields.hip
@@ -755,7 +755,7 @@
   const float4 rec = p.r[idx];
   if (record_cell(rec) < 0) return;
   float w[8];
-  node_weights(rec.x, rec.y, rec.z, p.q[idx], r8V, w);
+  node_weights(rec.x, rec.y, rec.z, record_charge(p.u, idx), r8V, w);
   float *r = rhof + record_cell(rec);
   atomicAdd(r, w[0]); atomicAdd(r + 1, w[1]); atomicAdd(r + sy, w[2]); atomicAdd(r + sy + 1, w[3]);
   atomicAdd(r + sz, w[4]); atomicAdd(r + sz + 1, w[5]); atomicAdd(r + sz + sy, w[6]); atomicAdd(r + sz + sy + 1, w[7]);
@@ -772,7 +772,7 @@
   for (int idx = first; idx < last; idx++) {
     float w[8];
     const float4 rec = p.r[idx];
-    node_weights(rec.x, rec.y, rec.z, p.q[idx], r8V, w);
+    node_weights(rec.x, rec.y, rec.z, record_charge(p.u, idx), r8V, w);
     s0 += w[0]; s1 += w[1]; s2 += w[2]; s3 += w[3]; s4 += w[4]; s5 += w[5]; s6 += w[6]; s7 += w[7];
   }
   float *r = rhof + v;
diff --git a/old-vpic_amd/csrc/load.hip b/old-vpic_amd/csrc/load.hip
--- a/old-vpic_amd/csrc/load.hip
+++ b/old-vpic_amd/csrc/load.hip
@@ -83,7 +83,7 @@
   const float n[3] = {d[3], d[4], d[5]};
   load_momentum(uth, ud, n, d[6], k.flip != 0, u);
   p.r[m] = make_record(load_offset(d[0]), load_offset(d[1]), load_offset(d[2]), v);
-  p.ux[m] = u[0]; p.uy[m] = u[1]; p.uz[m] = u[2]; p.q[m] = k.q[at];
+  p.u[m] = make_float4(u[0], u[1], u[2], k.q[at]);
   if (tags) { tag[m] = tags == 1 ? k.tag0 + m : 0; tag2[m] = 0; }
 }
 
diff --git a/old-vpic_amd/csrc/moments.hip b/old-vpic_amd/csrc/moments.hip
--- a/old-vpic_amd/csrc/moments.hip
+++ b/old-vpic_amd/csrc/moments.hip
@@ -62,7 +62,8 @@
     static_assert(NM == HYDRO_MOMENTS, "a selection is for the hydro moments");
     constexpr bool FIELDS = SEL == MOM_SEL_FIELD;
     if (K.sel.use_tag && !select_tag_ok(K.sel.s, K.tag ? K.tag[idx] : 0)) return;
-    const DistRaw r{voxel, rec.x, rec.y, rec.z, K.p.ux[idx], K.p.uy[idx], K.p.uz[idx]};
+    const float4 mom = K.p.u[idx];
+    const DistRaw r{voxel, rec.x, rec.y, rec.z, mom.x, mom.y, mom.z};
     InterpK f;
     if (FIELDS) f = load_interp(K.fi, voxel);
     if (K.sel.s.n_sel > 0) {
@@ -73,13 +74,14 @@
     }
     if (!FIELDS) f = load_interp(K.fi, voxel);
     n.live++;
-    hydro_particle(r.dx, r.dy, r.dz, r.ux, r.uy, r.uz, K.p.q[idx], f, K.h, P);
+    hydro_particle(r.dx, r.dy, r.dz, r.ux, r.uy, r.uz, mom.w, f, K.h, P);
   } else {
     n.live++;
-    if constexpr (NM == HYDRO_MOMENTS)
-      hydro_particle(rec.x, rec.y, rec.z, K.p.ux[idx], K.p.uy[idx], K.p.uz[idx], K.p.q[idx], load_interp(K.fi, voxel), K.h, P);
-    else
-      node_weights(rec.x, rec.y, rec.z, K.p.q[idx], K.h.r8V, P.w);
+    if constexpr (NM == HYDRO_MOMENTS) {
+      const float4 mom = K.p.u[idx];
+      hydro_particle(rec.x, rec.y, rec.z, mom.x, mom.y, mom.z, mom.w, load_interp(K.fi, voxel), K.h, P);
+    } else
+      node_weights(rec.x, rec.y, rec.z, record_charge(K.p.u, idx), K.h.r8V, P.w);
   }
   bool inside = false;
   int slot0 = 0;
diff --git a/old-vpic_amd/csrc/particles.hip b/old-vpic_amd/csrc/particles.hip
--- a/old-vpic_amd/csrc/particles.hip
+++ b/old-vpic_amd/csrc/particles.hip
@@ -14,7 +14,7 @@
   const vpic_particle_t s = src[t];
   const int64_t k = first + t;
   p.r[k] = make_record(s.dx, s.dy, s.dz, s.i);
-  p.ux[k] = s.ux; p.uy[k] = s.uy; p.uz[k] = s.uz; p.q[k] = s.q;
+  p.u[k] = make_float4(s.ux, s.uy, s.uz, s.q);
   if (tag) { tag[k] = s.tag; tag2[k] = s.tag2; }
 }
 __global__ void particles_to_aos_kernel(ParticlesK p, const int64_t *tag, const int64_t *tag2,
@@ -25,7 +25,8 @@
   vpic_particle_t s;
   const float4 rec = p.r[k];
   s.dx = rec.x; s.dy = rec.y; s.dz = rec.z; s.i = record_cell(rec);
-  s.ux = p.ux[k]; s.uy = p.uy[k]; s.uz = p.uz[k]; s.q = p.q[k];
+  const float4 mom = p.u[k];
+  s.ux = mom.x; s.uy = mom.y; s.uz = mom.z; s.q = mom.w;
   s.tag = tag ? tag[k] : 0; s.tag2 = tag ? tag2[k] : 0;
   dst[t] = s;
 }
@@ -111,10 +112,7 @@
                          (cx + 1) + g.sy * (cy + 1) + g.sz * (cz + 1));
   const float r1 = sqrtf(-2.f * logf(u01(seed, idx, 3))), a1 = 6.2831853f * u01(seed, idx, 4);
   const float r2 = sqrtf(-2.f * logf(u01(seed, idx, 5))), a2 = 6.2831853f * u01(seed, idx, 6);
-  p.ux[idx] = ux0 + vth * r1 * cosf(a1);
-  p.uy[idx] = uy0 + vth * r1 * sinf(a1);
-  p.uz[idx] = uz0 + vth * r2 * cosf(a2);
-  p.q[idx] = q;
+  p.u[idx] = make_float4(ux0 + vth * r1 * cosf(a1), uy0 + vth * r1 * sinf(a1), uz0 + vth * r2 * cosf(a2), q);
 }
 
 int k_load_maxwellian(Engine *e, Species &s, int ppc, unsigned seed, float q, float ux, float uy, float uz, float vth) {
@@ -231,7 +229,7 @@
   const float4 rec = in.r[li];
   const int key = idx < np ? record_cell(rec) : -1;
   const bool valid = key >= 0;
-  const float ux = in.ux[li], uy = in.uy[li], uz = in.uz[li], q = in.q[li];
+  const float4 mom = in.u[li];
   int leader, rank, cnt;
   group_info(key, valid, lane, leader, rank, cnt);
   int base = 0;
@@ -240,7 +238,7 @@
   if (!valid) return;
   const int dst = base + rank;
   out.r[dst] = rec;
-  out.ux[dst] = ux; out.uy[dst] = uy; out.uz[dst] = uz; out.q[dst] = q;
+  out.u[dst] = mom;
   if (tin) { tout[dst] = tin[idx]; t2out[dst] = t2in[idx]; }
 }
 
@@ -296,7 +294,6 @@
   static_assert(WG_CHUNK >= 4 * WG_TABLE, "the tables fit the first staging buffer");
   __shared__ float4 s_both[WG_CHUNK / 2];
   int *const s_tables = reinterpret_cast<int *>(s_both);
-  float *const s_stage = reinterpret_cast<float *>(s_both) + WG_CHUNK;
   int *const s_key = s_tables, *const s_cnt = s_tables + WG_TABLE, *const s_lbase = s_tables + 2 * WG_TABLE, *const s_gbase = s_tables + 3 * WG_TABLE;
   __shared__ int s_dst[WG_CHUNK];
   __shared__ int s_wave[WG_T / 64], s_total;
@@ -357,12 +354,11 @@
   }
   __syncthreads();
   const int n_staged = s_total;
-  float *const src[4] = {in.ux, in.uy, in.uz, in.q};
-  float *const dst[4] = {out.ux, out.uy, out.uz, out.q};
-  float *const stage2 = reinterpret_cast<float *>(s_tables);
-  float v[WG_PER_THREAD];
-  {
-    constexpr int HALF = WG_CHUNK / 2, GROUP = 4;
+  const float4 *const src[2] = {in.r, in.u};
+  float4 *const dst[2] = {out.r, out.u};
+  constexpr int HALF = WG_CHUNK / 2, GROUP = 4;
+#pragma unroll
+  for (int f = 0; f < 2; f++) {
 #pragma unroll
     for (int half = 0; half < 2; half++) {
 #pragma unroll
@@ -373,43 +369,18 @@
         for (int j = 0; j < GROUP; j++) {
           const int idx = first + (j0 + j) * WG_T + threadIdx.x;
           here[j] = local[j0 + j] >= 0 ? (local[j0 + j] >= HALF) == (half == 1) : (slot[j0 + j] == -1 && half == 0);
-          rec[j] = here[j] ? in.r[idx] : make_float4(0.f, 0.f, 0.f, 0.f);
+          rec[j] = here[j] ? src[f][idx] : make_float4(0.f, 0.f, 0.f, 0.f);
         }
 #pragma unroll
         for (int j = 0; j < GROUP; j++) {
           if (!here[j]) continue;
           if (local[j0 + j] >= 0) s_both[local[j0 + j] - half * HALF] = rec[j];
-          else out.r[rank[j0 + j]] = rec[j];
+          else dst[f][rank[j0 + j]] = rec[j];
         }
       }
-      if (half == 1) {
-#pragma unroll
-        for (int j = 0; j < WG_PER_THREAD; j++) { const int idx = first + j * WG_T + threadIdx.x; v[j] = (slot[j] != -2) ? src[0][idx] : 0.f; }
-      }
       __syncthreads();
-      for (int k = threadIdx.x; k < HALF; k += WG_T) { if (half * HALF + k < n_staged) out.r[s_dst[half * HALF + k]] = s_both[k]; }
+      for (int k = threadIdx.x; k < HALF; k += WG_T) { if (half * HALF + k < n_staged) dst[f][s_dst[half * HALF + k]] = s_both[k]; }
       __syncthreads();
-    }
-  }
-#pragma unroll
-  for (int f = 0; f < 4; f++) {
-    float *const stage = (f & 1) ? stage2 : s_stage;
-    float vn[WG_PER_THREAD];
-    if (f + 1 < 4) {
-#pragma unroll
-      for (int j = 0; j < WG_PER_THREAD; j++) { const int idx = first + j * WG_T + threadIdx.x; vn[j] = (slot[j] != -2) ? src[f + 1][idx] : 0.f; }
-    }
-#pragma unroll
-    for (int j = 0; j < WG_PER_THREAD; j++) {
-      if (local[j] >= 0) stage[local[j]] = v[j];
-      else if (slot[j] == -1) dst[f][rank[j]] = v[j];
-    }
-    __syncthreads();
-#pragma unroll
-    for (int j = 0; j < WG_PER_THREAD; j++) { const int k = j * WG_T + threadIdx.x; if (k < n_staged) dst[f][s_dst[k]] = stage[k]; }
-    if (f + 1 < 4) {
-#pragma unroll
-      for (int j = 0; j < WG_PER_THREAD; j++) v[j] = vn[j];
     }
   }
   if (tin) {
@@ -462,15 +433,13 @@
   const int64_t n = (n_req + PUSH_TILE + PARTICLE_PAD - 1) / PARTICLE_PAD * PARTICLE_PAD;
   if (alloc_particles_raw(p, n)) return 1;
   VH_CHECK(hipMemset(p.r + (n - PARTICLE_PAD), 0, sizeof(float4) * PARTICLE_PAD));
-  float *arr[4] = {p.ux, p.uy, p.uz, p.q};
-  for (float *a : arr) VH_CHECK(hipMemset(a + (n - PARTICLE_PAD), 0, sizeof(float) * PARTICLE_PAD));
+  VH_CHECK(hipMemset(p.u + (n - PARTICLE_PAD), 0, sizeof(float4) * PARTICLE_PAD));
   VH_CHECK(hipDeviceSynchronize());
   return 0;
 }
 static int alloc_particles_raw_impl(ParticlesK &p, int64_t n) {
   VH_CHECK(hipMalloc(&p.r, sizeof(float4) * n));
-  VH_CHECK(hipMalloc(&p.ux, sizeof(float) * n)); VH_CHECK(hipMalloc(&p.uy, sizeof(float) * n));
-  VH_CHECK(hipMalloc(&p.uz, sizeof(float) * n)); VH_CHECK(hipMalloc(&p.q, sizeof(float) * n));
+  VH_CHECK(hipMalloc(&p.u, sizeof(float4) * n));
   return 0;
 }
 
@@ -595,12 +564,8 @@
   if (max_np > s.max_np) {
     ParticlesK bigger{};
     if (alloc_particles(bigger, max_np)) return 1;
-    float *src[4] = {s.p.ux, s.p.uy, s.p.uz, s.p.q};
-    float *dst[4] = {bigger.ux, bigger.uy, bigger.uz, bigger.q};
     if (s.np > 0) VH_CHECK(hipMemcpyAsync(bigger.r, s.p.r, sizeof(float4) * (size_t)s.np, hipMemcpyDeviceToDevice, e->stream));
-    for (int a = 0; a < 4; a++) {
-      if (s.np > 0) VH_CHECK(hipMemcpyAsync(dst[a], src[a], sizeof(float) * (size_t)s.np, hipMemcpyDeviceToDevice, e->stream));
-    }
+    if (s.np > 0) VH_CHECK(hipMemcpyAsync(bigger.u, s.p.u, sizeof(float4) * (size_t)s.np, hipMemcpyDeviceToDevice, e->stream));
     VH_CHECK(hipStreamSynchronize(e->stream));
     free_particles(s.p);
     s.p = bigger;
@@ -639,7 +604,7 @@
   if (k >= n) return;
   if (k >= *n_live) { record_set_cell(dst.r, k, -1); return; }
   dst.r[k] = src.r[k];
-  dst.ux[k] = src.ux[k]; dst.uy[k] = src.uy[k]; dst.uz[k] = src.uz[k]; dst.q[k] = src.q[k];
+  dst.u[k] = src.u[k];
   if (tsrc) { tdst[k] = tsrc[k]; t2dst[k] = t2src[k]; }
 }
 
@@ -835,7 +800,8 @@
   const int idx = m.i, new_np = np - nm;
   const float4 rec = p.r[idx];
   const float dx = rec.x, dy = rec.y, dz = rec.z;
-  const float ux = p.ux[idx], uy = p.uy[idx], uz = p.uz[idx], q = p.q[idx];
+  const float4 mom = p.u[idx];
+  const float ux = mom.x, uy = mom.y, uz = mom.z, q = mom.w;
   const int pi = record_cell(rec);
   bool absorb = true;
   int abs_face = 6, abs_flags = 0;
@@ -971,7 +937,7 @@
   if (t >= counters[C_HOLES]) return;
   const int d = holes[t], s = fills[t];
   p.r[d] = p.r[s];
-  p.ux[d] = p.ux[s]; p.uy[d] = p.uy[s]; p.uz[d] = p.uz[s]; p.q[d] = p.q[s];
+  p.u[d] = p.u[s];
   if (tag) { tag[d] = tag[s]; tag2[d] = tag2[s]; }
 }
 
@@ -1114,7 +1080,7 @@
   const int stuck = move_p_lane<false>(dx, dy, dz, pi, ux, uy, uz, inj.q, mx, my, mz, nullptr, g_acc, NO_WINDOW, g, false, det_scale);
   const ParticlesK p = Tp->p[s];
   p.r[idx] = make_record(dx, dy, dz, pi);
-  p.ux[idx] = ux; p.uy[idx] = uy; p.uz[idx] = uz; p.q[idx] = inj.q;
+  p.u[idx] = make_float4(ux, uy, uz, inj.q);
   if (Tp->tag[s]) { Tp->tag[s][idx] = tags ? tags[2 * t] : 0; Tp->tag2[s][idx] = tags ? tags[2 * t + 1] : 0; }
 
   if (stuck) {
diff --git a/old-vpic_amd/csrc/push.hip b/old-vpic_amd/csrc/push.hip
--- a/old-vpic_amd/csrc/push.hip
+++ b/old-vpic_amd/csrc/push.hip
@@ -53,9 +53,16 @@
   return reinterpret_cast<rec4 *>(reinterpret_cast<char *>(base) + ((uint64_t)dst << RECORD_SHIFT));
 }
 __device__ __forceinline__ int ldcell(const float4 *base, unsigned off) { return __float_as_int(*reinterpret_cast<const float *>(reinterpret_cast<const char *>(base) + off + 12u)); }
-__device__ __forceinline__ float ldf(const float *base, unsigned off) { return *reinterpret_cast<const float *>(reinterpret_cast<const char *>(base) + off); }
-__device__ __forceinline__ void stf(float *base, unsigned off, float v) { *reinterpret_cast<float *>(reinterpret_cast<char *>(base) + off) = v; }
-__device__ __forceinline__ void stf_nt(float *base, unsigned off, float v) { __builtin_nontemporal_store(v, reinterpret_cast<float *>(reinterpret_cast<char *>(base) + off)); }
+__device__ __forceinline__ void stu(float4 *base, unsigned off, float x, float y, float z, float q) {
+  rec4 v; v.x = x; v.y = y; v.z = z; v.w = q;
+  *reinterpret_cast<rec4 *>(reinterpret_cast<char *>(base) + off) = v;
+}
+__device__ __forceinline__ void stu_nt(float4 *base, unsigned off, float x, float y, float z, float q) {
+  rec4 v; v.x = x; v.y = y; v.z = z; v.w = q;
+  __builtin_nontemporal_store(v, reinterpret_cast<rec4 *>(reinterpret_cast<char *>(base) + off));
+}
+__device__ __forceinline__ float ldf(const float4 *base, unsigned off) { return *reinterpret_cast<const float *>(reinterpret_cast<const char *>(base) + off); }
+__device__ __forceinline__ void stf(float4 *base, unsigned off, float v) { *reinterpret_cast<float *>(reinterpret_cast<char *>(base) + off) = v; }
 
 
 __device__ __forceinline__ int in_vgpr(int s) { int v; asm volatile("v_mov_b32 %0, %1" : "=v"(v) : "s"(s)); return v; }
@@ -289,7 +296,7 @@
     const float q = mq->q[kq];
     vpic_particle_mover_t m; m.dispx = c2.x; m.dispy = c2.y; m.dispz = c2.z; m.i = __float_as_int(c2.w);
     const int idx = m.i;
-    const unsigned o4 = word_offset(idx, rel);
+    const unsigned o16 = record_offset(idx, rel);
     float dx = c0.x, dy = c0.y, dz = c0.z;
     int flips = (__float_as_int(c0.w) >> FLIP_SHIFT) & 7;
     const bool staged = STAGE && live && (__float_as_int(c0.w) >> STAGED_BIT) & 1;
@@ -399,14 +406,21 @@
 #endif
       if (!staged) {
         if (WIDE) { rec4 v; v.x = dx; v.y = dy; v.z = dz; v.w = __int_as_float(pi); __builtin_nontemporal_store(v, rec_at(p.r, (unsigned)idx)); }
-        else str_nt(p.r, o4 << 2, dx, dy, dz, pi);
+        else str_nt(p.r, o16, dx, dy, dz, pi);
       }
       if (HIST) hist_count<W>(*hk, pi, wbase, gsy, gsz, td);
       if (flips) {
         asm volatile("s_waitcnt vmcnt(0)" ::: "memory");
-        if (flips & 1) stf(p.ux, o4, -ldf(p.ux, o4));
-        if (flips & 2) stf(p.uy, o4, -ldf(p.uy, o4));
-        if (flips & 4) stf(p.uz, o4, -ldf(p.uz, o4));
+        if (WIDE) {
+          float *const m = reinterpret_cast<float *>(rec_at(p.u, (unsigned)idx));
+          if (flips & 1) m[0] = -m[0];
+          if (flips & 2) m[1] = -m[1];
+          if (flips & 4) m[2] = -m[2];
+        } else {
+          if (flips & 1) stf(p.u, o16 + word_offset(0, 0), -ldf(p.u, o16 + word_offset(0, 0)));
+          if (flips & 2) stf(p.u, o16 + word_offset(1, 0), -ldf(p.u, o16 + word_offset(1, 0)));
+          if (flips & 4) stf(p.u, o16 + word_offset(2, 0), -ldf(p.u, o16 + word_offset(2, 0)));
+        }
       }
       if (stuck) {
         const int gs = __hip_atomic_fetch_add(nm_counter, 1, __ATOMIC_RELAXED, __HIP_MEMORY_SCOPE_AGENT);
@@ -662,12 +676,11 @@
   pw = offset_particles(p, sfirst);
   rel = SORT ? 0 : sfirst;
   const int vrel_max = TILE ? in_vgpr(P.np - 1 - sfirst) : P.np - 1 - sfirst;
-  rec4 r_rec;
-  float r_ux, r_uy, r_uz, r_q;
+  rec4 r_rec, r_mom;
   {
-    const unsigned k4 = (unsigned)min(wave_first - sfirst + lane, P.np - 1 - sfirst) << 2;
-    r_rec = ldr(pw.r, k4 << 2);
-    r_ux = ldf(pw.ux, k4); r_uy = ldf(pw.uy, k4); r_uz = ldf(pw.uz, k4); r_q = ldf(pw.q, k4);
+    const unsigned k16 = (unsigned)min(wave_first - sfirst + lane, P.np - 1 - sfirst) << RECORD_SHIFT;
+    r_rec = ldr(pw.r, k16);
+    r_mom = ldr(pw.u, k16);
   }
 
 #pragma unroll 1
@@ -675,7 +688,7 @@
     const int base = wave_first + it * PASS_STRIDE;
     if (base >= wave_last) break;
     int idx = base + lane, key = (base + lane < wave_last) ? __float_as_int(r_rec.w) : -1;
-    float dx = r_rec.x, dy = r_rec.y, dz = r_rec.z, ux = r_ux, uy = r_uy, uz = r_uz, q = r_q;
+    float dx = r_rec.x, dy = r_rec.y, dz = r_rec.z, ux = r_mom.x, uy = r_mom.y, uz = r_mom.z, q = r_mom.w;
     const int kk = key < 0 ? 0x7fffffff : key;
     const int kprev = __builtin_amdgcn_update_dpp((int)0x80000000, kk, 0x138 , 0xf, 0xf, false);
     if (!UNORDERED && !(ablate & 16) && __ballot(kk < kprev)) {
@@ -719,9 +732,9 @@
     __builtin_amdgcn_sched_barrier(0);
     {
       const int k = base - sfirst + ((it + 1 < wave_passes) ? PASS_STRIDE : 0) + lane;
-      const unsigned k4 = (unsigned)min(k, vrel_max) << 2;
-      r_rec = ldr(pw.r, k4 << 2);
-      r_ux = ldf(pw.ux, k4); r_uy = ldf(pw.uy, k4); r_uz = ldf(pw.uz, k4); r_q = ldf(pw.q, k4);
+      const unsigned k16 = (unsigned)min(k, vrel_max) << RECORD_SHIFT;
+      r_rec = ldr(pw.r, k16);
+      r_mom = ldr(pw.u, k16);
     }
     __builtin_amdgcn_sched_barrier(0);
     const bool active = key >= 0;
@@ -730,7 +743,7 @@
     float sux, suy, suz;
     float spx = 0.f, spy = 0.f, spz = 0.f;
     {
-      const unsigned o4 = word_offset(idx, sfirst);
+      const unsigned o16 = record_offset(idx, sfirst);
       float v0, v1, v2, v3, v4, v5;
       if (FAST) {
         const float hax = qdt_2mc * __builtin_fmaf(dz, __builtin_fmaf(dy, fe_x.w, fe_x.z), __builtin_fmaf(dy, fe_x.y, fe_x.x));
@@ -784,20 +797,19 @@
       if (SORT) {
         dst = __shfl(sort_b, sort_head) + (lane - sort_head);
         if (active) {
-          const unsigned d4 = (unsigned)dst << 2;
-          stf(P.out.ux, d4, sux); stf(P.out.uy, d4, suy); stf(P.out.uz, d4, suz);
+          rec4 m; m.x = sux; m.y = suy; m.z = suz; m.w = q;
+          *rec_at(P.out.u, (unsigned)dst) = m;
           rec4 v; v.x = incell ? v3 : dx; v.y = incell ? v4 : dy; v.z = incell ? v5 : dz; v.w = __int_as_float(key);
           *rec_at(P.out.r, (unsigned)dst) = v;
-          stf(P.out.q, d4, q);
         }
       } else
       if (STAGE && stage) {
-        if (!TILE || active) { stf(pw.ux, o4, sux); stf(pw.uy, o4, suy); stf(pw.uz, o4, suz); }
+        if (!TILE || active) stu(pw.u, o16, sux, suy, suz, q);
         spx = incell ? v3 : dx; spy = incell ? v4 : dy; spz = incell ? v5 : dz;
       } else
       if ((!TILE || active) && !(ablate & 128)) {
-        stf_nt(pw.ux, o4, sux); stf_nt(pw.uy, o4, suy); stf_nt(pw.uz, o4, suz);
-        str(pw.r, o4 << 2, incell ? v3 : dx, incell ? v4 : dy, incell ? v5 : dz, key);
+        stu_nt(pw.u, o16, sux, suy, suz, q);
+        str(pw.r, o16, incell ? v3 : dx, incell ? v4 : dy, incell ? v5 : dz, key);
       }
       if (!CHARGELESS && !(ablate & 1)) {
         const float qd = (incell && active) ? q : 0.f;
@@ -1170,12 +1182,13 @@
     const float dx = rec.x, dy = rec.y, dz = rec.z;
     const float4 *f = fi + (size_t)record_cell(rec) * 5;
     const float4 fe_x = f[0], fe_y = f[1], fe_z = f[2];
-    float v0 = p.ux[idx] + qdt_2mc * ((fe_x.x + dy * fe_x.y) + dz * (fe_x.z + dy * fe_x.w));
-    float v1 = p.uy[idx] + qdt_2mc * ((fe_y.x + dz * fe_y.y) + dx * (fe_y.z + dz * fe_y.w));
-    float v2 = p.uz[idx] + qdt_2mc * ((fe_z.x + dx * fe_z.y) + dy * (fe_z.z + dx * fe_z.w));
+    const float4 mom = p.u[idx];
+    float v0 = mom.x + qdt_2mc * ((fe_x.x + dy * fe_x.y) + dz * (fe_x.z + dy * fe_x.w));
+    float v1 = mom.y + qdt_2mc * ((fe_y.x + dz * fe_y.y) + dx * (fe_y.z + dz * fe_y.w));
+    float v2 = mom.z + qdt_2mc * ((fe_z.x + dx * fe_z.y) + dy * (fe_z.z + dx * fe_z.w));
     v0 = v0 * v0 + v1 * v1 + v2 * v2;
     v0 /= sqrtf(one + v0) + one;
-    en += (double)v0 * (double)p.q[idx];
+    en += (double)v0 * (double)mom.w;
   }
   for (int off = 32; off; off >>= 1) en += __shfl_down(en, off);
   if ((threadIdx.x & 63) == 0) s_sum[threadIdx.x >> 6] = en;
@@ -1219,7 +1232,8 @@
   const float hay = qdt_2mc * ((fe_y.x + dz * fe_y.y) + dx * (fe_y.z + dz * fe_y.w));
   const float haz = qdt_2mc * ((fe_z.x + dx * fe_z.y) + dy * (fe_z.z + dx * fe_z.w));
   const float cbx = fb0.x + dx * fb0.y, cby = fb0.z + dy * fb0.w, cbz = fb1.x + dz * fb1.y;
-  float ux = p.ux[idx], uy = p.uy[idx], uz = p.uz[idx], v0, v1, v2, v3, v4;
+  const float4 mom = p.u[idx];
+  float ux = mom.x, uy = mom.y, uz = mom.z, v0, v1, v2, v3, v4;
   if (!UNCENTER) { ux += hax; uy += hay; uz += haz; }
   v0 = qdt_4mc / sqrtf(one + (ux * ux + (uy * uy + uz * uz)));
   v1 = cbx * cbx + (cby * cby + cbz * cbz);
@@ -1234,7 +1248,7 @@
   uy += v4 * (v2 * cbx - v0 * cbz);
   uz += v4 * (v0 * cby - v1 * cbx);
   if (UNCENTER) { ux += hax; uy += hay; uz += haz; }
-  p.ux[idx] = ux; p.uy[idx] = uy; p.uz[idx] = uz;
+  p.u[idx] = make_float4(ux, uy, uz, mom.w);
 }
 
 int k_center_p(Engine *e, Species &s, bool uncenter) {
@@ -1260,7 +1274,8 @@
   const int ii = record_cell(rec);
   if (ii < 0) return;
   HydroP P;
-  hydro_particle(rec.x, rec.y, rec.z, p.ux[idx], p.uy[idx], p.uz[idx], p.q[idx], load_interp(fi, ii), hc, P);
+  const float4 mom = p.u[idx];
+  hydro_particle(rec.x, rec.y, rec.z, mom.x, mom.y, mom.z, mom.w, load_interp(fi, ii), hc, P);
   float *h = h0 + (size_t)ii * HYDRO_STRIDE;
 #pragma unroll
   for (int n = 0; n < 8; n++) {
@@ -1288,7 +1303,8 @@
   for (int idx = first; idx < last; idx++) {
     HydroP P;
     const float4 rec = p.r[idx];
-    hydro_particle(rec.x, rec.y, rec.z, p.ux[idx], p.uy[idx], p.uz[idx], p.q[idx], f, hc, P);
+    const float4 mom = p.u[idx];
+    hydro_particle(rec.x, rec.y, rec.z, mom.x, mom.y, mom.z, mom.w, f, hc, P);
 #pragma unroll
     for (int n = 0; n < 8; n++) {
       float c[HYDRO_MOMENTS];
diff --git a/old-vpic_amd/csrc/select.hip b/old-vpic_amd/csrc/select.hip
--- a/old-vpic_amd/csrc/select.hip
+++ b/old-vpic_amd/csrc/select.hip
@@ -129,7 +129,7 @@
       if (out_p) {
         float4 *rec = reinterpret_cast<float4 *>(out_p + dest);
         rec[0] = make_float4(dx, dy, dz, __int_as_float(voxel));
-        rec[1] = make_float4(p.ux[idx], p.uy[idx], p.uz[idx], p.q[idx]);
+        rec[1] = p.u[idx];
         const long long t1 = tag ? tag[idx] : 0, t2 = tag ? tag2[idx] : 0;
         *reinterpret_cast<ulonglong2 *>(rec + 2) = make_ulonglong2((unsigned long long)t1, (unsigned long long)t2);
       }
diff --git a/old-vpic_amd/csrc/spectrum.hip b/old-vpic_amd/csrc/spectrum.hip
--- a/old-vpic_amd/csrc/spectrum.hip
+++ b/old-vpic_amd/csrc/spectrum.hip
@@ -40,8 +40,8 @@
 
 template <bool TILE>
 __global__ __launch_bounds__(64 * SPEC_WAVES)
-void energy_spectrum_kernel(const float4 *__restrict__ prec, const float *__restrict__ pux, const float *__restrict__ puy,
-                            const float *__restrict__ puz, long long np, long long chunk, SpectrumK k, GridK g, TileK t,
+void energy_spectrum_kernel(const float4 *__restrict__ prec, const float4 *__restrict__ pu,
+                            long long np, long long chunk, SpectrumK k, GridK g, TileK t,
                             unsigned *__restrict__ lin, unsigned long long *__restrict__ logc,
                             unsigned long long *__restrict__ stats) {
   extern __shared__ unsigned s_mem[];
@@ -63,7 +63,8 @@
     if (!__any(live)) continue;
     double ke = 0;
     if (live) {
-      const float ux = pux[idx], uy = puy[idx], uz = puz[idx];
+      const float4 mom = pu[idx];
+      const float ux = mom.x, uy = mom.y, uz = mom.z;
       const double gam2 = ((1.0 + (double)ux * (double)ux) + (double)uy * (double)uy) + (double)uz * (double)uz;
       ke = sqrt(gam2) - 1.0;
     }
@@ -133,7 +134,7 @@
     const size_t lds = sizeof(unsigned) * ((size_t)sp.n_log + (size_t)SPEC_WAVES * k.win * sp.n_lin);
     const TileK tk = make_tile_k(e->gk);
     auto kernel = s.tile_valid ? energy_spectrum_kernel<true> : energy_spectrum_kernel<false>;
-    hipLaunchKernelGGL(kernel, dim3((unsigned)ch.groups), dim3(64 * SPEC_WAVES), lds, e->stream, (const float4 *)s.p.r, s.p.ux, s.p.uy, s.p.uz,
+    hipLaunchKernelGGL(kernel, dim3((unsigned)ch.groups), dim3(64 * SPEC_WAVES), lds, e->stream, (const float4 *)s.p.r, (const float4 *)s.p.u,
                        (long long)s.np, ch.chunk, k, e->gk, tk, e->spec_lin, e->spec_log, e->spec_stats.dev);
     VH_CHECK(hipGetLastError());
   }
```

Measured after the change: 58.93 billion. -2.2%, worse.
